# ai2cm/ace

Measured on AMD Instinct MI355X. Metric: rollout steps/sec (6-hourly forward steps of the 1-degree SFNO, whole job), higher is better.
Workload: dtype f32 (contractions with K>=32 on error-compensated fp16x3 MFMA, fp32 accumulate; DFT, norms, epilogues fp32; measured error vs fp64 below the fp32 CPU reference's); 1 GPU; ACE2-ERA5-shape 1deg SFNO rollout (BASELINE.json configs[1]): embed 384, 8 layers, dhconv, 44 in / 50 out channels, 180x360 legendre-gauss, lmax 180, mmax 181, B=1 member per GPU, random-init weights; members=1, members_per_gpu=1, graph=step, precision=f16x3, collective=none

## Files before the change

### ace_amd/csrc/capi.hip

```cpp
#include <hip/hip_runtime.h>

#include <algorithm>
#include <cmath>
#include <cstdio>
#include <cstdlib>
#include <cstring>
#include <map>
#include <memory>
#include <string>
#include <tuple>
#include <vector>

#include "../../include/ace_sfno.h"
#include "kernels.h"
#include "strip_pack.h"
#include "tables.h"

using namespace ace;

static thread_local std::string g_err;

static int fail(int code, const std::string& msg) {
    g_err = msg;
    return code;
}
#define HIP_TRY(expr)                                                                                      \
    do {                                                                                                   \
        hipError_t e__ = (expr);                                                                           \
        if (e__ != hipSuccess)                                                                             \
            return fail(ACE_ERR_RUNTIME, std::string(#expr) + ": " + hipGetErrorString(e__));              \
    } while (0)
#define ACE_TRY(expr)                \
    do {                             \
        int rc__ = (expr);           \
        if (rc__ != ACE_OK) return rc__; \
    } while (0)

extern "C" const char* ace_last_error(void) { return g_err.c_str(); }

namespace ace {
Switches read_switches() {
    auto on = [](const char* name) { const char* e = std::getenv(name); return e && e[0] && !(e[0] == '0' && !e[1]); };
    Switches sw;
    sw.no_fft = on("ACE_NO_FFT");
    sw.no_strip = on("ACE_NO_STRIP");
    sw.no_fold = on("ACE_NO_FOLD");
    sw.no_dhconv_strip = on("ACE_NO_DHCONV_STRIP");
#ifdef ACE_MEASUREMENT_SWITCHES
    sw.no_pk = on("ACE_NO_PK");
    sw.no_pk_sht = on("ACE_NO_PK_SHT");
#endif
    sw.no_enc_ws = on("ACE_NO_ENC_WS");
    sw.no_enc_pk = on("ACE_NO_ENC_PK");
    sw.no_cln_mfma = on("ACE_NO_CLN_MFMA");
    sw.no_cln_planes = on("ACE_NO_CLN_PLANES");
    sw.dense_grouped_filter = on("ACE_DENSE_GROUPED_FILTER");
    if (const char* e = std::getenv("ACE_CONV_WL")) sw.conv_wl = !(e[0] == '0' && !e[1]);
    if (const char* e = std::getenv("ACE_PLANES_STREAM")) sw.planes_stream = !(e[0] == '0' && !e[1]);
    if (const char* e = std::getenv("ACE_FUSED_PACK")) sw.fused_pack = !(e[0] == '0' && !e[1]);
    if (const char* e = std::getenv("ACE_CONV_WS")) {
        const std::string v(e);
        if (v == "all" || v == "1") sw.conv_ws_roles = 7;
        else sw.conv_ws_roles = (v.find("skip") != std::string::npos ? 1 : 0) | (v.find("fc1") != std::string::npos ? 2 : 0) |
                                (v.find("fc2") != std::string::npos ? 4 : 0);
    }
    return sw;
}
}
extern "C" int ace_version(void) { return 100; }

struct DevBuf {
    float* p = nullptr;
    size_t n = 0;
    DevBuf() = default;
    DevBuf(const DevBuf&) = delete;
    DevBuf& operator=(const DevBuf&) = delete;
    DevBuf(DevBuf&& o) noexcept : p(o.p), n(o.n) { o.p = nullptr; o.n = 0; }
    DevBuf& operator=(DevBuf&& o) noexcept {
        if (this != &o) { release(); p = o.p; n = o.n; o.p = nullptr; o.n = 0; }
        return *this;
    }
    ~DevBuf() { release(); }
    void release() {
        if (p) (void)hipFree(p);
        p = nullptr;
        n = 0;
    }
    hipError_t alloc(size_t count, bool zero = true) {
        release();
        if (count == 0) return hipSuccess;
        hipError_t e = hipMalloc(reinterpret_cast<void**>(&p), count * sizeof(float));
        if (e != hipSuccess) { p = nullptr; return e; }
        n = count;
        if (zero) e = hipMemset(p, 0, count * sizeof(float));
        return e;
    }
    hipError_t ensure(size_t count) { return count <= n ? hipSuccess : alloc(count); }
    hipError_t upload(const std::vector<float>& h) {
        hipError_t e = alloc(h.size(), false);
        if (e != hipSuccess) return e;
        return hipMemcpy(p, h.data(), h.size() * sizeof(float), hipMemcpyHostToDevice);
    }
};

struct ace_sht_plan {
    int nlat = 0, nlon = 0, lmax = 0, mmax = 0, Hp = 0, Lp = 0, Kfp = 0;
    Grid grid = GRID_LEGENDRE_GAUSS;
    DevBuf wt, pt, fc, fs, gc, gs;
    DevBuf X, D;
    DevBuf wt_hi, wt_lo, pt_hi, pt_lo;
    float wt_scale = 1.f, pt_scale = 1.f;
    float wt_winf = 0.f;
    bool f16 = false;
    DevBuf wt_frag, pt_frag, wt_off, pt_off;
    bool strip = false;
    DevBuf wt_ffrag, pt_ffrag, wt_foff, pt_foff;
    bool fold = false;
    DevBuf slots;
    Switches sw;
    mutable int route[2] = {-1, -1};
};
static int fold_route(const LegStripArgs& f) { return legendre_fold_is_big(f) ? 3 : 2; }

static float pow2_scale_for(const std::vector<float>& v) {
    float mx = 0.f;
    for (float x : v) mx = std::max(mx, std::fabs(x));
    int e = 0;
    if (mx > 0.f && std::isfinite(mx)) { (void)std::frexp(mx, &e); e = 10 - e; }
    return std::ldexp(1.0f, e);
}

static int plan_build(int nlat, int nlon, int lmax, int mmax, Grid g, std::unique_ptr<ace_sht_plan>& out,
                      bool f16 = false) {
    ShtTables t;
    std::string err = build_sht_tables(nlat, nlon, lmax, mmax, g, t);
    if (!err.empty()) return fail(ACE_ERR_INVALID, err);
    auto p = std::make_unique<ace_sht_plan>();
    p->sw = read_switches();
    p->nlat = t.nlat; p->nlon = t.nlon; p->lmax = t.lmax; p->mmax = t.mmax;
    p->Hp = t.Hp; p->Lp = t.Lp; p->Kfp = t.Kfp; p->grid = g;
    HIP_TRY(p->wt.upload(t.wt));
    HIP_TRY(p->pt.upload(t.pt));
    HIP_TRY(p->fc.upload(t.fc));
    HIP_TRY(p->fs.upload(t.fs));
    HIP_TRY(p->gc.upload(t.gc));
    HIP_TRY(p->gs.upload(t.gs));
    if (f16) {
        p->f16 = true;
        p->wt_scale = pow2_scale_for(t.wt);
        for (size_t r = 0; r < (size_t)t.mmax * t.lmax; ++r) {
            double rs = 0.0;
            for (int k = 0; k < t.nlat; ++k) rs += std::fabs((double)t.wt[r * t.Hp + k]);
            p->wt_winf = std::max(p->wt_winf, (float)(rs * (1.0 + 1e-6)));
        }
        p->pt_scale = pow2_scale_for(t.pt);
        const size_t hw = (t.wt.size() + 1) / 2, hp = (t.pt.size() + 1) / 2;
        HIP_TRY(p->wt_hi.alloc(hw, false)); HIP_TRY(p->wt_lo.alloc(hw, false));
        HIP_TRY(p->pt_hi.alloc(hp, false)); HIP_TRY(p->pt_lo.alloc(hp, false));
        HIP_TRY(launch_split_f16(p->wt.p, t.Hp, p->wt_hi.p, p->wt_lo.p, t.Hp, (long)t.mmax * t.lmax, t.Hp, p->wt_scale, nullptr));
        HIP_TRY(launch_split_f16(p->pt.p, t.Lp, p->pt_hi.p, p->pt_lo.p, t.Lp, (long)t.mmax * t.nlat, t.Lp, p->pt_scale, nullptr));
        HIP_TRY(hipDeviceSynchronize());
        auto up = [](const StripPack& sp, DevBuf& frag, DevBuf& off) -> hipError_t {
            hipError_t e = frag.alloc((sp.frags.size() + 1) / 2, false);
            if (e != hipSuccess) return e;
            e = hipMemcpy(frag.p, sp.frags.data(), sp.frags.size() * sizeof(uint16_t), hipMemcpyHostToDevice);
            if (e != hipSuccess) return e;
            e = off.alloc(sp.tile_off.size(), false);
            if (e != hipSuccess) return e;
            return hipMemcpy(off.p, sp.tile_off.data(), sp.tile_off.size() * sizeof(int), hipMemcpyHostToDevice);
        };
        if (t.nlat <= 192 && t.lmax <= 192) {
            StripPack sp;
            pack_legendre_strip(t.wt.data(), t.mmax, t.lmax, t.nlat, t.Hp, 0, p->wt_scale, sp);
            HIP_TRY(up(sp, p->wt_frag, p->wt_off));
            pack_legendre_strip(t.pt.data(), t.mmax, t.nlat, t.lmax, t.Lp, 1, p->pt_scale, sp);
            HIP_TRY(up(sp, p->pt_frag, p->pt_off));
            p->strip = true;
        }
        if ((t.nlat + 1) / 2 <= 16 * FOLD_NKP_BIG && (t.lmax + 1) / 2 <= 16 * FOLD_NKP_BIG && !p->sw.no_fold &&
            fold_symmetry_error(t.wt.data(), t.mmax, t.nlat, t.lmax, t.Hp, 0) < 2e-6 &&
            fold_symmetry_error(t.pt.data(), t.mmax, t.nlat, t.lmax, t.Lp, 1) < 2e-6) {
            StripPack sp;
            pack_legendre_fold(t.wt.data(), t.mmax, t.nlat, t.lmax, t.Hp, 0, p->wt_scale, sp);
            HIP_TRY(up(sp, p->wt_ffrag, p->wt_foff));
            pack_legendre_fold(t.pt.data(), t.mmax, t.nlat, t.lmax, t.Lp, 1, p->pt_scale, sp);
            HIP_TRY(up(sp, p->pt_ffrag, p->pt_foff));
            p->fold = true;
        }
    }
    out = std::move(p);
    return ACE_OK;
}

static int run_dft_forward(const ace_sht_plan& pl, const float* x, const float* sc, const float* sh, float* X, int Bt,
                           int C, hipStream_t s, unsigned* xmax = nullptr, const _Float16* xhi = nullptr,
                           const _Float16* xlo = nullptr, long sxp = 0, const unsigned* xslot = nullptr,
                           const PackFragArgs* ride = nullptr, bool* rode = nullptr) {
    DftArgs a;
    if (rode) *rode = false;
    if (ride && rode) { a.ride = *ride; a.nride = pack_frag_blocks(*ride); a.rode = rode; }
    a.omax = xmax;
    a.xhi = xhi; a.xlo = xlo; a.sxp = sxp; a.xslot = xslot;
    a.x = xhi ? nullptr : x; a.spec_out = X; a.tc = pl.fc.p; a.ts = pl.fs.p; a.ldt = pl.Kfp; a.sc = sc; a.sh = sh;
    a.Bt = Bt; a.C = C; a.H = pl.nlat; a.W = pl.nlon; a.Mm = pl.mmax; a.no_fft = pl.sw.no_fft;
    HIP_TRY(launch_dft_forward(a, s));
    return ACE_OK;
}
static int run_dft_inverse(const ace_sht_plan& pl, const float* X, const float* bias, float* y, int Bt, int C,
                           hipStream_t s, unsigned* ymax = nullptr) {
    DftArgs a;
    a.omax = ymax;
    a.spec = X; a.y = y; a.tc = pl.gc.p; a.ts = pl.gs.p; a.ldt = pl.Kfp; a.bias = bias;
    a.Bt = Bt; a.C = C; a.H = pl.nlat; a.W = pl.nlon; a.Mm = pl.mmax; a.no_fft = pl.sw.no_fft;
    HIP_TRY(launch_dft_inverse(a, s));
    return ACE_OK;
}
static int run_legendre_forward(const ace_sht_plan& pl, const float* X, float* D, long N2, hipStream_t s,
                                const unsigned* xmax = nullptr, unsigned* dmax = nullptr, bool planes = false) {
    GemmArgs g;
    g.omax = planes ? nullptr : dmax;
    g.A = pl.wt.p; g.lda = pl.Hp; g.sA = (long)pl.lmax * pl.Hp;
    g.B = X; g.ldb = N2; g.sB = (long)pl.nlat * N2;
    g.C = D; g.ldc = (long)pl.mmax * N2; g.sC = N2;
    g.M = pl.lmax; g.N = (int)N2; g.K = pl.nlat; g.nbatch = pl.mmax; g.a_kpad = pl.Hp;
    g.tri = TRI_ROWS_GE_BATCH;
    if ((pl.strip || pl.fold) && !pl.sw.no_strip && xmax) {
        LegStripArgs a;
        a.B = X; a.b_kstride = N2; a.b_moff = (long)pl.nlat * N2;
        a.A = reinterpret_cast<const _Float16*>(pl.wt_frag.p); a.tile_off = reinterpret_cast<const int*>(pl.wt_off.p);
        a.ascale = pl.wt_scale; a.bmax = xmax;
        a.c_rstride = (long)pl.mmax * N2; a.c_moff = N2;
        a.N = (int)N2; a.K = pl.nlat; a.R = pl.lmax; a.nbatch = pl.mmax; a.mode = 0;
        if (planes) {
            a.Chi = reinterpret_cast<_Float16*>(D);
            a.Clo = a.Chi + (size_t)pl.lmax * pl.mmax * N2;
            a.cw = pl.wt_winf; a.cslot = dmax;
        } else {
            a.C = D; a.omax = dmax;
        }
        if (pl.fold && !pl.sw.no_fold) {
            LegStripArgs f = a;
            f.A = reinterpret_cast<const _Float16*>(pl.wt_ffrag.p); f.tile_off = reinterpret_cast<const int*>(pl.wt_foff.p);
            if (legendre_fold_eligible(f)) {
                HIP_TRY(launch_legendre_fold(f, s));
                pl.route[0] = fold_route(f);
                return ACE_OK;
            }
        }
        if (pl.strip && legendre_strip_eligible(a)) {
            HIP_TRY(launch_legendre_strip(a, s));
            pl.route[0] = 1;
            return ACE_OK;
        }
    }
    pl.route[0] = 0;
    if (planes) {
        if (!(pl.f16 && xmax && dmax && gemm_f16x3_eligible(g))) return fail(ACE_ERR_STATE, "legendre planes path not eligible");
        _Float16* Dh = reinterpret_cast<_Float16*>(D);
        _Float16* Dl = Dh + (size_t)pl.lmax * pl.mmax * N2;
        HIP_TRY(launch_gemm_f16x3_planes(g, pl.wt_hi.p, pl.wt_lo.p, pl.wt_scale, xmax, Dh, Dl, pl.wt_winf, dmax, s));
        return ACE_OK;
    }
    if (pl.f16 && xmax && gemm_f16x3_eligible(g)) {
        HIP_TRY(launch_gemm_f16x3(g, pl.wt_hi.p, pl.wt_lo.p, pl.wt_scale, 1.f, s, xmax, dmax));
        return ACE_OK;
    }
    HIP_TRY(launch_gemm(g, s));
    return ACE_OK;
}
static int run_legendre_inverse(const ace_sht_plan& pl, const float* E, float* X, long N2, hipStream_t s,
                                const unsigned* emax = nullptr, bool dry = false) {
    GemmArgs g;
    g.A = pl.pt.p; g.lda = pl.Lp; g.sA = (long)pl.nlat * pl.Lp;
    g.B = E; g.ldb = (long)pl.mmax * N2; g.sB = N2;
    g.C = X; g.ldc = N2; g.sC = (long)pl.nlat * N2;
    g.M = pl.nlat; g.N = (int)N2; g.K = pl.lmax; g.nbatch = pl.mmax; g.a_kpad = pl.Lp;
    g.tri = TRI_K_GE_BATCH;
    if ((pl.strip || pl.fold) && !pl.sw.no_strip && emax) {
        LegStripArgs a;
        a.B = E; a.b_kstride = (long)pl.mmax * N2; a.b_moff = N2;
        a.A = reinterpret_cast<const _Float16*>(pl.pt_frag.p); a.tile_off = reinterpret_cast<const int*>(pl.pt_off.p);
        a.ascale = pl.pt_scale; a.bmax = emax;
        a.C = X; a.c_rstride = N2; a.c_moff = (long)pl.nlat * N2;
        a.N = (int)N2; a.K = pl.lmax; a.R = pl.nlat; a.nbatch = pl.mmax; a.mode = 1;
        if (pl.fold && !pl.sw.no_fold) {
            LegStripArgs f = a;
            f.A = reinterpret_cast<const _Float16*>(pl.pt_ffrag.p); f.tile_off = reinterpret_cast<const int*>(pl.pt_foff.p);
            if (legendre_fold_eligible(f)) {
                if (!dry) HIP_TRY(launch_legendre_fold(f, s));
                pl.route[1] = fold_route(f);
                return ACE_OK;
            }
        }
        if (pl.strip && legendre_strip_eligible(a)) {
            if (!dry) HIP_TRY(launch_legendre_strip(a, s));
            pl.route[1] = 1;
            return ACE_OK;
        }
    }
    pl.route[1] = 0;
    if (dry) return ACE_OK;
    if (pl.f16 && emax && gemm_f16x3_eligible(g)) {
        HIP_TRY(launch_gemm_f16x3(g, pl.pt_hi.p, pl.pt_lo.p, pl.pt_scale, 1.f, s, emax, nullptr));
        return ACE_OK;
    }
    HIP_TRY(launch_gemm(g, s));
    return ACE_OK;
}

extern "C" int ace_sht_plan_create_ex(int nlat, int nlon, int lmax, int mmax, const char* grid, int precision,
                                      ace_sht_plan** plan) {
    if (!plan || !grid) return fail(ACE_ERR_INVALID, "null argument");
    if (precision != 0 && precision != 1) return fail(ACE_ERR_INVALID, "precision must be 0 (fp32) or 1 (f16x3)");
    Grid g;
    if (std::string(grid) == "healpix") return fail(ACE_ERR_INVALID, "'healpix' grid not supported");
    if (!parse_grid(grid, &g)) return fail(ACE_ERR_INVALID, "Unknown quadrature mode");
    std::unique_ptr<ace_sht_plan> p;
    ACE_TRY(plan_build(nlat, nlon, lmax, mmax, g, p, precision == 1));
    if (precision == 1) HIP_TRY(p->slots.alloc((size_t)2 * AMAX_SHARDS));
    *plan = p.release();
    return ACE_OK;
}
extern "C" int ace_sht_plan_create(int nlat, int nlon, int lmax, int mmax, const char* grid, ace_sht_plan** plan) {
    return ace_sht_plan_create_ex(nlat, nlon, lmax, mmax, grid, 0, plan);
}
extern "C" void ace_sht_plan_destroy(ace_sht_plan* plan) { delete plan; }
extern "C" int ace_sht_plan_dims(const ace_sht_plan* p, int* nlat, int* nlon, int* lmax, int* mmax) {
    if (!p) return fail(ACE_ERR_INVALID, "null plan");
    if (nlat) *nlat = p->nlat;
    if (nlon) *nlon = p->nlon;
    if (lmax) *lmax = p->lmax;
    if (mmax) *mmax = p->mmax;
    return ACE_OK;
}

extern "C" int ace_sht_plan_route(const ace_sht_plan* p, int* forward, int* inverse) {
    if (!p) return fail(ACE_ERR_INVALID, "null plan");
    if (forward) *forward = p->route[0];
    if (inverse) *inverse = p->route[1];
    return ACE_OK;
}

extern "C" int ace_sht_forward(ace_sht_plan* p, const float* x, float* coeffs, int n, void* stream) {
    if (!p || !x || !coeffs || n <= 0) return fail(ACE_ERR_INVALID, "ace_sht_forward: bad argument");
    hipStream_t s = static_cast<hipStream_t>(stream);
    const long N2 = 2L * n;
    HIP_TRY(p->X.ensure(((size_t)p->mmax * p->nlat + LEG_STRIP_SLACK_ROWS) * N2));
    HIP_TRY(p->D.ensure(((size_t)p->lmax + LEG_STRIP_SLACK_ROWS) * p->mmax * N2));
    unsigned* xmax = nullptr;
    if (p->f16 && p->slots.p) {
        xmax = reinterpret_cast<unsigned*>(p->slots.p);
        HIP_TRY(launch_zero_u32(xmax, 2 * AMAX_SHARDS, s));
    }
    ACE_TRY(run_dft_forward(*p, x, nullptr, nullptr, p->X.p, 1, n, s, xmax));
    ACE_TRY(run_legendre_forward(*p, p->X.p, p->D.p, N2, s, xmax, xmax ? xmax + AMAX_SHARDS : nullptr));
    HIP_TRY(launch_spec_to_ref(p->D.p, coeffs, 1, n, p->lmax, p->mmax, s));
    return ACE_OK;
}
extern "C" int ace_sht_inverse(ace_sht_plan* p, const float* coeffs, float* x, int n, void* stream) {
    if (!p || !x || !coeffs || n <= 0) return fail(ACE_ERR_INVALID, "ace_sht_inverse: bad argument");
    hipStream_t s = static_cast<hipStream_t>(stream);
    const long N2 = 2L * n;
    HIP_TRY(p->X.ensure(((size_t)p->mmax * p->nlat + LEG_STRIP_SLACK_ROWS) * N2));
    HIP_TRY(p->D.ensure(((size_t)p->lmax + LEG_STRIP_SLACK_ROWS) * p->mmax * N2));
    unsigned* emax = nullptr;
    if (p->f16 && p->slots.p) {
        emax = reinterpret_cast<unsigned*>(p->slots.p);
        HIP_TRY(launch_zero_u32(emax, 2 * AMAX_SHARDS, s));
    }
    ACE_TRY(run_legendre_inverse(*p, p->D.p, p->X.p, N2, s, emax, true));
    HIP_TRY(launch_ref_to_spec(coeffs, p->D.p, 1, n, p->lmax, p->mmax, s, emax, p->route[1] != 0));
    ACE_TRY(run_legendre_inverse(*p, p->D.p, p->X.p, N2, s, emax));
    ACE_TRY(run_dft_inverse(*p, p->X.p, nullptr, x, 1, n, s));
    return ACE_OK;
}

extern "C" int ace_sht_tables_host(int nlat, int nlon, int lmax, int mmax, const char* grid, int which,
                                   void* out_host) {
    if (!grid || !out_host) return fail(ACE_ERR_INVALID, "null argument");
    Grid g;
    if (!parse_grid(grid, &g)) return fail(ACE_ERR_INVALID, "Unknown quadrature mode");
    if (which == 2 || which == 3) {
        std::vector<double> x, w;
        quadrature(g, nlat, x, w);
        std::memcpy(out_host, (which == 2 ? x : w).data(), sizeof(double) * nlat);
        return ACE_OK;
    }
    ShtTables t;
    std::string err = build_sht_tables(nlat, nlon, lmax, mmax, g, t);
    if (!err.empty()) return fail(ACE_ERR_INVALID, err);
    float* o = static_cast<float*>(out_host);
    for (int m = 0; m < t.mmax; ++m)
        for (int l = 0; l < t.lmax; ++l)
            for (int k = 0; k < t.nlat; ++k) {
                const size_t dst = ((size_t)m * t.lmax + l) * t.nlat + k;
                if (which == 0) o[dst] = t.wt[((size_t)m * t.lmax + l) * t.Hp + k];
                else if (which == 1) o[dst] = t.pt[((size_t)m * t.nlat + k) * t.Lp + l];
                else return fail(ACE_ERR_INVALID, "unknown table id");
            }
    return ACE_OK;
}

extern "C" int ace_conv1x1(const float* x, const float* weight, const float* bias, float* y, int n, int cin, int cout,
                           long hw, int act, void* stream) {
    if (!x || !weight || !y || n <= 0 || cin <= 0 || cout <= 0 || hw <= 0)
        return fail(ACE_ERR_INVALID, "ace_conv1x1: bad argument");
    GemmArgs g;
    g.A = weight; g.lda = cin; g.sA = 0;
    g.B = x; g.ldb = hw; g.sB = (long)cin * hw;
    g.C = y; g.ldc = hw; g.sC = (long)cout * hw;
    g.bias = bias; g.M = cout; g.N = (int)hw; g.K = cin; g.nbatch = n; g.act = act;
    g.a_kpad = cin;
    HIP_TRY(launch_gemm(g, static_cast<hipStream_t>(stream)));
    return ACE_OK;
}

extern "C" int ace_conv1x1_f16x3(const float* x, const float* weight, const float* bias, float* y, int n, int cin,
                                 int cout, long hw, int act, void* stream) {
    if (!x || !weight || !y || n <= 0 || cin <= 0 || cout <= 0 || hw <= 0)
        return fail(ACE_ERR_INVALID, "ace_conv1x1_f16x3: bad argument");
    hipStream_t s = static_cast<hipStream_t>(stream);
    const int pitch = (cin + 31) & ~31;
    std::vector<float> host((size_t)cout * cin);
    HIP_TRY(hipStreamSynchronize(s));
    HIP_TRY(hipMemcpy(host.data(), weight, host.size() * sizeof(float), hipMemcpyDeviceToHost));
    float mx = 0.f;
    for (float v : host) mx = std::max(mx, std::fabs(v));
    int e = 0;
    if (mx > 0.f && std::isfinite(mx)) { (void)std::frexp(mx, &e); e = 10 - e; }
    const float ascale = std::ldexp(1.0f, e);
    DevBuf hi, lo;
    const size_t halves = (size_t)cout * pitch;
    HIP_TRY(hi.alloc((halves + 1) / 2, false));
    HIP_TRY(lo.alloc((halves + 1) / 2, false));
    HIP_TRY(launch_split_f16(weight, cin, hi.p, lo.p, pitch, cout, cin, ascale, s));
    GemmArgs g;
    g.lda = pitch; g.sA = 0; g.a_kpad = pitch;
    g.B = x; g.ldb = hw; g.sB = (long)cin * hw;
    g.C = y; g.ldc = hw; g.sC = (long)cout * hw;
    g.bias = bias; g.M = cout; g.N = (int)hw; g.K = cin; g.nbatch = n; g.act = act;
    if (!gemm_f16x3_eligible(g)) return fail(ACE_ERR_INVALID, "ace_conv1x1_f16x3: needs 16-byte aligned x and hw % 4 == 0");
    if (g.act == ACT_GELU) g.act = ACT_GELU_FAST;
    DevBuf slotbuf;
    HIP_TRY(slotbuf.alloc(AMAX_SHARDS));
    unsigned* xslot = reinterpret_cast<unsigned*>(slotbuf.p);
    HIP_TRY(launch_absmax(x, (long)n * cin * hw, xslot, s));
    HIP_TRY(launch_gemm_f16x3(g, hi.p, lo.p, ascale, 1.0f, s, xslot, nullptr));
    HIP_TRY(hipStreamSynchronize(s));
    return ACE_OK;
}

struct PreparedWeight { DevBuf hi, lo; int pitch = 0; float ascale = 1.f, winf = 0.f; };
static int prepare_weight(const float* weight, int rows, int cols, hipStream_t s, PreparedWeight& out, bool tiled) {
    std::vector<float> host((size_t)rows * cols);
    HIP_TRY(hipStreamSynchronize(s));
    HIP_TRY(hipMemcpy(host.data(), weight, host.size() * sizeof(float), hipMemcpyDeviceToHost));
    float mx = 0.f;
    for (int r = 0; r < rows; ++r) {
        double rs = 0.0;
        for (int c = 0; c < cols; ++c) { const float v = std::fabs(host[(size_t)r * cols + c]); mx = std::max(mx, v); rs += v; }
        out.winf = std::max(out.winf, (float)(rs * (1.0 + 1e-6)));
    }
    int e = 0;
    if (mx > 0.f && std::isfinite(mx)) { (void)std::frexp(mx, &e); e = 10 - e; }
    out.ascale = std::ldexp(1.0f, e);
    out.pitch = (cols + 31) & ~31;
    const size_t halves = (size_t)((rows + 15) / 16 * 16) * out.pitch;
    HIP_TRY(out.hi.alloc((halves + 1) / 2, false));
    HIP_TRY(out.lo.alloc((halves + 1) / 2, false));
    if (tiled) HIP_TRY(launch_split_f16_tiled(weight, cols, out.hi.p, out.lo.p, out.pitch, rows, cols, out.ascale, s));
    else HIP_TRY(launch_split_f16(weight, cols, out.hi.p, out.lo.p, out.pitch, rows, cols, out.ascale, s));
    return ACE_OK;
}

extern "C" int ace_mlp_f16x3(const float* x, const float* w1, const float* b1, const float* w2, const float* b2, float* y,
                             int n, int cin, int hid, int cout, long hw, int act, void* stream) {
    if (!x || !w1 || !w2 || !y || n <= 0 || cin <= 0 || hid <= 0 || cout <= 0 || hw <= 0)
        return fail(ACE_ERR_INVALID, "ace_mlp_f16x3: bad argument");
    if (cin % 8 != 0 || hid % 8 != 0 || hw % 4 != 0)
        return fail(ACE_ERR_INVALID, "ace_mlp_f16x3: needs cin % 8 == 0, hid % 8 == 0, hw % 4 == 0");
    hipStream_t s = static_cast<hipStream_t>(stream);
    PreparedWeight p1, p2;
    ACE_TRY(prepare_weight(w1, hid, cin, s, p1, true));
    ACE_TRY(prepare_weight(w2, cout, hid, s, p2, true));
    float b1max = 0.f;
    if (b1) {
        std::vector<float> hb((size_t)hid);
        HIP_TRY(hipMemcpy(hb.data(), b1, hb.size() * sizeof(float), hipMemcpyDeviceToHost));
        for (float v : hb) b1max = std::max(b1max, std::fabs(v));
    }
    DevBuf slots, xp, up;
    HIP_TRY(slots.alloc(2 * AMAX_SHARDS, true));
    HIP_TRY(xp.alloc((size_t)n * cin * hw, true));
    HIP_TRY(up.alloc((size_t)n * hid * hw, true));
    unsigned* xslot = reinterpret_cast<unsigned*>(slots.p);
    unsigned* uslot = xslot + AMAX_SHARDS;
    _Float16* xh = reinterpret_cast<_Float16*>(xp.p);
    _Float16* xl = xh + (size_t)n * cin * hw;
    _Float16* uh = reinterpret_cast<_Float16*>(up.p);
    _Float16* ul = uh + (size_t)n * hid * hw;
    HIP_TRY(launch_absmax(x, (long)n * cin * hw, xslot, s));
    HIP_TRY(launch_pack_pformat(x, hw, (long)cin * hw, cin, (int)hw, n, nullptr, nullptr, 0, xslot, xh, xl, hw,
                                (long)cin * hw, s));
    Gemm4Args a;
    a.Ahi = reinterpret_cast<const _Float16*>(p1.hi.p); a.Alo = reinterpret_cast<const _Float16*>(p1.lo.p);
    a.lda = p1.pitch; a.ascale = p1.ascale; a.a_tiled = 1;
    a.Bhi = xh; a.Blo = xl; a.ldn = hw; a.sB = (long)cin * hw; a.bmax = xslot;
    a.Chi = uh; a.Clo = ul; a.ldnc = hw; a.sCp = (long)hid * hw; a.cw = p1.winf; a.cb = b1max; a.cslot = uslot;
    a.bias = b1; a.M = hid; a.N = (int)hw; a.K = cin; a.nbatch = n;
    a.act = act == ACT_GELU ? ACT_GELU_FAST : act;
    HIP_TRY(launch_gemm_f16x3_packed(a, s));
    Gemm4Args b;
    b.Ahi = reinterpret_cast<const _Float16*>(p2.hi.p); b.Alo = reinterpret_cast<const _Float16*>(p2.lo.p);
    b.lda = p2.pitch; b.ascale = p2.ascale; b.a_tiled = 1;
    b.Bhi = uh; b.Blo = ul; b.ldn = hw; b.sB = (long)hid * hw; b.bmax = uslot;
    b.C = y; b.ldc = hw; b.sC = (long)cout * hw;
    b.bias = b2; b.M = cout; b.N = (int)hw; b.K = hid; b.nbatch = n; b.act = ACT_NONE;
    HIP_TRY(launch_gemm_f16x3_packed(b, s));
    HIP_TRY(hipStreamSynchronize(s));
    return ACE_OK;
}

static hipError_t upload_dhconv_units(int L, int Mrows, int trimul, int C, DevBuf& buf, int* per_xcd) {
    std::vector<int> u;
    *per_xcd = dhconv_build_units(L, Mrows, trimul, C, u);
    hipError_t e = buf.alloc(u.size(), false);
// ... 136 lines not shown
    HIP_TRY(launch_unpack_denormalize(src, mean, std_, dsts, strides, batch, nch, hw, static_cast<hipStream_t>(stream)));
    return ACE_OK;
}

struct Weight {
    std::string name;
    long numel = 0;
    DevBuf buf;
    bool set = false;
    int block = -1;
    bool is_filter = false;
    long ext_numel = 0;
    int rows = 0, cols = 0, pitch = 0;
    DevBuf hi, lo;
    float ascale = 1.f;
    DevBuf thi, tlo;
    DevBuf frag0;
    float wabs = 0.f;
    float winf = 0.f;
    float absmax = 0.f;
};

struct GraphKey {
    const float* in; float* out; int batch;
    bool operator<(const GraphKey& o) const { return std::tie(in, out, batch) < std::tie(o.in, o.out, o.batch); }
};

struct ace_sfno {
    ace_sfno_config cfg;
    int H = 0, W = 0, C = 0, L = 0, Mm = 0, hid = 0, Bmax = 1;
    long HW = 0;
    long HWs = 0;
    int Hs = 0, Ws = 0;
    std::unique_ptr<ace_sht_plan> plan_lg, plan_data_own;
    ace_sht_plan* plan_data = nullptr;
    std::vector<std::unique_ptr<Weight>> weights;
    std::map<std::string, int> index;
    std::vector<DevBuf> wx;
    std::vector<DevBuf> wx_hi, wx_lo;
    std::vector<float> wx_scale;
    std::vector<char> wx_compact;
    std::vector<DevBuf> dh_units; std::vector<int> dh_units_per_xcd;
    std::vector<char> wx_native;
    DevBuf h0, h1, Y, T, R, U, X, D, E, stats;
    DevBuf P;
    DevBuf cln_stats;
    DevBuf inN;
    std::unique_ptr<ace_sht_plan> plan_res;
    DevBuf resX, resD, inF;
    DevBuf P2;
    DevBuf part;
    DevBuf Wp0, Wp1;
    DevBuf Wq1;
    DevBuf Wq0;
    DevBuf zero_c;
    DevBuf inP;
    DevBuf pe_slot;
    DevBuf phys;
    int nstrips = 0;
    DevBuf bf0, bf1;
    DevBuf amax;
    bool taps_on = false;
    std::vector<DevBuf> taps;
    std::map<GraphKey, hipGraphExec_t> graphs;
    hipStream_t capture_stream = nullptr;
    long weights_generation = 0;
    bool graphs_stale = false;
    mutable int norm_batch = 0;
    mutable hipStream_t norm_stream = nullptr;
    Switches sw;

    const float* w(const std::string& name) const {
        auto it = index.find(name);
        return it == index.end() ? nullptr : weights[it->second]->buf.p;
    }
    const Weight* find(const std::string& name) const {
        auto it = index.find(name);
        return it == index.end() ? nullptr : weights[it->second].get();
    }
};

static void add_weight(ace_sfno* n, const std::string& name, long numel, int block = -1, bool is_filter = false) {
    auto w = std::make_unique<Weight>();
    w->name = name; w->numel = numel; w->block = block; w->is_filter = is_filter;
    n->index[name] = (int)n->weights.size();
    n->weights.push_back(std::move(w));
}
static void add_conv_weight(ace_sfno* n, const std::string& name, int rows, int cols) {
    add_weight(n, name, (long)rows * cols);
    Weight& w = *n->weights.back();
    w.rows = rows; w.cols = cols; w.pitch = (cols + 31) & ~31;
}

static bool skip_on_conv_ws(const Switches& sw, int K, int M, long HW) { return conv_ws_eligible(K, M, HW, 0, sw.conv_ws_roles); }
static bool fc1_on_conv_ws(const Switches& sw, int K, int M, long HW) { return conv_ws_eligible(K, M, HW, 1, sw.conv_ws_roles); }
static bool fc2_on_conv_ws(const Switches& sw, int K, int M, long HW) { return conv_ws_eligible(K, M, HW, 2, sw.conv_ws_roles); }
static bool fc1_on_conv_wl(const Switches& sw, int K, int M, long HW) { return sw.conv_wl && conv_wl_eligible(K, M, HW); }
static bool cln_skip_on_conv_ws(const Switches& sw, int K, int M, long HW) {
    return (sw.conv_ws_roles & 1) && conv_ws_eligible(K, M, HW, -1, sw.conv_ws_roles);
}

extern "C" int ace_sfno_create(const ace_sfno_config* cfg, ace_sfno** out) {
    if (!cfg || !out) return fail(ACE_ERR_INVALID, "null argument");
    const ace_sfno_config& c = *cfg;
    if (c.scale_factor < 1) return fail(ACE_ERR_INVALID, "scale_factor must be >= 1");
    if ((c.scale_factor != 1 || c.residual_filter_factor > 1) && c.normalization_layer == 2)
        return fail(ACE_ERR_INVALID, "scale_factor / residual_filter_factor != 1 are not built for the noise-conditioned nets");
    if (c.residual_filter_factor < 0) return fail(ACE_ERR_INVALID, "residual_filter_factor must be >= 1");
    if (c.in_chans <= 0 || c.out_chans <= 0 || c.embed_dim <= 0 || c.num_layers <= 0 || c.nlat < 2 || c.nlon < 2)
        return fail(ACE_ERR_INVALID, "non-positive dimension in ace_sfno_config");
    if (c.operator_type != 0 && c.operator_type != 1) return fail(ACE_ERR_INVALID, "Unsupported operator type");
    if (c.normalization_layer < 0 || c.normalization_layer > 3)
        return fail(ACE_ERR_INVALID, "normalization_layer must be 'none', 'instance_norm', conditional layer norm or 'layer_norm'");
    const bool cln = c.normalization_layer == 2;
    if (cln) {
        if (c.operator_type != 1) return fail(ACE_ERR_INVALID, "Only 'dhconv' operator_type is supported for NoiseConditionedSFNO models.");
        if (c.noise_embed_dim < 0 || c.noise_embed_dim > 512) return fail(ACE_ERR_INVALID, "noise_embed_dim must be in [0, 512]");
        if (c.filter_num_groups < 1 || c.embed_dim % c.filter_num_groups != 0)
            return fail(ACE_ERR_INVALID, "embed_dim must be divisible by filter_num_groups");
    }
    if (c.activation_function < 1 || c.activation_function > 3)
        return fail(ACE_ERR_INVALID, "Unknown activation function");
    if (c.data_grid != GRID_LEGENDRE_GAUSS && c.data_grid != GRID_EQUIANGULAR && c.data_grid != GRID_LOBATTO)
        return fail(ACE_ERR_INVALID, "data_grid must be 'legendre-gauss', 'equiangular' or 'lobatto'");
    if (c.encoder_layers < 0) return fail(ACE_ERR_INVALID, "encoder_layers must be >= 0");
    if (c.precision != 0 && c.precision != 1) return fail(ACE_ERR_INVALID, "precision must be 0 (fp32) or 1 (f16x3)");

    auto n = std::make_unique<ace_sfno>();
    n->cfg = c;
    n->sw = read_switches();
    n->H = c.nlat; n->W = c.nlon; n->C = c.embed_dim; n->HW = (long)c.nlat * c.nlon;
    n->Bmax = c.max_batch > 0 ? c.max_batch : 1;
    const int sf = c.scale_factor;
    n->Hs = c.nlat / sf; n->Ws = c.nlon / sf; n->HWs = (long)n->Hs * n->Ws;
    if (n->Hs < 1 || n->Ws < 2) return fail(ACE_ERR_INVALID, "scale_factor leaves no grid");
    n->L = (int)(n->Hs * c.hard_thresholding_fraction);
    n->Mm = (int)((n->Ws / 2 + 1) * c.hard_thresholding_fraction);
    if (n->L < 1 || n->Mm < 1) return fail(ACE_ERR_INVALID, "hard_thresholding_fraction leaves no modes");
    n->hid = (int)(c.embed_dim * c.mlp_ratio);

    ACE_TRY(plan_build(n->Hs, n->Ws, n->L, n->Mm, GRID_LEGENDRE_GAUSS, n->plan_lg, c.precision == 1));
    if (c.data_grid == GRID_LEGENDRE_GAUSS && sf == 1) {
        n->plan_data = n->plan_lg.get();
    } else {
        ACE_TRY(plan_build(c.nlat, c.nlon, n->L, n->Mm, (Grid)c.data_grid, n->plan_data_own, c.precision == 1));
        n->plan_data = n->plan_data_own.get();
    }

    if (c.residual_filter_factor > 1 && c.big_skip) {
        const int rl = c.nlat / c.residual_filter_factor, rm = c.nlon / c.residual_filter_factor / 2 + 1;
        if (rl < 1 || rm < 1) return fail(ACE_ERR_INVALID, "residual_filter_factor leaves no modes");
        ACE_TRY(plan_build(c.nlat, c.nlon, rl, rm, (Grid)c.data_grid, n->plan_res, false));
        const size_t n2 = (size_t)n->Bmax * 2 * c.in_chans;
        HIP_TRY(n->resX.alloc(((size_t)rm * c.nlat + LEG_STRIP_SLACK_ROWS) * n2));
        HIP_TRY(n->resD.alloc(((size_t)rl + LEG_STRIP_SLACK_ROWS) * rm * n2));
        HIP_TRY(n->inF.alloc((size_t)n->Bmax * c.in_chans * n->HW));
    }

    const long C = n->C, HW = n->HW;
    if (c.pos_embed) add_weight(n.get(), "pos_embed", C * HW);
    long cur = c.in_chans;
    for (int j = 0; j < c.encoder_layers; ++j) {
        add_conv_weight(n.get(), "encoder." + std::to_string(2 * j) + ".weight", (int)C, (int)cur);
        add_weight(n.get(), "encoder." + std::to_string(2 * j) + ".bias", C);
        cur = C;
    }
    add_conv_weight(n.get(), "encoder." + std::to_string(2 * c.encoder_layers) + ".weight", (int)C, (int)cur);
    for (int i = 0; i < c.num_layers; ++i) {
        const std::string p = "blocks." + std::to_string(i) + ".";
        if (c.normalization_layer == 1) { add_weight(n.get(), p + "norm0.weight", C); add_weight(n.get(), p + "norm0.bias", C); }
        const long hw_n0 = i == 0 ? HW : n->HWs;
        const long hw_n1 = (i == 0 || i + 1 < c.num_layers) ? n->HWs : HW;
        if (c.normalization_layer == 3) { add_weight(n.get(), p + "norm0.weight", hw_n0); add_weight(n.get(), p + "norm0.bias", hw_n0); }
        auto add_cln = [&](const std::string& q, long ch) {
            if (c.noise_embed_dim > 0) {
                add_weight(n.get(), q + "W_scale_2d.weight", ch * c.noise_embed_dim);
                add_weight(n.get(), q + "W_bias_2d.weight", ch * c.noise_embed_dim);
            }
            if (c.affine_norms) { add_weight(n.get(), q + "norm.weight", ch); add_weight(n.get(), q + "norm.bias", ch); }
        };
        if (cln) add_cln(p + "norm0.", C);
        const long fw = c.operator_type == 1 ? C * C * n->L * 2 : C * C * (long)n->L * n->Mm * 2;
        add_weight(n.get(), p + "filter.filter.weight", fw, i, true);
        if (cln) n->weights.back()->ext_numel = fw / c.filter_num_groups;
        add_weight(n.get(), p + "filter.filter.bias", C);
        add_conv_weight(n.get(), p + "inner_skip.weight", (int)C, (int)C);
        add_weight(n.get(), p + "inner_skip.bias", C);
        if (c.normalization_layer == 1) { add_weight(n.get(), p + "norm1.weight", C); add_weight(n.get(), p + "norm1.bias", C); }
        if (c.normalization_layer == 3) { add_weight(n.get(), p + "norm1.weight", hw_n1); add_weight(n.get(), p + "norm1.bias", hw_n1); }
        if (cln) add_cln(p + "norm1.", C);
        if (c.use_mlp) {
            add_conv_weight(n.get(), p + "mlp.fwd.0.weight", n->hid, (int)C);
            add_weight(n.get(), p + "mlp.fwd.0.bias", n->hid);
            add_conv_weight(n.get(), p + "mlp.fwd.2.weight", (int)C, n->hid);
            add_weight(n.get(), p + "mlp.fwd.2.bias", C);
        }
    }
    cur = C + (c.big_skip ? c.in_chans : 0);
    for (int j = 0; j < c.encoder_layers; ++j) {
        add_conv_weight(n.get(), "decoder." + std::to_string(2 * j) + ".weight", (int)C, (int)cur);
        add_weight(n.get(), "decoder." + std::to_string(2 * j) + ".bias", C);
        cur = C;
    }
    add_conv_weight(n.get(), "decoder." + std::to_string(2 * c.encoder_layers) + ".weight", c.out_chans, (int)cur);
    if (cln && c.normalize_big_skip && c.big_skip) {
        if (c.noise_embed_dim > 0) {
            add_weight(n.get(), "norm_big_skip.W_scale_2d.weight", (long)c.in_chans * c.noise_embed_dim);
            add_weight(n.get(), "norm_big_skip.W_bias_2d.weight", (long)c.in_chans * c.noise_embed_dim);
        }
        if (c.affine_norms) { add_weight(n.get(), "norm_big_skip.norm.weight", c.in_chans); add_weight(n.get(), "norm_big_skip.norm.bias", c.in_chans); }
    }

    n->wx.resize(c.num_layers);
    n->wx_hi.resize(c.num_layers);
    n->wx_lo.resize(c.num_layers);
    n->wx_scale.assign(c.num_layers, 1.f);
    n->wx_compact.assign(c.num_layers, 0);
    n->wx_native.assign(c.num_layers, 0);
    for (int i = 0; i < c.num_layers; ++i) {
        const bool mixed = (n->plan_data != n->plan_lg.get()) && (i == 0 || i == c.num_layers - 1);
        n->wx_compact[i] = (!n->sw.no_pk_sht && c.precision == 1 && c.operator_type == 1 && n->C % 128 == 0 && !mixed &&
                            ((long)n->Bmax * 2 * n->C) % 4 == 0) ? 1 : 0;
        const bool strip_rows_ok = ((long)n->Mm * n->Bmax + 191) / 192 <= 65535;
        n->wx_native[i] = (n->wx_compact[i] && cln && c.filter_num_groups > 1 && !n->sw.dense_grouped_filter && !n->sw.no_dhconv_strip &&
                           strip_rows_ok && dhconv_native_groups_ok(n->C, c.filter_num_groups)) ? 1 : 0;
    }
    if (c.operator_type == 1 && c.precision == 1 && n->C % 128 == 0) {
        n->dh_units.resize(n->Bmax);
        n->dh_units_per_xcd.assign(n->Bmax, 0);
        for (int b = 1; b <= n->Bmax; ++b)
            HIP_TRY(upload_dhconv_units(n->L, n->Mm * b, b, n->C, n->dh_units[b - 1], &n->dh_units_per_xcd[b - 1]));
    }
    const size_t act = (size_t)n->Bmax * C * HW;
    const size_t spec_x = ((size_t)n->Mm * n->H + LEG_STRIP_SLACK_ROWS) * n->Bmax * 2 * C;
    const size_t spec_d = ((size_t)n->L + LEG_STRIP_SLACK_ROWS) * n->Mm * n->Bmax * 2 * C;
    HIP_TRY(n->h0.alloc(act));
    HIP_TRY(n->h1.alloc(act));
    HIP_TRY(n->Y.alloc(act));
    HIP_TRY(n->T.alloc(act));
    if (n->plan_data != n->plan_lg.get()) HIP_TRY(n->R.alloc(act));
    if (c.use_mlp) HIP_TRY(n->U.alloc((size_t)n->Bmax * n->hid * HW, true));
    if (c.precision == 1) {
        HIP_TRY(n->P.alloc(act, true));
        if (c.normalization_layer == 1 && c.use_mlp) {
            HIP_TRY(n->P2.alloc(act, true));
            n->nstrips = (int)((HW + 31) / 32) + 8;
            if (fc1_on_conv_ws(n->sw, (int)C, n->hid, HW) || fc1_on_conv_wl(n->sw, (int)C, n->hid, HW))
                HIP_TRY(n->Wq1.alloc((size_t)n->Bmax * n->hid * C, true));
            if (skip_on_conv_ws(n->sw, (int)C, (int)C, HW)) HIP_TRY(n->Wq0.alloc((size_t)n->Bmax * C * C, true));
            HIP_TRY(n->zero_c.alloc((size_t)C, true));
            HIP_TRY(n->inP.alloc((size_t)n->Bmax * ((c.in_chans + 7) / 8 * 8) * n->HW, true));
            HIP_TRY(n->pe_slot.alloc(64, true));
            HIP_TRY(n->part.alloc((size_t)2 * n->Bmax * n->nstrips * C * 4, true));
            const size_t cp = (size_t)((C + 31) & ~31);
            HIP_TRY(n->Wp0.alloc((size_t)n->Bmax * ((C + 15) / 16 * 16) * cp, true));
            HIP_TRY(n->Wp1.alloc((size_t)n->Bmax * ((n->hid + 15) / 16 * 16) * cp, true));
        }
    }
    HIP_TRY(n->X.alloc(spec_x));
    HIP_TRY(n->D.alloc(spec_d));
    HIP_TRY(n->E.alloc(spec_d));
    HIP_TRY(n->stats.alloc((size_t)4 * n->Bmax * C));
    if (cln) {
        HIP_TRY(n->cln_stats.alloc((size_t)2 * n->Bmax * HW));
        if (c.normalize_big_skip && c.big_skip) HIP_TRY(n->inN.alloc((size_t)n->Bmax * c.in_chans * HW));
    }
    HIP_TRY(n->amax.alloc((size_t)(16 + 12 * c.num_layers + 1) * AMAX_SHARDS));
    if (c.normalization_layer == 1) {
        HIP_TRY(n->bf0.alloc((size_t)n->Bmax * C));
        if (c.use_mlp) {
            HIP_TRY(n->bf1.alloc((size_t)n->Bmax * n->hid));
        }
    }
    *out = n.release();
    return ACE_OK;
}

extern "C" void ace_sfno_destroy(ace_sfno* n) {
    if (!n) return;
    for (auto& kv : n->graphs) (void)hipGraphExecDestroy(kv.second);
    if (n->capture_stream) (void)hipStreamDestroy(n->capture_stream);
    delete n;
}

extern "C" long ace_sfno_weights_generation(const ace_sfno* n) { return n ? n->weights_generation : -1; }

extern "C" long ace_sfno_workspace_size(const ace_sfno* n, int batch) {
    if (!n) { (void)fail(ACE_ERR_INVALID, "null argument"); return -1; }
    if (batch <= 0 || batch > n->Bmax) {
        (void)fail(ACE_ERR_INVALID, "batch " + std::to_string(batch) + " outside [1, max_batch=" + std::to_string(n->Bmax) + "]");
        return -1;
    }
    size_t fl = 0;
    auto add = [&](const DevBuf& b) { fl += b.n; };
    for (const DevBuf* b : {&n->h0, &n->h1, &n->Y, &n->T, &n->R, &n->U, &n->X, &n->D, &n->E, &n->stats, &n->P, &n->cln_stats, &n->inN,
                            &n->P2, &n->part, &n->Wp0, &n->Wp1, &n->Wq1, &n->Wq0, &n->zero_c, &n->inP, &n->pe_slot, &n->bf0,
                            &n->bf1, &n->amax, &n->phys})
        add(*b);
    for (const auto& t : n->taps) add(t);
    for (const auto& v : {&n->wx, &n->wx_hi, &n->wx_lo})
        for (const auto& b : *v) add(b);
    for (const auto& w : n->weights)
        for (const DevBuf* b : {&w->buf, &w->hi, &w->lo, &w->thi, &w->tlo, &w->frag0}) add(*b);
    auto plan_bytes = [&](const ace_sht_plan* p) {
        if (!p) return;
        for (const DevBuf* b : {&p->wt, &p->pt, &p->fc, &p->fs, &p->gc, &p->gs, &p->X, &p->D, &p->wt_hi, &p->wt_lo, &p->pt_hi, &p->pt_lo,
                                &p->wt_frag, &p->pt_frag, &p->wt_off, &p->pt_off, &p->slots})
            add(*b);
    };
    plan_bytes(n->plan_lg.get());
    plan_bytes(n->plan_data_own.get());
    plan_bytes(n->plan_res.get());
    for (const DevBuf* b : {&n->resX, &n->resD, &n->inF}) add(*b);
    return (long)(fl * sizeof(float));
}

extern "C" int ace_sfno_num_weights(const ace_sfno* n) { return n ? (int)n->weights.size() : 0; }
extern "C" const char* ace_sfno_weight_name(const ace_sfno* n, int i) {
    if (!n || i < 0 || i >= (int)n->weights.size()) return nullptr;
    return n->weights[i]->name.c_str();
}
extern "C" long ace_sfno_weight_numel(const ace_sfno* n, int i) {
    if (!n || i < 0 || i >= (int)n->weights.size()) return -1;
    return n->weights[i]->ext_numel ? n->weights[i]->ext_numel : n->weights[i]->numel;
}

extern "C" int ace_sfno_set_weight(ace_sfno* n, const char* name, const float* src, long numel, void* stream) {
    if (!n || !name || !src) return fail(ACE_ERR_INVALID, "null argument");
    auto it = n->index.find(name);
    if (it == n->index.end()) return fail(ACE_ERR_INVALID, std::string("unknown parameter '") + name + "'");
    Weight& w = *n->weights[it->second];
    const long expect = w.ext_numel ? w.ext_numel : w.numel;
    if (numel != expect)
        return fail(ACE_ERR_INVALID, std::string("size mismatch for ") + name + ": expected " +
                                         std::to_string(expect) + " elements, got " + std::to_string(numel));
    hipStream_t s = static_cast<hipStream_t>(stream);
    const bool native_groups = w.ext_numel && w.is_filter && w.block >= 0 && n->wx_native[w.block];
    if (native_groups) {
        if (!w.buf.p) HIP_TRY(w.buf.alloc((size_t)w.ext_numel, false));
        HIP_TRY(hipMemcpyAsync(w.buf.p, src, sizeof(float) * w.ext_numel, hipMemcpyDeviceToDevice, s));
        src = nullptr;
        numel = w.ext_numel;
    } else if (w.ext_numel) {
        if (!w.buf.p) HIP_TRY(w.buf.alloc((size_t)w.numel, false));
        HIP_TRY(launch_csfno_weight_to_dense(src, w.buf.p, n->C, n->cfg.filter_num_groups, n->L, s));
        src = nullptr;
        numel = w.numel;
    }
    if (w.pitch > 0) {
        if (!w.buf.p) HIP_TRY(w.buf.alloc((size_t)w.rows * w.pitch, true));
        HIP_TRY(hipMemcpy2DAsync(w.buf.p, sizeof(float) * w.pitch, src, sizeof(float) * w.cols, sizeof(float) * w.cols,
                                 w.rows, hipMemcpyDeviceToDevice, s));
    } else if (src) {
        if (!w.buf.p) HIP_TRY(w.buf.alloc((size_t)numel, false));
        HIP_TRY(hipMemcpyAsync(w.buf.p, src, sizeof(float) * numel, hipMemcpyDeviceToDevice, s));
    }
    if (w.is_filter && n->cfg.operator_type == 1) {
        const size_t cnt = (size_t)n->L * 2 * n->C * 2 * n->C;
        const bool packed = n->cfg.precision == 1 && (2 * n->C) % 32 == 0;
        if (packed) {
            DevBuf slotbuf;
            HIP_TRY(slotbuf.alloc(AMAX_SHARDS));
            HIP_TRY(launch_absmax(w.buf.p, numel, reinterpret_cast<unsigned*>(slotbuf.p), s));
            unsigned bits[AMAX_SHARDS];
            HIP_TRY(hipMemcpyAsync(bits, slotbuf.p, sizeof(bits), hipMemcpyDeviceToHost, s));
            HIP_TRY(hipStreamSynchronize(s));
            float mx = 0.f;
            for (unsigned b : bits) { float f; std::memcpy(&f, &b, 4); mx = std::max(mx, f); }
            int e = 0;
            if (mx > 0.f && std::isfinite(mx)) { (void)std::frexp(mx, &e); e = 10 - e; }
            n->wx_scale[w.block] = std::ldexp(1.0f, e);
            const bool compact = n->wx_compact[w.block] != 0;
            const size_t halves = native_groups ? cnt / 2 / n->cfg.filter_num_groups : (compact ? cnt / 2 : cnt);
            if (!n->wx_hi[w.block].p) HIP_TRY(n->wx_hi[w.block].alloc((halves + 1) / 2, false));
            if (!n->wx_lo[w.block].p) HIP_TRY(n->wx_lo[w.block].alloc((halves + 1) / 2, false));
            if (native_groups)
                HIP_TRY(launch_pack_dhconv_f16g(w.buf.p, n->wx_hi[w.block].p, n->wx_lo[w.block].p, n->C, n->cfg.filter_num_groups, n->L,
                                                n->wx_scale[w.block], s));
            else if (compact)
                HIP_TRY(launch_pack_dhconv_f16c(w.buf.p, n->wx_hi[w.block].p, n->wx_lo[w.block].p, n->C, n->C, n->L,
                                                n->wx_scale[w.block], s));
            else
                HIP_TRY(launch_pack_dhconv_f16(w.buf.p, n->wx_hi[w.block].p, n->wx_lo[w.block].p, n->C, n->C, n->L,
                                               n->wx_scale[w.block], s));
        } else {
            DevBuf& wx = n->wx[w.block];
            if (!wx.p) HIP_TRY(wx.alloc(cnt, false));
            HIP_TRY(launch_expand_dhconv_weight(w.buf.p, wx.p, n->C, n->C, n->L, s));
        }
    }
    HIP_TRY(hipStreamSynchronize(s));
    if (w.pitch > 0 && n->cfg.precision == 1) {
        std::vector<float> host((size_t)w.rows * w.pitch);
        HIP_TRY(hipMemcpy(host.data(), w.buf.p, host.size() * sizeof(float), hipMemcpyDeviceToHost));
        float mx = 0.f;
        for (float v : host) mx = std::max(mx, std::fabs(v));
        w.wabs = mx;
        w.winf = 0.f;
        for (int r = 0; r < w.rows; ++r) {
            double rs = 0.0;
            for (int cidx = 0; cidx < w.cols; ++cidx) rs += std::fabs((double)host[(size_t)r * w.pitch + cidx]);
            w.winf = std::max(w.winf, (float)(rs * (1.0 + 1e-6)));
        }
        int e = 0;
        if (mx > 0.f && std::isfinite(mx)) { (void)std::frexp(mx, &e); e = 10 - e; }
        w.ascale = std::ldexp(1.0f, e);
        const size_t halves = (size_t)w.rows * w.pitch;
        if (!w.hi.p) HIP_TRY(w.hi.alloc((halves + 1) / 2, false));
        if (!w.lo.p) HIP_TRY(w.lo.alloc((halves + 1) / 2, false));
        HIP_TRY(launch_split_f16(w.buf.p, w.pitch, w.hi.p, w.lo.p, w.pitch, w.rows, w.pitch, w.ascale, s));
        const size_t thalves = (size_t)((w.rows + 15) / 16 * 16) * w.pitch;
        if (!w.thi.p) HIP_TRY(w.thi.alloc((thalves + 1) / 2, false));
// ... 326 lines not shown
    return ACE_OK;
}

static int pack_act(const Fwd& f, const float* x, long x_bs, int cin, const float* sc, const float* sh, const unsigned* slot,
                    void* hi, void* lo) {
    HIP_TRY(launch_pack_pformat(x, f.HW, x_bs, cin, (int)f.HW, f.B, sc, sh, sc ? cin : 0, slot, hi, lo, f.HW, (long)cin * f.HW, f.s));
    return ACE_OK;
}
struct PkOpts {
    const Weight* w = nullptr;
    const void* fhi = nullptr; const void* flo = nullptr; const unsigned* fslot = nullptr; long f_stride = 0;
    const float* bias = nullptr; long sbias = 0;
    const void* bhi = nullptr; const void* blo = nullptr; int cin = 0; const unsigned* in_slot = nullptr;
    float* out = nullptr; int cout = 0; unsigned* omax = nullptr;
    const float* R = nullptr; long r_bs = 0; const float* rsc = nullptr; const float* rsh = nullptr;
    int act = ACT_NONE;
    void* ohi = nullptr; void* olo = nullptr; float cb = 0.f; unsigned* cslot = nullptr;
    const unsigned* cinb = nullptr; const unsigned* rmax = nullptr;
    float* part = nullptr;
};
static int conv_packed(const Fwd& f, const PkOpts& o) {
    Gemm4Args a;
    if (o.fhi) {
        a.Ahi = static_cast<const _Float16*>(o.fhi); a.Alo = static_cast<const _Float16*>(o.flo);
        a.sA = o.f_stride; a.amax = o.fslot;
    } else {
        a.Ahi = reinterpret_cast<const _Float16*>(o.w->thi.p); a.Alo = reinterpret_cast<const _Float16*>(o.w->tlo.p);
        a.sA = 0; a.ascale = o.w->ascale;
    }
    a.lda = o.w->pitch; a.a_tiled = 1;
    a.Bhi = static_cast<const _Float16*>(o.bhi); a.Blo = static_cast<const _Float16*>(o.blo);
    a.ldn = f.HW; a.sB = (long)o.cin * f.HW; a.bmax = o.in_slot;
    a.C = o.out; a.ldc = f.HW; a.sC = (long)o.cout * f.HW; a.omax = o.omax;
    a.Chi = static_cast<_Float16*>(o.ohi); a.Clo = static_cast<_Float16*>(o.olo); a.ldnc = f.HW; a.sCp = (long)o.cout * f.HW;
    a.cw = o.w->winf; a.cb = o.cb; a.cslot = o.cslot; a.cinb = o.cinb; a.rmax = o.rmax;
    a.part = reinterpret_cast<float4*>(o.part);
    a.bias = o.bias; a.sbias = o.sbias;
    a.R = o.R; a.ldr = f.HW; a.sR = o.r_bs; a.rsc = o.rsc; a.rsh = o.rsh; a.srs = o.rsc ? o.cout : 0;
    a.M = o.cout; a.N = (int)f.HW; a.K = o.cin; a.nbatch = f.B;
    a.act = o.act == ACT_GELU ? ACT_GELU_FAST : o.act;
    HIP_TRY(launch_gemm_f16x3_packed(a, f.s));
    return ACE_OK;
}
static ConvStripArgs strip_args(const Fwd& f, const _Float16* xhi, const _Float16* xlo, const unsigned* xslot, int cin, int cout, int act) {
    ConvStripArgs k;
    k.Xhi = xhi; k.Xlo = xlo; k.ldn = f.HW; k.sX = (long)cin * f.HW; k.xslot = xslot;
    k.C = cin; k.M = cout; k.HW = (int)f.HW; k.nbatch = f.B; k.act = act;
    return k;
}
static void static_frags(ConvStripArgs& k, const Weight& w, const float* bias) {
    k.A = reinterpret_cast<const _Float16*>(w.frag0.p); k.sA = 0; k.ascale = w.ascale;
    k.bias = bias; k.sbias = 0;
}

static int cond_norm(const Fwd& f, const float* x, float* y, const std::string& q, int Cc, unsigned* omax, _Float16* phi = nullptr,
                     _Float16* plo = nullptr, bool fp32_needed = true, bool* planes_done = nullptr) {
    const ace_sfno* n = f.n;
    const int J = n->cfg.noise_embed_dim;
    const Weight* wsc = n->find(q + "W_scale_2d.weight");
    const Weight* wbi = n->find(q + "W_bias_2d.weight");
    const Weight* wga = n->find(q + "norm.weight");
    const Weight* wbe = n->find(q + "norm.bias");
    if (planes_done) *planes_done = false;
    ClnMfmaArgs a;
    a.x = x; a.y = y; a.sx = (long)Cc * f.HW; a.C = Cc; a.HW = f.HW; a.nbatch = f.B; a.eps = 1e-5f; a.omax = omax;
    a.gamma = f.W(q + "norm.weight"); a.beta = f.W(q + "norm.bias");
    if (n->cfg.precision == 1 && f.noise && wsc && wbi && wsc->frag0.p && wbi->frag0.p && !n->sw.no_cln_mfma) {
        a.cond = f.noise; a.scond = (long)J * f.HW; a.J = J; a.cslot = f.slot(16 + 12 * n->cfg.num_layers);
        a.As = reinterpret_cast<const _Float16*>(wsc->frag0.p); a.Ab = reinterpret_cast<const _Float16*>(wbi->frag0.p);
        a.ascale_s = wsc->ascale; a.ascale_b = wbi->ascale;
        if (phi && plo && omax && !n->sw.no_cln_planes && cln_mfma_planes_ok(a) && (!a.gamma || (wga && wbe))) {
            a.Phi = phi; a.Plo = plo; a.sP = (long)Cc * f.HW;
            a.gmax = a.gamma ? wga->absmax : 1.f; a.bmax = a.gamma ? wbe->absmax : 0.f;
            a.ws_inf = wsc->winf; a.wb_inf = wbi->winf;
            if (!fp32_needed) a.y = nullptr;
        }
        if (cln_mfma_eligible(a)) {
            HIP_TRY(launch_cln_mfma(a, f.s));
            if (planes_done) *planes_done = a.Phi != nullptr;
            return ACE_OK;
        }
        a.Phi = a.Plo = nullptr; a.y = y;
    }
    HIP_TRY(launch_cond_layer_norm(x, f.noise, a.gamma, a.beta, f.W(q + "W_scale_2d.weight"), f.W(q + "W_bias_2d.weight"), 1e-5f,
                                   n->cln_stats.p, y, f.B, Cc, J, f.HW, f.s, omax));
    return ACE_OK;
}

static int enqueue_encoder(Fwd& f, const float* in) {
    const ace_sfno* n = f.n;
    const ace_sfno_config& c = n->cfg;
    const FwdRoute& r = *f.route;
    const int C = n->C, Cin = c.in_chans, act = c.activation_function;
    const long HW = f.HW, actB = f.actB();
    if (c.precision == 1) {
        HIP_TRY(launch_zero_u32(f.slot(0), (long)n->amax.n, f.s));
        HIP_TRY(launch_absmax(in, (long)f.B * Cin * HW, f.slot(0), f.s));
    }
    const float* cur = in;
    long cur_bs = (long)Cin * HW;
    int curC = Cin;
    float* ping[2] = {n->Y.p, n->T.p};
    if (r.enc_hidden_planes) {
        const Weight& b0 = f.wt("encoder.0.bias");
        const int cin8 = (Cin + 7) / 8 * 8;
        _Float16* Ih = reinterpret_cast<_Float16*>(n->inP.p);
        _Float16* Il = Ih + (size_t)n->Bmax * cin8 * HW;
        HIP_TRY(launch_pack_pformat(in, HW, (long)Cin * HW, Cin, (int)HW, f.B, nullptr, nullptr, 0, f.slot(0), Ih, Il, HW, (long)cin8 * HW, f.s));
        PkOpts o;
        o.w = &f.wt("encoder.0.weight"); o.bias = b0.buf.p;
        o.bhi = Ih; o.blo = Il; o.cin = cin8; o.in_slot = f.slot(0);
        o.cout = C; o.act = act;
        o.ohi = f.PAh; o.olo = f.PAl; o.cb = b0.absmax; o.cslot = f.slot(1);
        ACE_TRY(conv_packed(f, o));
    } else {
        for (int j = 0; j < c.encoder_layers; ++j) {
            const std::string p = "encoder." + std::to_string(2 * j);
            ACE_TRY(conv(f, conv_weight(n, p + ".weight", p + ".bias"), cur, cur_bs, curC, nullptr, 0, -1, ping[j & 1], C,
                         nullptr, 0, nullptr, nullptr, act, nullptr, nullptr, f.slot(j), nullptr, f.slot(1 + j)));
            cur = ping[j & 1]; cur_bs = actB; curC = C;
        }
    }
    const std::string last = "encoder." + std::to_string(2 * c.encoder_layers) + ".weight";
    if (r.enc_planes) {
        const Weight& we = f.wt(last);
        if (!r.enc_hidden_planes) ACE_TRY(pack_act(f, cur, cur_bs, C, nullptr, nullptr, f.slot(c.encoder_layers), f.PAh, f.PAl));
        ConvStripArgs k = strip_args(f, f.PAh, f.PAl, f.slot(c.encoder_layers), C, C, ACT_NONE);
        static_frags(k, we, n->zero_c.p);
        k.R = f.W("pos_embed"); k.sR = 0;
        if (!r.enc_planes_only) { k.Cf = f.h; k.sCf = actB; }
        k.Chi = f.PBh; k.Clo = f.PBl; k.sCp = (long)C * HW; k.cslot = f.hslot(0);
        k.cw = we.winf; k.cb = 0.f; k.rmax = reinterpret_cast<const unsigned*>(n->pe_slot.p);
        k.part = reinterpret_cast<float4*>(f.part_h); k.nstrips32 = r.enc_nparts;
        HIP_TRY(launch_conv_ws(k, f.s));
    } else {
        ACE_TRY(conv(f, conv_weight(n, last, ""), cur, cur_bs, curC, nullptr, 0, -1, f.h, C, c.pos_embed ? f.W("pos_embed") : nullptr, 0,
                     nullptr, nullptr, ACT_NONE, nullptr, nullptr, f.slot(c.encoder_layers), nullptr, f.hslot(0)));
    }
    MARK(ST_ENCODER);
    if (n->taps_on) HIP_TRY(hipMemcpyAsync(n->taps[0].p, f.h, sizeof(float) * f.B * actB, hipMemcpyDeviceToDevice, f.s));
    return ACE_OK;
}

static int enqueue_big_skip_source(Fwd& f, const float* in) {
    const ace_sfno* n = f.n;
    const ace_sfno_config& c = n->cfg;
    const int Cin = c.in_chans;
    f.skip_in = in;
    f.skip_in_slot = f.slot(0);
    if (f.route->noise_range)
        HIP_TRY(launch_absmax(f.noise, (long)f.B * c.noise_embed_dim * f.HW, f.slot(16 + 12 * c.num_layers), f.s));
    if (n->plan_res) {
        const long NR = (long)f.B * 2 * Cin;
        ACE_TRY(run_dft_forward(*n->plan_res, in, nullptr, nullptr, n->resX.p, f.B, Cin, f.s));
        ACE_TRY(run_legendre_forward(*n->plan_res, n->resX.p, n->resD.p, NR, f.s));
        ACE_TRY(run_legendre_inverse(*n->plan_res, n->resD.p, n->resX.p, NR, f.s));
        ACE_TRY(run_dft_inverse(*n->plan_res, n->resX.p, nullptr, n->inF.p, f.B, Cin, f.s, f.slot(7)));
        f.skip_in = n->inF.p;
        f.skip_in_slot = f.slot(7);
    }
    if (c.normalization_layer == 2 && c.big_skip && c.normalize_big_skip) {
        ACE_TRY(cond_norm(f, in, n->inN.p, "norm_big_skip.", Cin, f.slot(7)));
        f.skip_in = n->inN.p;
        f.skip_in_slot = f.slot(7);
    }
    return ACE_OK;
}

static int enqueue_norm0(Fwd& f, int i, const BlockRoute& b) {
    const ace_sfno* n = f.n;
    const int C = n->C, sb = 16 + 12 * i, kind = n->cfg.normalization_layer;
    const std::string p = "blocks." + std::to_string(i) + ".";
    if (n->cfg.precision == 1 && i + 1 >= 8) HIP_TRY(launch_zero_u32(f.hslot(i + 1), AMAX_SHARDS, f.s));
    f.a0 = f.b0 = nullptr;
    f.n0_planes = false;
    if (kind == 0) return ACE_OK;
    if (kind == 2) {
        ACE_TRY(cond_norm(f, f.h, f.h, p + "norm0.", C, f.slot(sb + 3), b.n0_to_planes ? f.PAh : nullptr,
                          b.n0_to_planes ? f.Pl() : nullptr, true, &f.n0_planes));
    } else if (kind == 3) {
        HIP_TRY(launch_spatial_layer_norm(f.h, f.W(p + "norm0.weight"), f.W(p + "norm0.bias"), 1e-6f, (long)f.B * C, f.HW, f.h, f.slot(sb + 3), f.s));
    } else {
        if (b.in_planes)
            HIP_TRY(launch_instnorm_finalize(reinterpret_cast<const float4*>(f.part_h), b.in_nparts, f.B, C, f.HW,
                                             f.W(p + "norm0.weight"), f.W(p + "norm0.bias"), 1e-6f, f.sc0, f.sh0, f.slot(sb + 3), f.s));
        else
            HIP_TRY(launch_instnorm_stats(f.h, f.W(p + "norm0.weight"), f.W(p + "norm0.bias"), 1e-6f, f.B, C, f.HW, f.sc0, f.sh0, f.s,
                                          f.slot(sb + 3)));
        f.a0 = f.sc0; f.b0 = f.sh0;
    }
    MARK(ST_NORM0);
    return ACE_OK;
}

static int enqueue_forward_transform(Fwd& f, int i, const BlockRoute& b) {
    const ace_sfno* n = f.n;
    const int C = n->C, sb = 16 + 12 * i, B = f.B;
    const long N2 = (long)B * 2 * C;
    unsigned *xmax = f.slot(sb + 0), *dmax = f.slot(sb + 1);
    PackFragArgs skip_pack;
    if (b.ride_skip_pack) {
        const std::string p = "blocks." + std::to_string(i) + ".";
        const Weight& wsk = f.wt(p + "inner_skip.weight");
        skip_pack.W = wsk.buf.p; skip_pack.ldw = wsk.pitch; skip_pack.O = C; skip_pack.I = C; skip_pack.order = 0;
        skip_pack.a = f.a0; skip_pack.wmax = wsk.wabs; skip_pack.scale_static = 1.f; skip_pack.wslot = f.slot(sb + 8);
        skip_pack.dst = reinterpret_cast<_Float16*>(n->Wq0.p); skip_pack.sDst = (long)C * C * 2;
        skip_pack.b = f.b0; skip_pack.bias = f.wt(p + "inner_skip.bias").buf.p; skip_pack.bf = n->bf0.p; skip_pack.nsamples = B;
    }
    const PackFragArgs* ride = b.ride_skip_pack ? &skip_pack : nullptr;
    if (b.in_planes_only)
        ACE_TRY(run_dft_forward(*b.fwd, nullptr, f.a0, f.b0, n->X.p, B, C, f.s, xmax, f.PBh, f.PBl, (long)C * f.HW, f.hslot(i), ride, &f.skip_pack_rode));
    else
        ACE_TRY(run_dft_forward(*b.fwd, f.h, f.a0, f.b0, n->X.p, B, C, f.s, xmax, nullptr, nullptr, 0, nullptr, ride, &f.skip_pack_rode));
    MARK(ST_DFT_FWD);
    ACE_TRY(run_legendre_forward(*b.fwd, n->X.p, n->D.p, N2, f.s, xmax, dmax, b.dplanes));
    MARK(ST_LEGENDRE_FWD);
    f.res = f.h; f.ra = f.a0; f.rb = f.b0;
    if (b.scale_residual) {
        ACE_TRY(run_legendre_inverse(*b.inv, n->D.p, n->X.p, N2, f.s, dmax));
        MARK(ST_LEGENDRE_INV);
        ACE_TRY(run_dft_inverse(*b.inv, n->X.p, nullptr, n->R.p, B, C, f.s));
        MARK(ST_DFT_INV);
        f.res = n->R.p; f.ra = nullptr; f.rb = nullptr;
    }
    return ACE_OK;
}

static int enqueue_contraction(Fwd& f, int i, const BlockRoute& b) {
    const ace_sfno* n = f.n;
    const int C = n->C, sb = 16 + 12 * i, B = f.B;
    const long N2 = (long)B * 2 * C;
    unsigned *dmax = f.slot(sb + 1), *emax = f.slot(sb + 2);
    switch (b.filter) {
    case FLT_DHCONV_STRIP:
        HIP_TRY(launch_dhconv_strip(dhconv_strip_args(n, i, B, dmax, emax), f.s));
        break;
    case FLT_PACKED_TILE: {
        Gemm4Args a;
        a.Ahi = reinterpret_cast<const _Float16*>(n->D.p);
        a.Alo = a.Ahi + (size_t)n->L * n->Mm * N2;
        a.lda = 2 * C; a.sA = (long)n->Mm * N2; a.amax = dmax;
        a.Bhi = reinterpret_cast<const _Float16*>(n->wx_hi[i].p);
        a.Blo = reinterpret_cast<const _Float16*>(n->wx_lo[i].p);
        a.ldn = 2 * C; a.sB = (long)2 * C * 2 * C; a.bscale = n->wx_scale[i];
        if (n->wx_compact[i]) { a.cplx = C; a.ldn = C; a.sB = (long)2 * C * C; a.tile = 1; }
        a.C = n->E.p; a.ldc = 2 * C; a.sC = (long)n->Mm * N2; a.omax = emax;
        a.M = n->Mm * B; a.N = 2 * C; a.K = 2 * C; a.nbatch = n->L;
        a.tri = TRI_ROWS_LE_BATCH; a.trimul = B;
        HIP_TRY(launch_gemm_f16x3_packed(a, f.s));
        break;
    }
    case FLT_ADYN_F16X3:
    case FLT_FP32: {
        GemmArgs g;
        g.A = n->D.p; g.lda = 2 * C; g.sA = (long)n->Mm * N2;
        g.B = n->wx[i].p; g.ldb = 2 * C; g.sB = (long)2 * C * 2 * C;
        g.C = n->E.p; g.ldc = 2 * C; g.sC = (long)n->Mm * N2;
        g.M = n->Mm * B; g.N = 2 * C; g.K = 2 * C; g.nbatch = n->L; g.a_kpad = 2 * C;
        g.tri = TRI_ROWS_LE_BATCH; g.trimul = B;
        g.omax = emax;
        if (b.filter == FLT_ADYN_F16X3)
            HIP_TRY(launch_gemm_f16x3_adyn(g, n->wx_hi[i].p, n->wx_lo[i].p, 2 * C, (long)2 * C * 2 * C, n->wx_scale[i], dmax, emax, f.s));
        else
            HIP_TRY(launch_gemm(g, f.s));
        break;
    }
    case FLT_DIAGONAL:
        HIP_TRY(launch_contract_diagonal(n->D.p, f.W("blocks." + std::to_string(i) + ".filter.filter.weight"), n->E.p, B, C, C, n->L, n->Mm, f.s, emax));
        break;
    }
    MARK(ST_CONTRACT);
    return ACE_OK;
}

static int enqueue_inverse_transform(Fwd& f, int i, const BlockRoute& b) {
    const ace_sfno* n = f.n;
    const int sb = 16 + 12 * i;
    ACE_TRY(run_legendre_inverse(*b.inv, n->E.p, n->X.p, (long)f.B * 2 * n->C, f.s, f.slot(sb + 2)));
    MARK(ST_LEGENDRE_INV);
    ACE_TRY(run_dft_inverse(*b.inv, n->X.p, f.W("blocks." + std::to_string(i) + ".filter.filter.bias"), n->Y.p, f.B, n->C, f.s, f.slot(sb + 7)));
    MARK(ST_DFT_INV);
    f.HW = b.hw_out;
    return ACE_OK;
}

static int enqueue_fused_body(Fwd& f, int i, const BlockRoute& b) {
    const ace_sfno* n = f.n;
    const int C = n->C, hid = n->hid, B = f.B, act = n->cfg.activation_function, sb = 16 + 12 * i;
    const long HW = f.HW, actB = f.actB();
    hipStream_t s = f.s;
    const std::string p = "blocks." + std::to_string(i) + ".";
    const Weight &ws = f.wt(p + "inner_skip.weight"), &bsw = f.wt(p + "inner_skip.bias");
    const Weight &w1 = f.wt(p + "mlp.fwd.0.weight"), &b1w = f.wt(p + "mlp.fwd.0.bias");
    const Weight &w2 = f.wt(p + "mlp.fwd.2.weight"), &b2w = f.wt(p + "mlp.fwd.2.bias");
    const long cp = ws.pitch;
    _Float16* F0h = reinterpret_cast<_Float16*>(n->Wp0.p);
    const long f0s = (long)((C + 15) / 16 * 16) * cp;
    _Float16* F0l = F0h + (size_t)n->Bmax * f0s;
    _Float16* F1h = reinterpret_cast<_Float16*>(n->Wp1.p);
    const long f1s = (long)((hid + 15) / 16 * 16) * cp;
    _Float16* F1l = F1h + (size_t)n->Bmax * f1s;
    _Float16 *Uh = f.Uh(), *Ul = f.Ul();

    const float* skip_bias = bsw.buf.p;
    long skip_sbias = 0;
    const unsigned* in_slot = f.slot(b.skip_slot);
    if (b.in_planes) {
        if (b.skip != CONV_WS)
            HIP_TRY(launch_fold_affine_f16(ws.buf.p, ws.pitch, ws.wabs, f.ra, f.rb, bsw.buf.p, F0h, F0l, n->bf0.p, B, C, C, cp, f0s, f.slot(sb + 8), s));
        skip_bias = n->bf0.p; skip_sbias = C; in_slot = f.hslot(i);
    } else {
        ACE_TRY(pack_act(f, f.res, actB, C, f.ra, f.rb, in_slot, f.PBh, f.PBl));
    }
    if (b.skip == CONV_WS) {
        ConvStripArgs k = strip_args(f, f.PBh, f.PBl, in_slot, C, C, ACT_GELU);
        if (b.in_planes) {
            _Float16* Q0 = reinterpret_cast<_Float16*>(n->Wq0.p);
            if (!f.skip_pack_rode)
                HIP_TRY(launch_pack_conv_frag(ws.buf.p, ws.pitch, C, C, 0, f.ra, ws.wabs, 1.f, f.slot(sb + 8), Q0, (long)C * C * 2, B, s,
                                              f.rb, bsw.buf.p, n->bf0.p));
            k.A = Q0; k.sA = (long)C * C * 2; k.aslot = f.slot(sb + 8);
        } else {
            k.A = reinterpret_cast<const _Float16*>(ws.frag0.p); k.sA = 0; k.ascale = ws.ascale;
        }
        k.bias = skip_bias; k.sbias = skip_sbias;
        k.R = n->Y.p; k.sR = actB;
        k.cw = ws.winf; k.cb = bsw.absmax; k.cinb = f.slot(sb + 3); k.rmax = f.slot(sb + 7);
        k.Chi = f.PAh; k.Clo = f.PAl; k.sCp = (long)C * HW; k.cslot = f.slot(sb + 4);
        k.part = reinterpret_cast<float4*>(f.part_t); k.nstrips32 = b.t_nparts;
        HIP_TRY(launch_conv_ws(k, s));
    } else {
        PkOpts o;
        o.w = &ws; o.cin = C; o.cout = C; o.act = act;
        if (b.in_planes) { o.fhi = F0h; o.flo = F0l; o.fslot = f.slot(sb + 8); o.f_stride = f0s; }
        o.bias = skip_bias; o.sbias = skip_sbias;
        o.bhi = f.PBh; o.blo = f.PBl; o.in_slot = in_slot;
        o.R = n->Y.p; o.r_bs = actB;
        o.ohi = f.PAh; o.olo = f.PAl; o.cb = bsw.absmax; o.cslot = f.slot(sb + 4); o.cinb = f.slot(sb + 3); o.rmax = f.slot(sb + 7);
        o.part = f.part_t;
        ACE_TRY(conv_packed(f, o));
    }
    MARK(ST_INNER_SKIP);

    HIP_TRY(launch_instnorm_finalize(reinterpret_cast<const float4*>(f.part_t), b.t_nparts, B, C, HW, f.W(p + "norm1.weight"),
                                     f.W(p + "norm1.bias"), 1e-6f, f.sc1, f.sh1, f.slot(sb + 5), s));
    if (b.fc1 == CONV_WS || b.fc1 == CONV_WL) {
        _Float16* Q1 = reinterpret_cast<_Float16*>(n->Wq1.p);
        const long q1s = (long)hid * C * 2;
        if (!b.pfold)
            HIP_TRY(launch_pack_conv_frag(w1.buf.p, w1.pitch, hid, C, 0, f.sc1, w1.wabs, 1.f, f.slot(sb + 9), Q1, q1s, B, s, f.sh1,
                                          b1w.buf.p, n->bf1.p));
        MARK(ST_NORM1);
        ConvStripArgs k = strip_args(f, f.PAh, f.PAl, f.slot(sb + 4), C, hid, ACT_GELU);
        if (b.pfold) {
            k.Wraw = w1.buf.p; k.ldw = w1.pitch; k.wabs = w1.wabs; k.fa = f.sc1; k.fb = f.sh1; k.sfa = C;
            k.bias = b1w.buf.p; k.sbias = 0;
        } else {
            k.A = Q1; k.sA = q1s; k.aslot = f.slot(sb + 9);
            k.bias = n->bf1.p; k.sbias = hid;
        }
        k.cw = w1.winf; k.cb = b1w.absmax; k.cinb = f.slot(sb + 5);
        k.Chi = Uh; k.Clo = Ul; k.sCp = (long)hid * HW; k.cslot = f.slot(sb + 6);
        HIP_TRY(b.fc1 == CONV_WL ? launch_conv_wl(k, s) : launch_conv_ws(k, s));
    } else {
        HIP_TRY(launch_fold_affine_f16(w1.buf.p, w1.pitch, w1.wabs, f.sc1, f.sh1, b1w.buf.p, F1h, F1l, n->bf1.p, B, hid, C, cp, f1s,
                                       f.slot(sb + 9), s));
        MARK(ST_NORM1);
        PkOpts f1;
        f1.w = &w1; f1.fhi = F1h; f1.flo = F1l; f1.fslot = f.slot(sb + 9); f1.f_stride = f1s;
        f1.bias = n->bf1.p; f1.sbias = hid;
        f1.bhi = f.PAh; f1.blo = f.PAl; f1.cin = C; f1.in_slot = f.slot(sb + 4);
        f1.cout = hid; f1.act = act;
        f1.ohi = Uh; f1.olo = Ul; f1.cb = b1w.absmax; f1.cslot = f.slot(sb + 6); f1.cinb = f.slot(sb + 5);
        ACE_TRY(conv_packed(f, f1));
    }
    MARK(ST_MLP_FC1);

    if (b.fc2 == CONV_WS) {
        ConvStripArgs k = strip_args(f, Uh, Ul, f.slot(sb + 6), hid, C, ACT_NONE);
        static_frags(k, w2, b2w.buf.p);
        k.rsc = f.ra; k.rsh = f.rb; k.srs = C;
        if (b.res_planes) { k.Rhi = f.PBh; k.Rlo = f.PBl; k.sRp = (long)C * HW; k.rslot = f.hslot(i); }
        else { k.R = f.res; k.sR = actB; }
        if (b.out_f32) { k.Cf = f.hn; k.sCf = actB; }
        if (b.out_planes) {
            k.Chi = f.PBh; k.Clo = f.PBl; k.sCp = (long)C * HW; k.cslot = f.hslot(i + 1);
            k.cw = w2.winf; k.cb = b2w.absmax; k.rmax = f.slot(sb + 3);
            k.part = reinterpret_cast<float4*>(f.part_h); k.nstrips32 = b.out_nparts;
        } else {
            k.omax = f.hslot(i + 1);
        }
        HIP_TRY(launch_conv_ws(k, s));
    } else {
        PkOpts f2;
        f2.w = &w2; f2.bias = b2w.buf.p;
        f2.bhi = Uh; f2.blo = Ul; f2.cin = hid; f2.in_slot = f.slot(sb + 6);
        f2.out = f.hn; f2.cout = C; f2.act = ACT_NONE;
        f2.R = f.res; f2.r_bs = actB; f2.rsc = f.ra; f2.rsh = f.rb;
        if (b.out_planes) {
            f2.ohi = f.PBh; f2.olo = f.PBl; f2.cb = b2w.absmax; f2.cslot = f.hslot(i + 1); f2.rmax = f.slot(sb + 3);
            f2.part = f.part_h;
        } else {
            f2.omax = f.hslot(i + 1);
        }
        ACE_TRY(conv_packed(f, f2));
    }
    return ACE_OK;
}

static int enqueue_norm1(Fwd& f, int i, const BlockRoute& b, const float** a1, const float** b1, bool* planes) {
    const ace_sfno* n = f.n;
    const int C = n->C, sb = 16 + 12 * i, kind = n->cfg.normalization_layer;
    const std::string p = "blocks." + std::to_string(i) + ".";
    *a1 = *b1 = nullptr;
    *planes = false;
    if (kind == 0) return ACE_OK;
    if (kind == 2) {
        ACE_TRY(cond_norm(f, n->T.p, n->T.p, p + "norm1.", C, f.slot(sb + 5), b.n1_to_planes ? f.PAh : nullptr,
                          b.n1_to_planes ? f.Pl() : nullptr, false, planes));
    } else if (kind == 3) {
        HIP_TRY(launch_spatial_layer_norm(n->T.p, f.W(p + "norm1.weight"), f.W(p + "norm1.bias"), 1e-6f, (long)f.B * C, f.HW, n->T.p, f.slot(sb + 5), f.s));
    } else {
        HIP_TRY(launch_instnorm_stats(n->T.p, f.W(p + "norm1.weight"), f.W(p + "norm1.bias"), 1e-6f, f.B, C, f.HW, f.sc1, f.sh1, f.s,
                                      f.slot(sb + 5)));
        *a1 = f.sc1; *b1 = f.sh1;
    }
    MARK(ST_NORM1);
    return ACE_OK;
}

static int enqueue_packed_body(Fwd& f, int i, const BlockRoute& b) {
    const ace_sfno* n = f.n;
    const int C = n->C, hid = n->hid, act = n->cfg.activation_function, sb = 16 + 12 * i;
// ... 277 lines not shown
```

### ace_amd/csrc/fft.hip

```cpp
#include <hip/hip_runtime.h>

#include <cstdint>
#include <cstdlib>

#include "kernels.h"
#include "pack_frag.h"
#include "small_fft.h"
#include "strip_common.h"

namespace ace {
namespace {

#define FDEV __device__ __forceinline__

typedef float v2f __attribute__((ext_vector_type(2)));
typedef unsigned u32x4 __attribute__((ext_vector_type(4)));

FDEV v2f cmul(const v2f y, const v2f w) {
    const v2f t = v2f{y.x, y.x} * w;
    return v2f{y.y, y.y} * v2f{-w.y, w.x} + t;
}
FDEV auto wide_rsrc(const void* base) { return __builtin_amdgcn_make_buffer_rsrc(const_cast<void*>(base), 0, 0x7FFFFFFF, 0x00020000); }

using sfft::cdbl;
using sfft::kPi;
using sfft::unit_root;

template <int N>
struct RootTab {
    float re[N], im[N];
    constexpr explicit RootTab(double scale = 1.0) : re(), im() {
        for (int j = 0; j < N; ++j) {
            const cdbl w = unit_root(j, N);
            re[j] = (float)(scale * w.re);
            im[j] = (float)(scale * w.im);
        }
    }
};

template <int N1, int N2, bool INV>
struct alignas(16) TwTab {
    static constexpr int ROWS = INV ? N1 / 2 + 1 : N2, COLS = INV ? N2 : N1 / 2 + 1, CP = (COLS + 1) & ~1;
    float v[ROWS * CP * 2];
    constexpr TwTab() : v() {
        constexpr long W = (long)N1 * N2;
        for (int r = 0; r < ROWS; ++r)
            for (int c = 0; c < COLS; ++c) {
                const cdbl w = unit_root((long)r * c, W);
                const double scale = INV ? 1.0 : 2.0 * kPi / (double)W;
                v[2 * (r * CP + c)] = (float)(scale * w.re);
                v[2 * (r * CP + c) + 1] = (float)(scale * (INV ? -w.im : w.im));
            }
    }
};
template <int N1, int N2, bool INV>
__device__ constexpr TwTab<N1, N2, INV> kTw{};

#ifndef ACE_FFT_ABL
#define ACE_FFT_ABL 0
#endif
#ifndef ACE_FFT_ROWS
#define ACE_FFT_ROWS 16
#endif
constexpr int FFT_ROWS = ACE_FFT_ROWS;

template <int N2, int R>
struct ZPitch {
    static constexpr int raw = N2 * R;
    static constexpr int value = R >= 32 ? raw : raw + ((R - raw) % 32 + 32) % 32;
};


#ifndef ACE_FFT_XCD
#define ACE_FFT_XCD 1
#endif
#ifndef ACE_FFT_XCD_INV
#define ACE_FFT_XCD_INV 0
#endif
template <bool XCD>
FDEV void fft_unit(int& cblk, int& lat) {
    const int gx = (int)gridDim.x, id = (int)blockIdx.x + gx * (int)blockIdx.y, total = gx * (int)gridDim.y;
    int u = id;
    if (XCD && (total & 7) == 0) u = (id & 7) * (total >> 3) + (id >> 3);
    cblk = u % gx;
    lat = u / gx;
}
template <bool XCD>
FDEV bool fft_unit_ride(int nride, int& cblk, int& lat, int& rid) {
    const int gx = (int)gridDim.x, id = (int)blockIdx.x + gx * (int)blockIdx.y, total = gx * (int)gridDim.y;
    const int nextra = nride > 0 ? (nride + gx - 1) / gx * gx : 0;
    int u;
    if (XCD && (total & 7) == 0 && (nextra & 7) == 0) {
        const int xcd = id & 7, pos = id >> 3, nr8 = nextra >> 3;
        if (pos < nr8) { rid = pos * 8 + xcd; return true; }
        u = xcd * ((total >> 3) - nr8) + (pos - nr8);
    } else {
        if (id < nextra) { rid = id; return true; }
        u = id - nextra;
    }
    cblk = u % gx;
    lat = u / gx;
    return false;
}

#ifndef ACE_FFT_FWD_WAVES
#define ACE_FFT_FWD_WAVES 0
#endif
#ifndef ACE_FFT_FWD_PLN_WAVES
#define ACE_FFT_FWD_PLN_WAVES 7
#endif
#ifndef ACE_FFT_QROWS
#define ACE_FFT_QROWS 8
#endif
#ifndef ACE_FFT_INV_ROWS
#define ACE_FFT_INV_ROWS 32
#endif
#ifndef ACE_FFT_INV_WAVES
#define ACE_FFT_INV_WAVES 7
#endif
template <int N1, int N2, int R, bool PLN, bool FULLM>
__global__ __launch_bounds__(R * N2, N1 * N2 == 360 ? (PLN ? ACE_FFT_FWD_PLN_WAVES : ACE_FFT_FWD_WAVES) : (N1 * N2 == 1440 && R == 8 ? 4 : 0)) void dft_forward_fft_kernel(DftArgs p) {
    constexpr int W = N1 * N2, H1 = N1 / 2 + 1, NT = R * N2;
    constexpr int PITCH = W + 4;
    constexpr int K2N = N2 / 2 + 1;
    static_assert(N1 % 2 == 0 && N2 % 2 == 0 && N2 >= H1 && W % 4 == 0, "even factors, level 1 at least as wide as level 2");
    constexpr int ZP = ZPitch<N2, R>::value;
    constexpr int XS = R * PITCH, ZS = 2 * H1 * ZP;
    __shared__ __attribute__((aligned(16))) float smem[XS > ZS ? XS : ZS];
    float* xs = smem;
    v2f* Zs = reinterpret_cast<v2f*>(smem);

    const int tid = threadIdx.x;
    int cblk = 0, k = 0, rid = 0;
    if (fft_unit_ride<ACE_FFT_XCD != 0>(p.nride, cblk, k, rid)) {
        if (rid >= p.nride || blockIdx.z != 0) return;
        float* red = smem;
        for (int smp = 0; smp < p.ride.nsamples; ++smp) {
            if (smp) __syncthreads();
            pack_frag_block(p.ride, rid, smp, tid, red);
        }
        return;
    }
    const int c0 = cblk * R, b = blockIdx.z;
    const long HW = (long)p.H * W;
    constexpr int NPF = (R * (W / 4) + NT - 1) / NT;
    const int rlast = (p.C - c0 < R ? p.C - c0 : R) - 1;

    const int r1 = tid % R, b1 = tid / R;
    const int cr = c0 + (r1 < rlast ? r1 : rlast);
    float sc = 1.f, sh = 0.f;
    using Tw = TwTab<N1, N2, false>;
    float4 tw[Tw::CP / 2];
    constexpr bool TW_EARLY = Tw::CP / 2 <= 6;
    auto load_tw = [&]() {
        const float4* twp = reinterpret_cast<const float4*>(kTw<N1, N2, false>.v) + b1 * (Tw::CP / 2);
#pragma unroll
        for (int i = 0; i < Tw::CP / 2; ++i) tw[i] = twp[i];
    };
    auto load_affine = [&]() {
        sc = p.sc ? p.sc[(long)b * p.C + cr] : 1.f;
        sh = p.sc ? p.sh[(long)b * p.C + cr] : 0.f;
        if constexpr (TW_EARLY) load_tw();
    };
    if constexpr (PLN) {
        static_assert(R % 8 == 0, "whole k-groups");
        constexpr int NE = (R / 8) * W, NPE = (NE + NT - 1) / NT;
        const int kgmax = p.C / 8 - 1;
        const auto rsh = wide_rsrc(p.xhi + (long)b * p.sxp + (long)k * W * 8);
        const auto rsl = wide_rsrc(p.xlo + (long)b * p.sxp + (long)k * W * 8);
        u32x4 eh[NPE], el[NPE];
#pragma unroll
        for (int q = 0; q < NPE; ++q) {
            const int idx = tid + q * NT;
            if (idx < NE) {
                int kg = c0 / 8 + idx / W;
                kg = kg < kgmax ? kg : kgmax;
                const int off = (int)(((unsigned)kg * (unsigned)HW + (unsigned)(idx % W)) * 16u);
                eh[q] = __builtin_amdgcn_raw_buffer_load_b128(rsh, off, 0, 0);
                el[q] = __builtin_amdgcn_raw_buffer_load_b128(rsl, off, 0, 0);
            }
        }
        __builtin_amdgcn_sched_barrier(0);
        load_affine();
        sc *= ldexpf(1.0f, -pow2_exponent_for(wave_max_bits(slot_load(p.xslot + (tid & 63)))));
#pragma unroll
        for (int q = 0; q < NPE; ++q) {
            const int idx = tid + q * NT;
            if (idx < NE) {
                const half8 h8 = __builtin_bit_cast(half8, eh[q]), l8 = __builtin_bit_cast(half8, el[q]);
                float* d = xs + (8 * (idx / W)) * PITCH + idx % W;
#pragma unroll
                for (int e = 0; e < 8; ++e) d[e * PITCH] = (float)h8[e] + (float)l8[e];
            }
        }
    } else {
    const auto rsx = wide_rsrc(p.x + ((long)b * p.C + c0) * HW + (long)k * W);
    float4 pf[NPF];
#pragma unroll
    for (int q = 0; q < NPF; ++q) {
        const int idx = tid + q * NT;
        if (idx < R * (W / 4)) {
            const int r = idx / (W / 4), j = idx % (W / 4);
            const unsigned off = ((unsigned)(r < rlast ? r : rlast) * (unsigned)HW + 4u * j) * 4u;
#if ACE_FFT_ABL == 3
            pf[q] = make_float4(1.f + off, 2.f, 3.f, 4.f);
#else
            pf[q] = __builtin_bit_cast(float4, __builtin_amdgcn_raw_buffer_load_b128(rsx, (int)off, 0, 0));
#endif
        }
    }
    __builtin_amdgcn_sched_barrier(0);
    load_affine();
#pragma unroll
    for (int q = 0; q < NPF; ++q) {
        const int idx = tid + q * NT;
        if (idx < R * (W / 4)) {
            const int r = idx / (W / 4), j = idx % (W / 4);
            *reinterpret_cast<float4*>(xs + r * PITCH + 4 * j) = pf[q];
        }
    }
    }
    __syncthreads();

    const int kb = k * p.Bt + b;
    {
        float xv[N1];
#pragma unroll
        for (int a = 0; a < N1; ++a) xv[a] = fmaf(xs[r1 * PITCH + N2 * a + b1], sc, sh);
        if constexpr (!TW_EARLY) load_tw();
        __syncthreads();
        sfft::RFft<N1, v2f>::run([&](int a) { return xv[a]; }, [&](int k1, v2f y) {
            const v2f w = k1 % 2 ? v2f{tw[k1 / 2].z, tw[k1 / 2].w} : v2f{tw[k1 / 2].x, tw[k1 / 2].y};
            Zs[k1 * ZP + b1 * R + r1] = cmul(y, w);
        });
    }
    __syncthreads();

    float vmax = 0.f;
    {
        const int r = tid % R, k1 = tid / R;
        if (k1 < H1 && r <= rlast) {
            const long ms = (long)p.H * p.Bt * 2 * p.C;
            char* obase = reinterpret_cast<char*>(p.spec_out + (long)kb * 2 * p.C + c0);
            constexpr unsigned kDrop = 0xF0000000u;
            const unsigned od = (unsigned)(k1 * ms + r) * 4u, om = (unsigned)((N1 - k1) * ms + r) * 4u;
            const int imoff = p.C * 4;
            const bool has_mirror = k1 > 0 && k1 < N1 / 2;
            const v2f* zcol = Zs + k1 * ZP + r;
            sfft::CFft<N2, false, v2f>::run([&](int bb) { return zcol[bb * R]; }, [&](int q, v2f out) {
                const float mag = FULLM ? 0.f : fmaxf(fabsf(out.x), fabsf(out.y));
                if (FULLM) vmax = fmaxf(vmax, fmaxf(fabsf(out.x), fabsf(out.y)));
                if (q < K2N) {
                    const bool ok = k1 + N1 * q < p.Mm && (ACE_FFT_ABL != 1 || out.x == 1.2345e-30f);
                    const auto rs = wide_rsrc(obase + (long)q * N1 * ms * 4);
                    const int off = (int)(ok ? od : kDrop);
                    __builtin_amdgcn_raw_buffer_store_b32(__float_as_uint(out.x), rs, off, 0, 0);
                    __builtin_amdgcn_raw_buffer_store_b32(__float_as_uint(out.y), rs, off, imoff, 0);
                    if (!FULLM) vmax = fmaxf(vmax, ok ? mag : 0.f);
                }
                if (q >= N2 / 2) {
                    const bool ok = has_mirror && (N1 - k1) + N1 * (N2 - 1 - q) < p.Mm && (ACE_FFT_ABL != 1 || out.x == 1.2345e-30f);
                    const auto rs = wide_rsrc(obase + (long)(N2 - 1 - q) * N1 * ms * 4);
                    const int off = (int)(ok ? om : kDrop);
                    __builtin_amdgcn_raw_buffer_store_b32(__float_as_uint(out.x), rs, off, 0, 0);
                    __builtin_amdgcn_raw_buffer_store_b32(__float_as_uint(-out.y), rs, off, imoff, 0);
                    if (!FULLM) vmax = fmaxf(vmax, ok ? mag : 0.f);
                }
            });
        }
    }
    if (p.omax) {
#pragma unroll
        for (int off = 32; off > 0; off >>= 1) vmax = fmaxf(vmax, __shfl_xor(vmax, off, 64));
        __syncthreads();
        if ((tid & 63) == 0) smem[tid >> 6] = vmax;
        __syncthreads();
        if (tid == 0) {
            float m = 0.f;
            for (int w = 0; w < (NT + 63) / 64; ++w) m = fmaxf(m, smem[w]);
            atomicMax(p.omax + ((blockIdx.x + blockIdx.y) & 63), __float_as_uint(m));
        }
    }
}

template <int N1, int N2, int R = FFT_ROWS>
hipError_t launch_fwd(const DftArgs& a0, hipStream_t s) {
    DftArgs a = a0;
    const int gx = (a.C + R - 1) / R;
    if (a.nride > 0 && (R * N2 < 256 || !pack_frag_args_ok(a.ride) || a.nride != pack_frag_blocks(a.ride) || a.H + (a.nride + gx - 1) / gx > 65535)) a.nride = 0;
    if (a.rode) *a.rode = a.nride > 0;
    dim3 grid((unsigned)gx, (unsigned)(a.H + (a.nride > 0 ? (a.nride + gx - 1) / gx : 0)), (unsigned)a.Bt), block(R * N2);
    const bool full = a.Mm == a.W / 2 + 1;
    if (a.xhi) {
        if (!a.xlo || !a.xslot || a.C % 8 != 0) return hipErrorInvalidValue;
        if (full) hipLaunchKernelGGL((dft_forward_fft_kernel<N1, N2, R, true, true>), grid, block, 0, s, a);
        else hipLaunchKernelGGL((dft_forward_fft_kernel<N1, N2, R, true, false>), grid, block, 0, s, a);
    } else {
        if (full) hipLaunchKernelGGL((dft_forward_fft_kernel<N1, N2, R, false, true>), grid, block, 0, s, a);
        else hipLaunchKernelGGL((dft_forward_fft_kernel<N1, N2, R, false, false>), grid, block, 0, s, a);
    }
    return hipGetLastError();
}


template <int N1, int N2, int R, bool XCD>
__global__ __launch_bounds__(R * N2, N1 * N2 == 360 ? ACE_FFT_INV_WAVES : (N1 * N2 == 1440 && R == 8 ? 4 : 0)) void dft_inverse_fft_kernel(DftArgs p) {
    constexpr int W = N1 * N2, H1 = N1 / 2 + 1, NT = R * N2;
    constexpr int RP = R + 1;
    static_assert(N1 % 2 == 0 && N2 % 2 == 0 && N1 >= 4 && N2 >= H1 && W % 4 == 0 && R % 8 == 0, "even factors, whole row groups");
    constexpr int ZP = ZPitch<N2, R>::value;
    constexpr int YS = W * RP, US = 2 * H1 * ZP;
    __shared__ __attribute__((aligned(16))) float smem[YS > US ? YS : US];
    float* ys = smem;
    v2f* Us = reinterpret_cast<v2f*>(smem);

    const int tid = threadIdx.x;
    int cblk, k;
    fft_unit<XCD>(cblk, k);
    const int c0 = cblk * R, b = blockIdx.z;
    const int kb = k * p.Bt + b;
    const long HW = (long)p.H * W;
    const int rlast = (p.C - c0 < R ? p.C - c0 : R) - 1;
    const int crb = c0 + ((tid % R) < rlast ? (tid % R) : rlast);
    const float bias = p.bias ? p.bias[crb] : 0.f;

    {
        const int r = tid % R, k1 = tid / R;
        if (k1 < H1) {
            const int rr = r < rlast ? r : rlast;
            const long ms = (long)p.H * p.Bt * 2 * p.C;
            const char* sbase = reinterpret_cast<const char*>(p.spec + (long)kb * 2 * p.C + c0);
            constexpr unsigned kDrop = 0xF0000000u;
            const unsigned od = (unsigned)(k1 * ms + rr) * 4u, om = (unsigned)((N1 - k1) * ms + rr) * 4u;
            const int imoff = p.C * 4;
            v2f f[N2];
#pragma unroll
            for (int k2 = 0; k2 < N2; ++k2) {
                const bool mir = k2 > N2 / 2 || (k2 == N2 / 2 && k1 > 0);
                const int blk = k2 < N2 / 2 ? k2 : N2 - 1 - k2;
                const int m = (mir ? N1 - k1 : k1) + N1 * blk;
                if (k2 == N2 / 2) {
                    const auto rs0 = wide_rsrc(sbase + (long)(N2 / 2) * N1 * ms * 4);
                    const auto rs1 = wide_rsrc(sbase + (long)(N2 / 2 - 1) * N1 * ms * 4);
                    const int off0 = (int)((k1 == 0 && N1 * (N2 / 2) < p.Mm) ? od : kDrop);
                    const int off1 = (int)((k1 > 0 && m < p.Mm) ? om : kDrop);
                    const float re0 = __uint_as_float(__builtin_amdgcn_raw_buffer_load_b32(rs0, off0, 0, 0));
                    const float re1 = __uint_as_float(__builtin_amdgcn_raw_buffer_load_b32(rs1, off1, 0, 0));
                    const float im1 = __uint_as_float(__builtin_amdgcn_raw_buffer_load_b32(rs1, off1, imoff, 0));
                    f[k2] = v2f{re0 + re1, -im1};
                } else {
                    const auto rs = wide_rsrc(sbase + (long)blk * N1 * ms * 4);
                    const int off = (int)(m < p.Mm ? (mir ? om : od) : kDrop);
                    const float re = __uint_as_float(__builtin_amdgcn_raw_buffer_load_b32(rs, off, 0, 0));
                    const float im = __uint_as_float(__builtin_amdgcn_raw_buffer_load_b32(rs, off, imoff, 0));
                    f[k2] = v2f{re, mir ? -im : ((k2 == 0 && k1 == 0) ? 0.f : im)};
                }
            }
            using Tw = TwTab<N1, N2, true>;
            const float4* twp = reinterpret_cast<const float4*>(kTw<N1, N2, true>.v) + k1 * (Tw::CP / 2);
            sfft::CFft<N2, true, v2f>::run([&](int j) { return f[j]; }, [&](int j, v2f t) {
                const float4 w2 = twp[j / 2];
                Us[k1 * ZP + j * R + r] = cmul(t, j % 2 ? v2f{w2.z, w2.w} : v2f{w2.x, w2.y});
            });
        }
    }
    __syncthreads();

    {
        const int r = tid % R, b1 = tid / R;
        v2f u[H1];
#pragma unroll
        for (int k1 = 0; k1 < H1; ++k1) u[k1] = Us[k1 * ZP + b1 * R + r];
        __syncthreads();
        constexpr RootTab<N1> T1{};
        float* yr = ys + b1 * RP + r;
        float s0 = u[0].x + u[N1 / 2].x + bias, sh = u[0].x + ((N1 / 2) % 2 ? -u[N1 / 2].x : u[N1 / 2].x) + bias;
#pragma unroll
        for (int k1 = 1; k1 < N1 / 2; ++k1) {
            s0 += 2.f * u[k1].x;
            sh += (k1 % 2 ? -2.f : 2.f) * u[k1].x;
        }
        yr[0] = s0;
        yr[N2 * (N1 / 2) * RP] = sh;
#pragma unroll
        for (int a = 1; a < N1 / 2; ++a) {
            v2f pq = {u[0].x + (a % 2 ? -u[N1 / 2].x : u[N1 / 2].x) + bias, 0.f};
#pragma unroll
            for (int k1 = 1; k1 < N1 / 2; ++k1) {
                const int j = (k1 * a) % N1;
                pq += u[k1] * v2f{2.f * T1.re[j], 2.f * T1.im[j]};
            }
            yr[N2 * a * RP] = pq.x + pq.y;
            yr[N2 * (N1 - a) * RP] = pq.x - pq.y;
        }
    }
    __syncthreads();

    float vmax = 0.f;
    const auto rsy = wide_rsrc(p.y + ((long)b * p.C + c0) * HW + (long)k * W);
    constexpr int JG = (W / 4 + 7) / 8;
    for (int idx = tid; idx < JG * 8 * R; idx += NT) {
        const int j = (idx / (8 * R)) * 8 + (idx & 7), r = (idx >> 3) % R;
        if (r <= rlast && j < W / 4) {
            const float* src = ys + (4 * j) * RP + r;
            const float4 v = make_float4(src[0], src[RP], src[2 * RP], src[3 * RP]);
            __builtin_amdgcn_raw_buffer_store_b128(__builtin_bit_cast(u32x4, v), rsy, (int)(((unsigned)r * (unsigned)HW + 4u * j) * 4u), 0, 0);
            vmax = fmaxf(vmax, fmaxf(fmaxf(fabsf(v.x), fabsf(v.y)), fmaxf(fabsf(v.z), fabsf(v.w))));
        }
    }
    if (p.omax) {
#pragma unroll
        for (int off = 32; off > 0; off >>= 1) vmax = fmaxf(vmax, __shfl_xor(vmax, off, 64));
        __syncthreads();
        if ((tid & 63) == 0) smem[tid >> 6] = vmax;
        __syncthreads();
        if (tid == 0) {
            float m = 0.f;
            for (int w = 0; w < (NT + 63) / 64; ++w) m = fmaxf(m, smem[w]);
            atomicMax(p.omax + ((blockIdx.x + blockIdx.y) & 63), __float_as_uint(m));
        }
    }
}

template <int N1, int N2, int R = FFT_ROWS>
hipError_t launch_inv(const DftArgs& a, hipStream_t s) {
    dim3 grid((unsigned)((a.C + R - 1) / R), (unsigned)a.H, (unsigned)a.Bt), block(R * N2);
    constexpr bool XCD = ACE_FFT_XCD_INV != 0 || R * 4 < 128;
    hipLaunchKernelGGL((dft_inverse_fft_kernel<N1, N2, R, XCD>), grid, block, 0, s, a);
    return hipGetLastError();
}

bool lane_offsets_fit(const DftArgs& a) {
    const double plane = (double)a.H * a.Bt * 2.0 * a.C * 4.0, rows = 33.0 * (double)a.H * a.W * 4.0;
    return 42.0 * plane < 2147483647.0 && rows < 2147483647.0;
}

}

bool launch_dft_forward_fft(const DftArgs& a, hipStream_t s, hipError_t* err) {
    if (a.no_fft || (!a.xhi && (reinterpret_cast<uintptr_t>(a.x) & 15) != 0) || a.Mm > a.W / 2 + 1 || a.H > 65535 || a.Bt > 65535 || !lane_offsets_fit(a))
        return false;
    switch (a.W) {
        case 360: *err = launch_fwd<20, 18>(a, s); return true;
        case 1440: *err = launch_fwd<40, 36, ACE_FFT_QROWS>(a, s); return true;
        case 720: *err = launch_fwd<30, 24, 8>(a, s); return true;
        case 48: *err = launch_fwd<8, 6>(a, s); return true;
        case 24: *err = launch_fwd<6, 4>(a, s); return true;
        case 16: *err = launch_fwd<4, 4>(a, s); return true;
        default: return false;
    }
}

bool dft_fft_has_width(int W) { return W == 360 || W == 1440 || W == 720 || W == 48 || W == 24 || W == 16; }

bool launch_dft_inverse_fft(const DftArgs& a, hipStream_t s, hipError_t* err) {
    if (a.no_fft || (reinterpret_cast<uintptr_t>(a.y) & 15) != 0 || a.Mm > a.W / 2 + 1 || a.H > 65535 || a.Bt > 65535 || !lane_offsets_fit(a))
        return false;
    switch (a.W) {
        case 360: *err = launch_inv<20, 18, ACE_FFT_INV_ROWS>(a, s); return true;
        case 1440: *err = launch_inv<40, 36, ACE_FFT_QROWS>(a, s); return true;
        case 720: *err = launch_inv<30, 24, 8>(a, s); return true;
        case 48: *err = launch_inv<8, 6>(a, s); return true;
        case 24: *err = launch_inv<6, 4>(a, s); return true;
        case 16: *err = launch_inv<4, 4>(a, s); return true;
        default: return false;
    }
}

}
```

### ace_amd/csrc/kernels.h

```cpp
#pragma once
#include "tuning_guard.h"

#include <hip/hip_runtime.h>

#include <vector>

namespace ace {

struct Switches {
    bool no_fft = false;
    bool no_strip = false;
    bool no_fold = false;
    bool no_dhconv_strip = false;
    bool no_pk = false;
    bool no_pk_sht = false;
    bool no_enc_ws = false;
    bool no_enc_pk = false;
    bool no_cln_mfma = false;
    bool no_cln_planes = false;
    int conv_ws_roles = 7;
    bool conv_wl = true;
    bool fused_pack = true;
    bool planes_stream = true;
    bool dense_grouped_filter = false;
};
Switches read_switches();

enum Act { ACT_NONE = 0, ACT_GELU = 1, ACT_RELU = 2, ACT_SILU = 3, ACT_GELU_FAST = 4  };
enum Tri {
    TRI_NONE = 0,
    TRI_ROWS_GE_BATCH = 1,
    TRI_K_GE_BATCH = 2,
    TRI_ROWS_LE_BATCH = 3
};

struct GemmArgs {
    const float* A = nullptr; long lda = 0; long sA = 0;
    const float* B = nullptr; long ldb = 0; long sB = 0;
    const float* B2 = nullptr; long ldb2 = 0; long sB2 = 0; int K1 = -1;
    const long* brow = nullptr;
    const float* bsc = nullptr; const float* bsh = nullptr; long sbs = 0;
    float* C = nullptr; long ldc = 0; long sC = 0;
    const float* bias = nullptr; long sbias = 0;
    int a_kpad = 0;
    const float* R = nullptr; long ldr = 0; long sR = 0;
    const float* rsc = nullptr; const float* rsh = nullptr; long srs = 0;
    const float* osc = nullptr; const float* osh = nullptr;
    int M = 0, N = 0, K = 0, nbatch = 1;
    int tri = TRI_NONE; int trimul = 1;
    int act = ACT_NONE;
    float cap = __builtin_inff();
    unsigned* omax = nullptr;
};
hipError_t launch_gemm(const GemmArgs& a, hipStream_t s);

bool gemm_f16x3_eligible(const GemmArgs& g);
constexpr int AMAX_SHARDS = 64;
hipError_t launch_gemm_f16x3(const GemmArgs& g, const void* Ahi, const void* Alo, float ascale, float bscale,
                             hipStream_t s, const unsigned* bmax = nullptr, unsigned* omax = nullptr,
                             const unsigned* bmax2 = nullptr);
hipError_t launch_gemm_f16x3_planes(const GemmArgs& g, const void* Ahi, const void* Alo, float ascale, const unsigned* bmax,
                                    void* Chi, void* Clo, float cw, unsigned* cslot, hipStream_t s);
hipError_t launch_gemm_f16x3_adyn(const GemmArgs& g, const void* Bhi, const void* Blo, long ldn, long sB_halves,
                                  float bscale_static, const unsigned* amax, unsigned* omax, hipStream_t s);
hipError_t launch_pack_dhconv_f16(const float* w, void* hi, void* lo, int Cin, int Cout, int L, float scale, hipStream_t s);
hipError_t launch_csfno_weight_to_dense(const float* w, float* dense, int C, int G, int L, hipStream_t s);
hipError_t launch_pack_dhconv_f16c(const float* w, void* hi, void* lo, int Cin, int Cout, int L, float scale, hipStream_t s);
hipError_t launch_zero_u32(unsigned* p, long n, hipStream_t s);
hipError_t launch_spatial_layer_norm(const float* x, const float* gamma, const float* beta, float eps, long planes, long HW, float* y,
                                     unsigned* omax, hipStream_t s);
hipError_t launch_absmax(const float* x, long n, unsigned* omax, hipStream_t s);
hipError_t launch_split_f16(const float* src, long lds, void* hi, void* lo, long ldd, long rows, int cols, float scale,
                            hipStream_t s);

struct Gemm4Args {
    const _Float16* Ahi = nullptr; const _Float16* Alo = nullptr; long lda = 0; long sA = 0;
    const _Float16* Bhi = nullptr; const _Float16* Blo = nullptr; long ldn = 0; long sB = 0;
    int a_tiled = 0;
    int cplx = 0;
    int tile = 0;
    float ascale = 1.f, bscale = 1.f;
    const unsigned* amax = nullptr;
    const unsigned* bmax = nullptr;
    float* C = nullptr; long ldc = 0; long sC = 0;
    _Float16* Chi = nullptr; _Float16* Clo = nullptr; long ldnc = 0; long sCp = 0;
    float cw = 0.f, cb = 0.f;
    unsigned* cslot = nullptr;
    const unsigned* cinb = nullptr;
    const unsigned* rmax = nullptr;
    float4* part = nullptr;
    unsigned* omax = nullptr;
    const float* bias = nullptr; long sbias = 0;
    const float* R = nullptr; long ldr = 0; long sR = 0;
    const float* rsc = nullptr; const float* rsh = nullptr; long srs = 0;
    int M = 0, N = 0, K = 0, nbatch = 1;
    int tri = TRI_NONE; int trimul = 1;
    int act = ACT_NONE;
    int impl_k = 0, impl_cg8 = 0, impl_pitch = 0, impl_dil = 1;
    float cap = 3.0e38f;
};
hipError_t launch_gemm_f16x3_packed(const Gemm4Args& a, hipStream_t s);
int gemm4_strips(int M, int N);
hipError_t launch_split_f16_tiled(const float* src, long lds_, void* hi, void* lo, long ldd, long rows, int cols,
                                  float scale, hipStream_t s);
hipError_t launch_pack_pformat(const float* src, long ldb, long sSrc, int K, int N, int nbatch, const float* sc,
                               const float* sh, long sbs, const unsigned* slot, void* hi, void* lo, long ldn, long sPl,
                               hipStream_t s);

struct LegStripArgs {
    const float* B = nullptr;
    long b_kstride = 0, b_moff = 0;
    const _Float16* A = nullptr;
    const int* tile_off = nullptr;
    float ascale = 1.f;
    const unsigned* bmax = nullptr;
    float* C = nullptr; _Float16* Chi = nullptr; _Float16* Clo = nullptr;
    long c_rstride = 0, c_moff = 0;
    float cw = 0.f; unsigned* cslot = nullptr;
    unsigned* omax = nullptr;
    int N = 0;
    int K = 0;
    int R = 0;
    int nbatch = 0;
    int mode = 0;
};
constexpr int LEG_STRIP_SLACK_ROWS = 16;
bool legendre_strip_eligible(const LegStripArgs& a);
hipError_t launch_legendre_strip(const LegStripArgs& a, hipStream_t s);
bool legendre_fold_eligible(const LegStripArgs& a);
bool legendre_fold_is_big(const LegStripArgs& a);
hipError_t launch_legendre_fold(const LegStripArgs& a, hipStream_t s);

hipError_t launch_pack_conv_frag(const float* W, long ldw, int O, int I, int order, const float* a, float wmax,
                                 float scale_static, unsigned* wslot, void* dst, long sDst, int nsamples, hipStream_t s,
                                 const float* b = nullptr, const float* bias = nullptr, float* bf = nullptr);

struct ConvStripArgs {
    const _Float16* Xhi = nullptr; const _Float16* Xlo = nullptr; long ldn = 0; long sX = 0;
    const unsigned* xslot = nullptr;
    const _Float16* A = nullptr; long sA = 0;
    const unsigned* aslot = nullptr; float ascale = 1.f;
    const float* Wraw = nullptr; long ldw = 0; float wabs = 0.f;
    const float* fa = nullptr; const float* fb = nullptr; long sfa = 0;
    const float* bias = nullptr; long sbias = 0;
    const float* R = nullptr; long sR = 0;
    const _Float16* Rhi = nullptr; const _Float16* Rlo = nullptr; long sRp = 0; const unsigned* rslot = nullptr;
    float cw = 0.f, cb = 0.f; const unsigned* cinb = nullptr; const unsigned* rmax = nullptr;
    _Float16* Chi = nullptr; _Float16* Clo = nullptr; long sCp = 0; unsigned* cslot = nullptr;
    float4* part = nullptr; int nstrips32 = 0;
    int C = 0, M = 0, HW = 0, nbatch = 1, act = ACT_NONE;
    float* Cf = nullptr; long sCf = 0;
    const float* rsc = nullptr; const float* rsh = nullptr; long srs = 0;
    unsigned* omax = nullptr;
};
bool conv_ws_eligible(int K, int M, long HW, int role, int roles_on = 7);
hipError_t launch_conv_ws(const ConvStripArgs& a, hipStream_t s);
int conv_ws_stat_parts(const ConvStripArgs& a);
bool conv_wl_eligible(int K, int M, long HW);
hipError_t launch_conv_wl(const ConvStripArgs& a, hipStream_t s);

struct DhconvStripArgs {
    const _Float16* Dhi = nullptr; const _Float16* Dlo = nullptr; long sD = 0;
    const unsigned* amax = nullptr;
    const _Float16* Whi = nullptr; const _Float16* Wlo = nullptr; long sW = 0;
    float bscale = 1.f;
    float* E = nullptr; long sE = 0;
    unsigned* omax = nullptr;
    int C = 0, L = 0, Mrows = 0, trimul = 1;
    int groups = 1;
    const int* units = nullptr; int units_per_xcd = 0;
    int kstore = 0;
};
bool dhconv_native_groups_ok(int C, int groups);
hipError_t launch_pack_dhconv_f16g(const float* w_grouped, void* hi, void* lo, int C, int G, int L, float scale, hipStream_t s);
bool dhconv_strip_eligible(const DhconvStripArgs& a);
int dhconv_build_units(int L, int Mrows, int trimul, int C, std::vector<int>& out);
hipError_t launch_dhconv_strip(const DhconvStripArgs& a, hipStream_t s);

struct PackFragArgs {
    const float* W = nullptr; long ldw = 0; int O = 0, I = 0, order = 0;
    const float* a = nullptr; float wmax = 0.f, scale_static = 1.f; unsigned* wslot = nullptr;
    _Float16* dst = nullptr; long sDst = 0;
    const float* b = nullptr; const float* bias = nullptr; float* bf = nullptr;
    int nsamples = 1;
};
inline int pack_frag_blocks(const PackFragArgs& q) { return (q.O / 32) * (q.I / 16) + (q.bf ? q.O / 32 : 0); }

bool pack_frag_args_ok(const PackFragArgs& q);

struct DftArgs {
    const float* x = nullptr;
    const _Float16* xhi = nullptr; const _Float16* xlo = nullptr; long sxp = 0; const unsigned* xslot = nullptr;
    float* y = nullptr;
    const float* spec = nullptr;
    float* spec_out = nullptr;
    const float* tc = nullptr; const float* ts = nullptr; int ldt = 0;
    const float* sc = nullptr; const float* sh = nullptr;
    const float* bias = nullptr;
    int Bt = 1, C = 0, H = 0, W = 0, Mm = 0;
    unsigned* omax = nullptr;
    bool no_fft = false;
    PackFragArgs ride; int nride = 0; bool* rode = nullptr;
};
hipError_t launch_dft_forward(const DftArgs& a, hipStream_t s);
hipError_t launch_dft_inverse(const DftArgs& a, hipStream_t s);
bool launch_dft_forward_fft(const DftArgs& a, hipStream_t s, hipError_t* err);
bool launch_dft_inverse_fft(const DftArgs& a, hipStream_t s, hipError_t* err);
bool dft_fft_has_width(int W);

struct ClnMfmaArgs {
    const float* x = nullptr; float* y = nullptr; long sx = 0;
    const float* cond = nullptr; long scond = 0; int J = 0;
    const unsigned* cslot = nullptr;
    const _Float16* As = nullptr; const _Float16* Ab = nullptr; float ascale_s = 1.f, ascale_b = 1.f;
    const float* gamma = nullptr; const float* beta = nullptr;
    float eps = 1e-5f; int C = 0; long HW = 0; int nbatch = 1;
    unsigned* omax = nullptr;
    _Float16* Phi = nullptr; _Float16* Plo = nullptr; long sP = 0;
    float gmax = 1.f, bmax = 0.f;
    float ws_inf = 0.f, wb_inf = 0.f;
};
bool cln_mfma_eligible(const ClnMfmaArgs& a);
bool cln_mfma_planes_ok(const ClnMfmaArgs& a);
hipError_t launch_cln_mfma(const ClnMfmaArgs& a, hipStream_t s);

hipError_t launch_instnorm_stats(const float* x, const float* gamma, const float* beta, float eps, int Bt, int C,
                                 long HW, float* scale, float* shift, hipStream_t s, unsigned* omax = nullptr);

hipError_t launch_instnorm_finalize(const float4* part, int nparts, int Bt, int C, long HW, const float* gamma,
                                    const float* beta, float eps, float* scale, float* shift, unsigned* omax,
                                    hipStream_t s);
hipError_t launch_fold_affine_f16(const float* W, long ldw, float wmax, const float* a, const float* b, const float* bias,
                                  void* hi, void* lo, float* bf, int nsamples, int O, int I, long ldd, long sPl,
                                  unsigned* wslot, hipStream_t s);

hipError_t launch_cond_layer_norm(const float* x, const float* noise, const float* gamma, const float* beta,
                                  const float* ws, const float* wb, float eps, float* stats, float* y, int Bt, int C,
                                  int J, long HW, hipStream_t s, unsigned* omax = nullptr);

hipError_t launch_spec_to_ref(const float* D, float* out, int Bt, int C, int L, int Mm, hipStream_t s);
hipError_t launch_ref_to_spec(const float* in, float* E, int Bt, int C, int L, int Mm, hipStream_t s, unsigned* omax = nullptr, bool triangular_consumer = false);

hipError_t launch_contract_diagonal(const float* D, const float* w, float* E, int Bt, int Cin, int Cout, int L, int Mm,
                                    hipStream_t s, unsigned* omax = nullptr);

hipError_t launch_expand_dhconv_weight(const float* w, float* wx, int Cin, int Cout, int L, hipStream_t s);

hipError_t launch_rowaffine_add(const float* x, const float* sc, const float* sh, const float* r, const float* rsc,
                                const float* rsh, float* y, long rows, long n, hipStream_t s);

hipError_t launch_pack_normalize(const float* const* srcs, const long* strides, const float* mean, const float* stdv,
                                 float* dst, int Bt, int nch, long HW, hipStream_t s);
hipError_t launch_unpack_denormalize(const float* src, const float* mean, const float* stdv, float* const* dsts,
                                     const long* strides, int Bt, int nch, long HW, hipStream_t s);

}
```

### ace_amd/csrc/strip_fold.hip

```cpp
#include <hip/hip_runtime.h>

#include <cstdint>
#include <cstdlib>
#include <type_traits>

#include "kernels.h"
#include "strip_pack.h"

namespace ace {
namespace {

#define FDEV __device__ __forceinline__

typedef _Float16 half8 __attribute__((ext_vector_type(8)));
typedef float f32x16 __attribute__((ext_vector_type(16)));
typedef float f32x4 __attribute__((ext_vector_type(4)));
typedef unsigned u32x4 __attribute__((ext_vector_type(4)));
typedef unsigned u32x2 __attribute__((ext_vector_type(2)));
typedef __attribute__((address_space(3))) char* lds_cptr;

constexpr int NH_MAX = FOLD_NKP_SMALL / 2;
constexpr int NH_BIG = FOLD_NKP_BIG / 2;
constexpr int FNSLOT = 3;
constexpr int FTS_BYTES = 2048;
constexpr int fold_lds_bytes(int nh) { return FNSLOT * 2 * nh * 2048 + 4 * FTS_BYTES; }
constexpr int FLDS_BYTES = fold_lds_bytes(NH_MAX);

FDEV unsigned slot_load(const unsigned* p) { return __hip_atomic_load(p, __ATOMIC_RELAXED, __HIP_MEMORY_SCOPE_AGENT); }
FDEV int pow2_exponent_for(float mx) {
    int e = 0;
    if (mx > 0.f && mx < 3.0e38f) { (void)frexpf(mx, &e); e = 12 - e; }
    return e > 100 ? 100 : (e < -100 ? -100 : e);
}
FDEV float wave_max_bits(unsigned raw) {
    float mx = __uint_as_float(raw);
#pragma unroll
    for (int off = 32; off > 0; off >>= 1) mx = fmaxf(mx, __shfl_xor(mx, off, 64));
    return __uint_as_float(__builtin_amdgcn_readfirstlane(__float_as_uint(mx)));
}
FDEV void glds16(const void* gsrc, const char* lds_dst_uniform) {
    const unsigned addr = __builtin_amdgcn_readfirstlane((unsigned)(size_t)(lds_cptr)lds_dst_uniform);
    asm volatile("s_mov_b32 m0, %1\n\ts_nop 0\n\tglobal_load_lds_dwordx4 %0, off"
                 :
                 : "v"(gsrc), "s"(addr)
                 : "memory", "m0");
}
FDEV int acc_row(int r, int h) { return (r & 3) + 8 * (r >> 2) + 4 * h; }

struct RowMap { int rbase, rstep, vlo, vhi; };

template <int NH, int OUT, bool FULLN, int MODE>
FDEV void fold_body(const LegStripArgs& p, char* smem, const int m, const int grp, const FoldGeom gm) {
    constexpr int NKP = 2 * NH;
    constexpr int FSLOT_BYTES = NKP * 2048;
    constexpr bool BIG = NH > NH_MAX;
    const int tid = threadIdx.x;
    const int lane = tid & 63;
    const int wave = __builtin_amdgcn_readfirstlane(tid >> 6);
    const int i = lane & 31, g = lane >> 5;
    const int N = p.N, K = p.K, R = p.R;
    const int H = MODE == 0 ? K : R;
    const int n0 = grp * 128 + wave * 32;
    const int n = n0 + i;
    const int nc = n < N ? n : N - 1;
    char* ring = smem;
    char* Ts = smem + FNSLOT * FSLOT_BYTES + wave * FTS_BYTES;
    const int nunits = 2 * gm.npairs;

    const unsigned raw_b = slot_load(p.bmax + lane);

    const _Float16* Am = p.A + (long)p.tile_off[m] * 1024;
    auto issue_unit = [&](int u) {
        const int uu = u < nunits ? u : nunits - 1;
        const _Float16* src = Am + (long)uu * NKP * 1024 + lane * 8;
        const char* dst = ring + (u % FNSLOT) * FSLOT_BYTES;
#pragma unroll
        for (int c = 0; c < NH; ++c) {
            const int pc = wave + 4 * c;
            glds16(src + pc * 512, dst + pc * 1024);
        }
    };
    if (nunits > 0) { issue_unit(0); issue_unit(1); }

    const long ks = p.b_kstride;
    float bbound = wave_max_bits(raw_b);
    if (MODE == 0) bbound *= 2.f;
    const int eb = pow2_exponent_for(bbound);
    const float bscale = ldexpf(1.0f, eb), inv_b = ldexpf(1.0f, -eb);
    half8 bh[2][NKP], bl[2][NKP];
#define ACE_FOLD_SPLIT(x, H_, L_) do { const float x_ = (x); const _Float16 h_ = (_Float16)x_; (H_) = h_; (L_) = (_Float16)(x_ - (float)h_); } while (0)
    if constexpr (MODE == 0) {
        const float* Xm = p.B + (long)m * p.b_moff;
        const long rowb = ks * 4;
        const auto rsD = __builtin_amdgcn_make_buffer_rsrc(const_cast<float*>(Xm), 0, (unsigned)((long)gm.Hh * rowb), 0x00020000);
        const auto rsM = __builtin_amdgcn_make_buffer_rsrc(const_cast<float*>(Xm + (long)gm.Hh * ks), 0, (unsigned)((long)(H - gm.Hh) * rowb), 0x00020000);
        unsigned vd[8], vm[8];
#pragma unroll
        for (int e = 0; e < 8; ++e) {
            vd[e] = (unsigned)(((long)(8 * g + e) * ks + nc) * 4);
            vm[e] = (unsigned)(((long)(H - 1 - gm.Hh - (8 * g + e)) * ks + nc) * 4);
        }
        constexpr int CHK = BIG ? 4 : NKP;
#pragma unroll
        for (int j0 = 0; j0 < NKP; j0 += CHK) {
            float ra[CHK][8], rb[CHK][8];
#pragma unroll
            for (int jc = 0; jc < CHK; ++jc) {
                const unsigned so = (unsigned)((long)(16 * (j0 + jc)) * rowb);
#pragma unroll
                for (int e = 0; e < 8; ++e) {
                    ra[jc][e] = __uint_as_float(__builtin_amdgcn_raw_buffer_load_b32(rsD, vd[e] + so, 0, 0));
                    rb[jc][e] = __uint_as_float(__builtin_amdgcn_raw_buffer_load_b32(rsM, vm[e] - so, 0, 0));
                }
            }
#pragma unroll
            for (int jc = 0; jc < CHK; ++jc)
#pragma unroll
                for (int e = 0; e < 8; ++e) {
                    const float a = ra[jc][e] * bscale, b = rb[jc][e] * bscale;
                    ACE_FOLD_SPLIT(a + b, bh[0][j0 + jc][e], bl[0][j0 + jc][e]);
                    ACE_FOLD_SPLIT(a - b, bh[1][j0 + jc][e], bl[1][j0 + jc][e]);
                }
            if (BIG) __builtin_amdgcn_sched_barrier(0);
        }
    } else {
        const float* Em = p.B + (long)m * p.b_moff;
        const long rowb = ks * 4;
        const long span = ((long)(K - 1) * ks + N) * 4;
        const auto rsE = __builtin_amdgcn_make_buffer_rsrc(const_cast<float*>(Em), 0, (unsigned)(span > 0 ? span : 0), 0x00020000);
        unsigned ve[8];
#pragma unroll
        for (int e = 0; e < 8; ++e) ve[e] = (unsigned)(((long)(m + 2 * (8 * g + e)) * ks + nc) * 4);
        constexpr int CHK = BIG ? 2 : NKP;
#pragma unroll
        for (int j0 = 0; j0 < NKP; j0 += CHK) {
            float r0[CHK][8], r1[CHK][8];
#pragma unroll
            for (int jc = 0; jc < CHK; ++jc) {
                const unsigned so = (unsigned)((long)(32 * (j0 + jc)) * rowb);
#pragma unroll
                for (int e = 0; e < 8; ++e) {
                    r0[jc][e] = __uint_as_float(__builtin_amdgcn_raw_buffer_load_b32(rsE, ve[e] + so, 0, 0));
                    r1[jc][e] = __uint_as_float(__builtin_amdgcn_raw_buffer_load_b32(rsE, ve[e] + so + (unsigned)rowb, 0, 0));
                }
            }
#pragma unroll
            for (int jc = 0; jc < CHK; ++jc)
#pragma unroll
                for (int e = 0; e < 8; ++e) {
                    ACE_FOLD_SPLIT(r0[jc][e] * bscale, bh[0][j0 + jc][e], bl[0][j0 + jc][e]);
                    ACE_FOLD_SPLIT(r1[jc][e] * bscale, bh[1][j0 + jc][e], bl[1][j0 + jc][e]);
                }
            if (BIG) __builtin_amdgcn_sched_barrier(0);
        }
    }

    const float inv_a = 1.0f / p.ascale;
    float oscale = inv_a * inv_b;
    if (OUT == 1) {
        const float cbound = p.cw * wave_max_bits(raw_b);
        oscale *= ldexpf(1.0f, pow2_exponent_for(cbound));
        if (tid == 0) atomicMax(p.cslot + (blockIdx.x & 63), __float_as_uint(cbound));
    }

    float vmax = 0.f;
    const long cm = (long)m * p.c_moff;
    auto tile_max = [&](const RowMap rm, const f32x16& acc, auto inner_tag) {
        constexpr bool NOMASK = decltype(inner_tag)::value && FULLN;
#pragma unroll
        for (int r = 0; r < 16; ++r) {
            const int row = rm.rbase + rm.rstep * acc_row(r, g);
            const bool ok = NOMASK || (row >= rm.vlo && row < rm.vhi && n < N);
            vmax = fmaxf(vmax, ok ? fabsf(acc[r] * oscale) : 0.f);
        }
    };
    auto store_tile = [&](const RowMap rm, const f32x16& acc, auto inner_tag) {
        constexpr bool NOMASK = decltype(inner_tag)::value && FULLN;
        if (OUT == 2) {
#pragma unroll
            for (int r = 0; r < 16; ++r) {
                const int row = rm.rbase + rm.rstep * acc_row(r, g);
                const float v = acc[r] * oscale;
                if (row >= rm.vlo && row < rm.vhi && n < N) p.C[cm + (long)row * p.c_rstride + n] = v;
            }
            return;
        }
        unsigned* T32 = reinterpret_cast<unsigned*>(Ts);
        const int c4 = (lane & 7) * 4;
        const int ncol = n0 + c4;
#pragma unroll
        for (int hf = 0; hf < 2; ++hf) {
#pragma unroll
            for (int r8 = 0; r8 < 8; ++r8) {
                const int r = 8 * hf + r8;
                const float v = acc[r] * oscale;
                unsigned w;
                if (OUT == 1) {
                    const _Float16 h = (_Float16)v;
                    const _Float16 l = (_Float16)(v - (float)h);
                    w = (unsigned)__builtin_bit_cast(unsigned short, h) | ((unsigned)__builtin_bit_cast(unsigned short, l) << 16);
                } else {
                    w = __float_as_uint(v);
                }
                T32[(acc_row(r, g) - 16 * hf) * 32 + i] = w;
            }
#pragma unroll
            for (int ps = 0; ps < 2; ++ps) {
                const int rl = ps * 8 + (lane >> 3);
                const int row = rm.rbase + rm.rstep * (16 * hf + rl);
                const u32x4 d = *reinterpret_cast<const u32x4*>(T32 + rl * 32 + c4);
                const bool ok = NOMASK || (row >= rm.vlo && row < rm.vhi && ncol < N);
                if (OUT == 1) {
                    u32x2 hi2, lo2;
                    hi2[0] = (d[0] & 0xffffu) | (d[1] << 16);
                    hi2[1] = (d[2] & 0xffffu) | (d[3] << 16);
                    lo2[0] = (d[0] >> 16) | (d[1] & 0xffff0000u);
                    lo2[1] = (d[2] >> 16) | (d[3] & 0xffff0000u);
                    if (ok) {
                        const long off = cm + (long)row * p.c_rstride + ncol;
                        *reinterpret_cast<u32x2*>(p.Chi + off) = hi2;
                        *reinterpret_cast<u32x2*>(p.Clo + off) = lo2;
                    }
                } else {
                    if (ok) {
                        f32x4 v;
                        v[0] = __uint_as_float(d[0]); v[1] = __uint_as_float(d[1]);
                        v[2] = __uint_as_float(d[2]); v[3] = __uint_as_float(d[3]);
                        *reinterpret_cast<f32x4*>(p.C + cm + (long)row * p.c_rstride + ncol) = v;
                    }
                }
            }
        }
    };
    auto fwd_map = [&](int tp, int par) { return RowMap{m + par + 64 * tp, 2, 0, R}; };
    auto north_map = [&](int tp) { return RowMap{32 * tp, 1, 0, gm.Hh}; };
    auto south_map = [&](int tp) { return RowMap{H - 1 - 32 * tp, -1, gm.Hh, H}; };

    auto unit = [&](int u, auto par_tag, auto&& under) -> f32x16 {
        constexpr int PAR = decltype(par_tag)::value;
        if (u == 0) asm volatile("s_waitcnt vmcnt(0)" ::: "memory");
        else asm volatile("s_waitcnt vmcnt(%0)" ::"n"(NH) : "memory");
        __syncthreads();
        issue_unit(u + 2);
        under();
        const char* slot = ring + (u % FNSLOT) * FSLOT_BYTES + lane * 16;
        f32x16 a0, a1, a2;
#pragma unroll
        for (int r = 0; r < 16; ++r) { a0[r] = 0.f; a1[r] = 0.f; a2[r] = 0.f; }
        (void)a1;
        constexpr int FG = BIG ? (MODE == 1 ? 1 : 2) : NKP;
        half8 fh[2][FG], fl[2][FG];
#pragma unroll
        for (int q = 0; q < FG; ++q) {
            fh[0][q] = *reinterpret_cast<const half8*>(slot + q * 2048);
            fl[0][q] = *reinterpret_cast<const half8*>(slot + q * 2048 + 1024);
        }
#pragma unroll
        for (int g0 = 0; g0 < NKP; g0 += FG) {
            constexpr int dummy = 0; (void)dummy;
            const int cur = (g0 / FG) & 1;
            if (g0 + FG < NKP) {
#pragma unroll
                for (int q = 0; q < FG; ++q) {
                    fh[cur ^ 1][q] = *reinterpret_cast<const half8*>(slot + (g0 + FG + q) * 2048);
                    fl[cur ^ 1][q] = *reinterpret_cast<const half8*>(slot + (g0 + FG + q) * 2048 + 1024);
                }
            }
#pragma unroll
            for (int q = 0; q < FG; ++q) {
                if constexpr (BIG) {
                    a0 = __builtin_amdgcn_mfma_f32_32x32x16_f16(fl[cur][q], bh[PAR][g0 + q], a0, 0, 0, 0);
                    a2 = __builtin_amdgcn_mfma_f32_32x32x16_f16(fh[cur][q], bh[PAR][g0 + q], a2, 0, 0, 0);
                    a0 = __builtin_amdgcn_mfma_f32_32x32x16_f16(fh[cur][q], bl[PAR][g0 + q], a0, 0, 0, 0);
                } else {
                    a0 = __builtin_amdgcn_mfma_f32_32x32x16_f16(fl[cur][q], bh[PAR][g0 + q], a0, 0, 0, 0);
                    a1 = __builtin_amdgcn_mfma_f32_32x32x16_f16(fh[cur][q], bl[PAR][g0 + q], a1, 0, 0, 0);
                    a2 = __builtin_amdgcn_mfma_f32_32x32x16_f16(fh[cur][q], bh[PAR][g0 + q], a2, 0, 0, 0);
                }
            }
        }
        if constexpr (BIG) return a0 + a2;
        else return (a0 + a1) + a2;
    };
    using T0 = std::integral_constant<int, 0>;
    using T1 = std::integral_constant<int, 1>;

    f32x16 pa, pb;
#pragma unroll
    for (int r = 0; r < 16; ++r) { pa[r] = 0.f; pb[r] = 0.f; }
    if constexpr (MODE == 0) {
        for (int tp = 0; tp < gm.npairs; ++tp) {
            const f32x16 ev = unit(2 * tp, T0{}, [&] {
                if (tp > 0) {
                    if (OUT != 1) tile_max(fwd_map(tp - 1, 1), pb, std::true_type{});
                    store_tile(fwd_map(tp - 1, 1), pb, std::true_type{});
                }
            });
            const bool last = tp + 1 == gm.npairs;
            pb = unit(2 * tp + 1, T1{}, [&] {
                if (!last) {
                    if (OUT != 1) tile_max(fwd_map(tp, 0), ev, std::true_type{});
                    store_tile(fwd_map(tp, 0), ev, std::true_type{});
                }
            });
            if (last) pa = ev;
        }
    } else if constexpr (BIG) {
        for (int tp = 0; tp < gm.npairs; ++tp) {
            const f32x16 ev = unit(2 * tp, T0{}, [] {});
            const f32x16 od = unit(2 * tp + 1, T1{}, [] {});
            f32x16 t = ev + od;
            const bool inner = tp + 1 < gm.npairs;
            if (inner) { tile_max(north_map(tp), t, std::true_type{}); store_tile(north_map(tp), t, std::true_type{}); }
            else { tile_max(north_map(tp), t, std::false_type{}); store_tile(north_map(tp), t, std::false_type{}); }
            __builtin_amdgcn_sched_barrier(0);
            t = ev - od;
            if (inner) { tile_max(south_map(tp), t, std::true_type{}); store_tile(south_map(tp), t, std::true_type{}); }
            else { tile_max(south_map(tp), t, std::false_type{}); store_tile(south_map(tp), t, std::false_type{}); }
            __builtin_amdgcn_sched_barrier(0);
        }
    } else {
        for (int tp = 0; tp < gm.npairs; ++tp) {
            const f32x16 ev = unit(2 * tp, T0{}, [&] {
                if (tp > 0) {
                    tile_max(north_map(tp - 1), pa, std::true_type{});
                    store_tile(north_map(tp - 1), pa, std::true_type{});
                }
            });
            const f32x16 od = unit(2 * tp + 1, T1{}, [&] {
                if (tp > 0) {
                    tile_max(south_map(tp - 1), pb, std::true_type{});
                    store_tile(south_map(tp - 1), pb, std::true_type{});
                }
            });
            pa = ev + od;
            pb = ev - od;
        }
    }
    asm volatile("s_waitcnt vmcnt(0)" ::: "memory");
    constexpr bool STORED_IN_LOOP = BIG && MODE == 1;
    const int tl = gm.npairs - 1;
    const RowMap ma = MODE == 0 ? fwd_map(tl, 0) : north_map(tl), mb = MODE == 0 ? fwd_map(tl, 1) : south_map(tl);
    if (OUT != 1 && gm.npairs > 0 && !STORED_IN_LOOP) {
        tile_max(ma, pa, std::false_type{});
        tile_max(mb, pb, std::false_type{});
    }
    if (OUT != 1 && p.omax) {
#pragma unroll
        for (int off = 32; off > 0; off >>= 1) vmax = fmaxf(vmax, __shfl_xor(vmax, off, 64));
        float* red = reinterpret_cast<float*>(smem);
        __syncthreads();
        if (lane == 0) red[wave] = vmax;
        __syncthreads();
        if (tid == 0) atomicMax(p.omax + (blockIdx.x & 63), __float_as_uint(fmaxf(fmaxf(red[0], red[1]), fmaxf(red[2], red[3]))));
        __syncthreads();
    }
    if (gm.npairs > 0 && !STORED_IN_LOOP) {
        store_tile(ma, pa, std::false_type{});
        store_tile(mb, pb, std::false_type{});
    }
}

#ifdef ACE_LF_TRACE
__device__ unsigned long long lf_wg_span[2][4096][5];
#endif

template <int OUT, bool FULLN, int MODE>
__global__ __launch_bounds__(256, 2) void legendre_fold_kernel(LegStripArgs p, int G) {
    __shared__ __attribute__((aligned(16))) char smem[FLDS_BYTES];
#ifdef ACE_LF_TRACE
    const unsigned long long lf_t0 = __builtin_amdgcn_s_memtime();
#endif
    const int xcd = blockIdx.x & 7, idx = blockIdx.x >> 3;
    const int m = (idx / G) * 8 + xcd;
    const int grp = idx % G;
    if (m >= p.nbatch) return;
    const FoldGeom gm = fold_geom(MODE, m, p.R, p.K);
    switch (gm.nkp2) {
        case 2: fold_body<1, OUT, FULLN, MODE>(p, smem, m, grp, gm); break;
        case 4: fold_body<2, OUT, FULLN, MODE>(p, smem, m, grp, gm); break;
        case 6: fold_body<3, OUT, FULLN, MODE>(p, smem, m, grp, gm); break;
        default: break;
    }
#ifdef ACE_LF_TRACE
    if (threadIdx.x == 0 && blockIdx.x < 4096) {
        unsigned xcc, hwid;
        asm volatile("s_getreg_b32 %0, hwreg(HW_REG_XCC_ID)" : "=s"(xcc));
        asm volatile("s_getreg_b32 %0, hwreg(HW_REG_HW_ID)" : "=s"(hwid));
        unsigned long long* e = lf_wg_span[MODE][blockIdx.x];
        e[0] = lf_t0; e[1] = __builtin_amdgcn_s_memtime(); e[2] = (unsigned long long)m; e[3] = hwid; e[4] = xcc & 0xf;
    }
#endif
}

template <int OUT, int MODE>
__global__ __launch_bounds__(256, 1) void legendre_fold_big_kernel(LegStripArgs p, int G) {
    extern __shared__ __attribute__((aligned(16))) char smem_big[];
    const int xcd = blockIdx.x & 7, idx = blockIdx.x >> 3;
    const int m = (idx / G) * 8 + xcd;
    const int grp = idx % G;
    if (m >= p.nbatch) return;
    const FoldGeom gm = fold_geom(MODE, m, p.R, p.K);
    switch (gm.nkp2) {
        case 12: fold_body<6, OUT, true, MODE>(p, smem_big, m, grp, gm); break;
        case 18: fold_body<9, OUT, true, MODE>(p, smem_big, m, grp, gm); break;
        case 24: fold_body<12, OUT, true, MODE>(p, smem_big, m, grp, gm); break;
        default:
            if constexpr (MODE == 1) {
                switch (gm.nkp2) {
                    case 2: fold_body<1, OUT, true, MODE>(p, smem_big, m, grp, gm); break;
                    case 4: fold_body<2, OUT, true, MODE>(p, smem_big, m, grp, gm); break;
                    case 6: fold_body<3, OUT, true, MODE>(p, smem_big, m, grp, gm); break;
                    default: break;
                }
            }
            break;
    }
}

}

#ifdef ACE_LF_TRACE
extern "C" int ace_debug_lf_spans(void* dst) { return (int)hipMemcpyFromSymbol(dst, HIP_SYMBOL(lf_wg_span), sizeof(lf_wg_span)); }
#endif

bool legendre_fold_eligible(const LegStripArgs& a) {
    if (a.K < 1 || a.R < 1 || a.N < 1 || a.nbatch < 1 || (a.mode != 0 && a.mode != 1)) return false;
    const FoldGeom g0 = fold_geom(a.mode, 0, a.R, a.K);
    if (g0.nkp2 > 2 * NH_BIG) return false;
    if (!a.A || !a.tile_off || !a.B || !a.bmax) return false;
    if (g0.nkp2 > 2 * NH_MAX) {
        const bool vec = a.N % 4 == 0 && a.c_rstride % 4 == 0 && a.c_moff % 4 == 0;
        if (a.N % 128 != 0 || !vec || (!a.Chi && (reinterpret_cast<uintptr_t>(a.C) & 15) != 0)) return false;
    }
    const double rowb = (double)a.b_kstride * 4.0;
    if (a.mode == 0 ? ((double)a.K + 2.0 * (16.0 * FOLD_NKP_BIG + 64.0)) * rowb >= 4.0e9 : ((double)a.K + 256.0) * rowb >= 4.0e9) return false;
    if (a.Chi) return a.mode == 0 && a.N % 4 == 0 && a.c_rstride % 4 == 0 && a.c_moff % 4 == 0 && a.cslot &&
                      (reinterpret_cast<uintptr_t>(a.Chi) & 7) == 0 && (reinterpret_cast<uintptr_t>(a.Clo) & 7) == 0;
    return a.C != nullptr;
}

bool legendre_fold_is_big(const LegStripArgs& a) { return fold_geom(a.mode, 0, a.R, a.K).nkp2 > 2 * NH_MAX; }

template <int MODE>
static hipError_t launch_fold_mode(const LegStripArgs& a, hipStream_t s) {
    const int G = (a.N + 127) / 128;
    const int mgroups = (a.nbatch + 7) / 8;
    dim3 grid((unsigned)(mgroups * 8 * G)), block(256);
    const bool fulln = a.N % 128 == 0;
    if (a.Chi) {
        if (fulln) hipLaunchKernelGGL((legendre_fold_kernel<1, true, MODE>), grid, block, 0, s, a, G);
        else hipLaunchKernelGGL((legendre_fold_kernel<1, false, MODE>), grid, block, 0, s, a, G);
    } else {
        const bool vec = a.N % 4 == 0 && a.c_rstride % 4 == 0 && a.c_moff % 4 == 0 && (reinterpret_cast<uintptr_t>(a.C) & 15) == 0;
        if (vec && fulln) hipLaunchKernelGGL((legendre_fold_kernel<0, true, MODE>), grid, block, 0, s, a, G);
        else if (vec) hipLaunchKernelGGL((legendre_fold_kernel<0, false, MODE>), grid, block, 0, s, a, G);
        else hipLaunchKernelGGL((legendre_fold_kernel<2, false, MODE>), grid, block, 0, s, a, G);
    }
    return hipGetLastError();
}

template <int OUT, int MODE>
static hipError_t launch_fold_big(const LegStripArgs& a, int nh, hipStream_t s) {
    const int G = a.N / 128;
    const int mgroups = (a.nbatch + 7) / 8;
    const int lds = fold_lds_bytes(nh);
    static bool configured = false;
    if (!configured) {
        const hipError_t e = hipFuncSetAttribute(reinterpret_cast<const void*>(legendre_fold_big_kernel<OUT, MODE>),
                                                 hipFuncAttributeMaxDynamicSharedMemorySize, fold_lds_bytes(NH_BIG));
        if (e != hipSuccess) return e;
        configured = true;
    }
    hipLaunchKernelGGL((legendre_fold_big_kernel<OUT, MODE>), dim3((unsigned)(mgroups * 8 * G)), dim3(256), (size_t)lds, s, a, G);
    return hipGetLastError();
}

hipError_t launch_legendre_fold(const LegStripArgs& a, hipStream_t s) {
    const FoldGeom g0 = fold_geom(a.mode, 0, a.R, a.K);
    if (legendre_fold_is_big(a)) {
        const int nh = g0.nkp2 / 2;
        if (a.mode == 0) return a.Chi ? launch_fold_big<1, 0>(a, nh, s) : launch_fold_big<0, 0>(a, nh, s);
        return launch_fold_big<0, 1>(a, nh, s);
    }
    return a.mode == 0 ? launch_fold_mode<0>(a, s) : launch_fold_mode<1>(a, s);
}

}
```

### ace_amd/csrc/strip_pack.h

```cpp
#pragma once
#include <cmath>
#include <cstdint>
#include <cstring>
#include <vector>

namespace ace {

struct StripGeom {
    int row0;
    int ntiles;
    int j0;
    int nks;
    int nks4;
    int klo;
};

#if defined(__HIPCC__)
__host__ __device__
#endif
inline StripGeom strip_geom(int mode, int m, int R, int K) {
    StripGeom g;
    if (mode == 0) {
        g.row0 = (m / 32) * 32;
        g.ntiles = (R - g.row0 + 31) / 32;
        g.j0 = 0;
        g.nks = (K + 15) / 16;
        g.klo = 0;
    } else {
        g.row0 = 0;
        g.ntiles = (R + 31) / 32;
        g.j0 = m / 16;
        g.nks = (K + 15) / 16 - g.j0;
        g.klo = m;
    }
    if (g.ntiles < 0) g.ntiles = 0;
    if (g.nks < 0) g.nks = 0;
    g.nks4 = g.nks > 0 ? (g.nks + 3) & ~3 : 4;
    return g;
}

inline uint16_t f32_to_f16_bits(float f) {
    uint32_t x;
    std::memcpy(&x, &f, 4);
    const uint32_t sign = (x >> 16) & 0x8000u;
    const uint32_t em = x & 0x7fffffffu;
    if (em >= 0x7f800000u) return (uint16_t)(sign | 0x7c00u | ((em > 0x7f800000u) ? 0x200u : 0u));
    if (em >= 0x477ff000u) return (uint16_t)(sign | 0x7c00u);
    if (em < 0x33000001u) return (uint16_t)sign;
    int e = (int)(em >> 23) - 127;
    uint32_t man = (em & 0x7fffffu) | 0x800000u;
    int shift;
    uint32_t base;
    if (e >= -14) { shift = 13; base = (uint32_t)(e + 15) << 10; man &= 0x7fffffu; }
    else { shift = 13 + (-14 - e); base = 0; }
    uint32_t q = man >> shift;
    const uint32_t rem = man & ((1u << shift) - 1u), half = 1u << (shift - 1);
    if (rem > half || (rem == half && (q & 1u))) ++q;
    return (uint16_t)(sign | (base + q));
}
inline float f16_bits_to_f32(uint16_t h) {
    const uint32_t sign = (uint32_t)(h & 0x8000u) << 16;
    const uint32_t e = (h >> 10) & 0x1fu, man = h & 0x3ffu;
    float v;
    if (e == 0) v = std::ldexp((float)man, -24);
    else if (e == 31) v = man ? NAN : INFINITY;
    else v = std::ldexp((float)(man | 0x400u), (int)e - 25);
    uint32_t b;
    std::memcpy(&b, &v, 4);
    b |= sign;
    std::memcpy(&v, &b, 4);
    return v;
}

struct StripPack {
    std::vector<uint16_t> frags;
    std::vector<int> tile_off;
    long blocks = 0;
};

inline void pack_legendre_strip(const float* tab, int mmax, int nrows, int ncols, int pitch, int mode, float scale,
                                StripPack& out) {
    out.tile_off.assign((size_t)mmax, 0);
    long blocks = 0;
    for (int m = 0; m < mmax; ++m) {
        const StripGeom g = strip_geom(mode, m, nrows, ncols);
        out.tile_off[m] = (int)blocks;
        blocks += (long)g.ntiles * g.nks4;
    }
    out.blocks = blocks;
    out.frags.assign((size_t)blocks * 1024, 0);
    for (int m = 0; m < mmax; ++m) {
        const StripGeom g = strip_geom(mode, m, nrows, ncols);
        for (int t = 0; t < g.ntiles; ++t)
            for (int jj = 0; jj < g.nks; ++jj) {
                uint16_t* blk = out.frags.data() + ((size_t)out.tile_off[m] + (size_t)t * g.nks4 + jj) * 1024;
                for (int lane = 0; lane < 64; ++lane) {
                    const int i = lane & 31, gg = lane >> 5;
                    const int row = g.row0 + 32 * t + i;
                    for (int e = 0; e < 8; ++e) {
                        const int col = 16 * (g.j0 + jj) + 8 * gg + e;
                        float v = 0.f;
                        const bool ok = row < nrows && col < ncols && (mode == 0 ? row >= m : col >= m);
                        if (ok) v = tab[((size_t)m * nrows + row) * pitch + col] * scale;
                        const uint16_t hi = f32_to_f16_bits(v);
                        const uint16_t lo = f32_to_f16_bits(v - f16_bits_to_f32(hi));
                        blk[lane * 8 + e] = hi;
                        blk[512 + lane * 8 + e] = lo;
                    }
                }
            }
    }
}

struct FoldGeom {
    int Hh;
    int nkp;
    int nkp2;
    int npairs;
};
#if defined(__HIPCC__)
__host__ __device__
#endif
inline int fold_round_nkp(int nkp) {
    if (nkp <= 6) return nkp > 0 ? (nkp + 1) & ~1 : 2;
    return ((nkp + 5) / 6) * 6;
}
constexpr int FOLD_NKP_SMALL = 6, FOLD_NKP_BIG = 24;

#if defined(__HIPCC__)
__host__ __device__
#endif
inline FoldGeom fold_geom(int mode, int m, int R, int K) {
    FoldGeom g;
    int n16;
    if (mode == 0) {
        g.Hh = (K + 1) / 2;
        n16 = g.Hh;
        const int nr0 = (R - m + 1) / 2;
        g.npairs = nr0 > 0 ? (nr0 + 31) / 32 : 0;
    } else {
        g.Hh = (R + 1) / 2;
        n16 = (K - m + 1) / 2;
        if (n16 < 0) n16 = 0;
        g.npairs = (g.Hh + 31) / 32;
    }
    g.nkp = (n16 + 15) / 16;
    g.nkp2 = fold_round_nkp(g.nkp);
    return g;
}

inline double fold_symmetry_error(const float* tab, int mmax, int nlat, int lmax, int pitch, int mode) {
    double worst = 0.0, mx = 0.0;
    for (int m = 0; m < mmax; ++m)
        for (int l = m; l < lmax; ++l) {
            const double s = ((l - m) & 1) ? -1.0 : 1.0;
            for (int k = 0; k < nlat; ++k) {
                const double a = mode == 0 ? tab[((size_t)m * lmax + l) * pitch + k] : tab[((size_t)m * nlat + k) * pitch + l];
                const double b = mode == 0 ? tab[((size_t)m * lmax + l) * pitch + (nlat - 1 - k)] : tab[((size_t)m * nlat + (nlat - 1 - k)) * pitch + l];
                worst = std::fmax(worst, std::fabs(b - s * a));
                mx = std::fmax(mx, std::fabs(a));
            }
        }
    return mx > 0.0 ? worst / mx : 0.0;
}

inline void pack_legendre_fold(const float* tab, int mmax, int nlat, int lmax, int pitch, int mode, float scale, StripPack& out) {
    const int R = mode == 0 ? lmax : nlat, K = mode == 0 ? nlat : lmax;
    out.tile_off.assign((size_t)mmax, 0);
    long blocks = 0;
    for (int m = 0; m < mmax; ++m) {
        const FoldGeom g = fold_geom(mode, m, R, K);
        out.tile_off[m] = (int)blocks;
        blocks += (long)g.npairs * 2 * g.nkp2;
    }
    out.blocks = blocks;
    out.frags.assign((size_t)blocks * 1024, 0);
    for (int m = 0; m < mmax; ++m) {
        const FoldGeom g = fold_geom(mode, m, R, K);
        for (int u = 0; u < 2 * g.npairs; ++u) {
            const int tp = u >> 1, p = u & 1;
            for (int jj = 0; jj < g.nkp; ++jj) {
                uint16_t* blk = out.frags.data() + ((size_t)out.tile_off[m] + (size_t)u * g.nkp2 + jj) * 1024;
                for (int lane = 0; lane < 64; ++lane) {
                    const int i = lane & 31, gg = lane >> 5;
                    for (int e = 0; e < 8; ++e) {
                        const int c = 16 * jj + 8 * gg + e;
                        const int kf = mode == 0 ? c : 32 * tp + i;
                        const int l = m + p + 2 * (mode == 0 ? 32 * tp + i : c);
                        float v = 0.f;
                        if (kf < g.Hh && l < lmax) {
                            const int km = nlat - 1 - kf;
                            const double s = p ? -1.0 : 1.0;
                            const double a = mode == 0 ? tab[((size_t)m * lmax + l) * pitch + kf] : tab[((size_t)m * nlat + kf) * pitch + l];
                            const double b = mode == 0 ? tab[((size_t)m * lmax + l) * pitch + km] : tab[((size_t)m * nlat + km) * pitch + l];
                            v = (float)((km == kf ? a : 0.5 * (a + s * b)) * (double)scale);
                        }
                        const uint16_t hi = f32_to_f16_bits(v);
                        const uint16_t lo = f32_to_f16_bits(v - f16_bits_to_f32(hi));
                        blk[lane * 8 + e] = hi;
                        blk[512 + lane * 8 + e] = lo;
                    }
                }
            }
        }
    }
}

inline float cln_frag_scale(float wabs) {
    int e = 0;
    if (wabs > 0.f && std::isfinite(wabs)) { (void)std::frexp(wabs, &e); e = 10 - e; }
    return std::ldexp(1.0f, e);
}
inline size_t cln_frag_halves(int C, int J) { return (size_t)(C / 32) * (size_t)((J + 15) / 16) * 1024; }
inline void pack_cln_frags(const float* W, int C, int J, float scale, uint16_t* out) {
    const int nk = (J + 15) / 16;
    for (int rt = 0; rt < C / 32; ++rt)
        for (int ks = 0; ks < nk; ++ks) {
            uint16_t* blk = out + ((size_t)rt * nk + ks) * 1024;
            for (int lane = 0; lane < 64; ++lane)
                for (int e = 0; e < 8; ++e) {
                    const int row = 32 * rt + (lane & 31), j = 16 * ks + 8 * (lane >> 5) + e;
                    const float v = j < J ? W[(size_t)row * J + j] * scale : 0.f;
                    const uint16_t hi = f32_to_f16_bits(v);
                    blk[lane * 8 + e] = hi;
                    blk[512 + lane * 8 + e] = f32_to_f16_bits(v - f16_bits_to_f32(hi));
                }
        }
}

}
```

Measured before the change: 187.3 steps/s.

## Skip polar-dead Legendre rows and truncate DFT modes per latitude

Scans the packed fold Legendre tables at plan build to find, for each order m, the first latitude whose weights are not zero in fp16 (r0), and from that, for each latitude, the highest useful m (mcut). The forward DFT and inverse DFT stop at mcut, the fold kernels start at r0, and when the table is small enough the forward weights are repacked without the leading dead K blocks. This removes multiply-adds against associated Legendre values that underflow near the poles. The cost is extra plan-time scanning, dry-run route probes on every call, and a poison option for debugging uninitialised spectral rows.

```diff
diff --git a/ace_amd/csrc/capi.hip b/ace_amd/csrc/capi.hip
--- a/ace_amd/csrc/capi.hip
+++ b/ace_amd/csrc/capi.hip
@@ -46,6 +46,8 @@
     sw.no_strip = on("ACE_NO_STRIP");
     sw.no_fold = on("ACE_NO_FOLD");
     sw.no_dhconv_strip = on("ACE_NO_DHCONV_STRIP");
+    sw.no_polar_cut = on("ACE_NO_POLAR_CUT");
+    sw.polar_poison = on("ACE_POLAR_POISON");
 #ifdef ACE_MEASUREMENT_SWITCHES
     sw.no_pk = on("ACE_NO_PK");
     sw.no_pk_sht = on("ACE_NO_PK_SHT");
@@ -96,6 +98,12 @@
         return e;
     }
     hipError_t ensure(size_t count) { return count <= n ? hipSuccess : alloc(count); }
+    hipError_t alloc_x(size_t count, bool poison) {
+        hipError_t e = alloc(count);
+        if (e == hipSuccess && poison && count) e = hipMemsetD32(reinterpret_cast<hipDeviceptr_t>(p), 0x7fc00000, count);
+        return e;
+    }
+    hipError_t ensure_x(size_t count, bool poison) { return count <= n ? hipSuccess : alloc_x(count, poison); }
     hipError_t upload(const std::vector<float>& h) {
         hipError_t e = alloc(h.size(), false);
         if (e != hipSuccess) return e;
@@ -116,6 +124,9 @@
     bool strip = false;
     DevBuf wt_ffrag, pt_ffrag, wt_foff, pt_foff;
     bool fold = false;
+    DevBuf cut_r0, cut_mcut;
+    bool cut = false, kdrop = false;
+    double cut_share = 0.0;
     DevBuf slots;
     Switches sw;
     mutable int route[2] = {-1, -1};
@@ -180,11 +191,30 @@
         if ((t.nlat + 1) / 2 <= 16 * FOLD_NKP_BIG && (t.lmax + 1) / 2 <= 16 * FOLD_NKP_BIG && !p->sw.no_fold &&
             fold_symmetry_error(t.wt.data(), t.mmax, t.nlat, t.lmax, t.Hp, 0) < 2e-6 &&
             fold_symmetry_error(t.pt.data(), t.mmax, t.nlat, t.lmax, t.Lp, 1) < 2e-6) {
-            StripPack sp;
+            StripPack sp, spi;
             pack_legendre_fold(t.wt.data(), t.mmax, t.nlat, t.lmax, t.Hp, 0, p->wt_scale, sp);
+            pack_legendre_fold(t.pt.data(), t.mmax, t.nlat, t.lmax, t.Lp, 1, p->pt_scale, spi);
+            if (!p->sw.no_polar_cut) {
+                const PolarCut pc = derive_polar_cut(sp, spi, t.mmax, t.nlat, t.lmax);
+                if (pc.ok && pc.dead_share > 0.0) {
+                    auto upi = [](const std::vector<int>& v, DevBuf& d) -> hipError_t {
+                        const hipError_t e = d.alloc(v.size(), false);
+                        return e != hipSuccess ? e : hipMemcpy(d.p, v.data(), v.size() * sizeof(int), hipMemcpyHostToDevice);
+                    };
+                    HIP_TRY(upi(pc.r0, p->cut_r0));
+                    HIP_TRY(upi(pc.mcut, p->cut_mcut));
+                    p->cut = true;
+                    p->cut_share = pc.dead_share;
+                    if (fold_geom(0, 0, t.lmax, t.nlat).nkp2 <= FOLD_NKP_SMALL) {
+                        std::vector<int> kskip(pc.r0.size());
+                        for (size_t m = 0; m < kskip.size(); ++m) kskip[m] = pc.r0[m] / 16;
+                        pack_legendre_fold(t.wt.data(), t.mmax, t.nlat, t.lmax, t.Hp, 0, p->wt_scale, sp, kskip.data());
+                        p->kdrop = true;
+                    }
+                }
+            }
             HIP_TRY(up(sp, p->wt_ffrag, p->wt_foff));
-            pack_legendre_fold(t.pt.data(), t.mmax, t.nlat, t.lmax, t.Lp, 1, p->pt_scale, sp);
-            HIP_TRY(up(sp, p->pt_ffrag, p->pt_foff));
+            HIP_TRY(up(spi, p->pt_ffrag, p->pt_foff));
             p->fold = true;
         }
     }
@@ -195,8 +225,9 @@
 static int run_dft_forward(const ace_sht_plan& pl, const float* x, const float* sc, const float* sh, float* X, int Bt,
                            int C, hipStream_t s, unsigned* xmax = nullptr, const _Float16* xhi = nullptr,
                            const _Float16* xlo = nullptr, long sxp = 0, const unsigned* xslot = nullptr,
-                           const PackFragArgs* ride = nullptr, bool* rode = nullptr) {
+                           const PackFragArgs* ride = nullptr, bool* rode = nullptr, const int* mcut = nullptr) {
     DftArgs a;
+    a.mcut = mcut;
     if (rode) *rode = false;
     if (ride && rode) { a.ride = *ride; a.nride = pack_frag_blocks(*ride); a.rode = rode; }
     a.omax = xmax;
@@ -206,17 +237,22 @@
     HIP_TRY(launch_dft_forward(a, s));
     return ACE_OK;
 }
-static int run_dft_inverse(const ace_sht_plan& pl, const float* X, const float* bias, float* y, int Bt, int C,
-                           hipStream_t s, unsigned* ymax = nullptr) {
+static DftArgs dft_inverse_args(const ace_sht_plan& pl, const float* X, const float* bias, float* y, int Bt, int C, unsigned* ymax) {
     DftArgs a;
     a.omax = ymax;
     a.spec = X; a.y = y; a.tc = pl.gc.p; a.ts = pl.gs.p; a.ldt = pl.Kfp; a.bias = bias;
     a.Bt = Bt; a.C = C; a.H = pl.nlat; a.W = pl.nlon; a.Mm = pl.mmax; a.no_fft = pl.sw.no_fft;
+    return a;
+}
+static int run_dft_inverse(const ace_sht_plan& pl, const float* X, const float* bias, float* y, int Bt, int C,
+                           hipStream_t s, unsigned* ymax = nullptr, const int* mcut = nullptr) {
+    DftArgs a = dft_inverse_args(pl, X, bias, y, Bt, C, ymax);
+    a.mcut = mcut;
     HIP_TRY(launch_dft_inverse(a, s));
     return ACE_OK;
 }
 static int run_legendre_forward(const ace_sht_plan& pl, const float* X, float* D, long N2, hipStream_t s,
-                                const unsigned* xmax = nullptr, unsigned* dmax = nullptr, bool planes = false) {
+                                const unsigned* xmax = nullptr, unsigned* dmax = nullptr, bool planes = false, bool dry = false) {
     GemmArgs g;
     g.omax = planes ? nullptr : dmax;
     g.A = pl.wt.p; g.lda = pl.Hp; g.sA = (long)pl.lmax * pl.Hp;
@@ -241,19 +277,21 @@
         if (pl.fold && !pl.sw.no_fold) {
             LegStripArgs f = a;
             f.A = reinterpret_cast<const _Float16*>(pl.wt_ffrag.p); f.tile_off = reinterpret_cast<const int*>(pl.wt_foff.p);
+            if (pl.cut) { f.r0 = reinterpret_cast<const int*>(pl.cut_r0.p); f.kdrop = pl.kdrop; }
             if (legendre_fold_eligible(f)) {
-                HIP_TRY(launch_legendre_fold(f, s));
+                if (!dry) HIP_TRY(launch_legendre_fold(f, s));
                 pl.route[0] = fold_route(f);
                 return ACE_OK;
             }
         }
         if (pl.strip && legendre_strip_eligible(a)) {
-            HIP_TRY(launch_legendre_strip(a, s));
+            if (!dry) HIP_TRY(launch_legendre_strip(a, s));
             pl.route[0] = 1;
             return ACE_OK;
         }
     }
     pl.route[0] = 0;
+    if (dry) return ACE_OK;
     if (planes) {
         if (!(pl.f16 && xmax && dmax && gemm_f16x3_eligible(g))) return fail(ACE_ERR_STATE, "legendre planes path not eligible");
         _Float16* Dh = reinterpret_cast<_Float16*>(D);
@@ -269,7 +307,7 @@
     return ACE_OK;
 }
 static int run_legendre_inverse(const ace_sht_plan& pl, const float* E, float* X, long N2, hipStream_t s,
-                                const unsigned* emax = nullptr, bool dry = false) {
+                                const unsigned* emax = nullptr, bool dry = false, bool skip_dead = false) {
     GemmArgs g;
     g.A = pl.pt.p; g.lda = pl.Lp; g.sA = (long)pl.nlat * pl.Lp;
     g.B = E; g.ldb = (long)pl.mmax * N2; g.sB = N2;
@@ -286,6 +324,7 @@
         if (pl.fold && !pl.sw.no_fold) {
             LegStripArgs f = a;
             f.A = reinterpret_cast<const _Float16*>(pl.pt_ffrag.p); f.tile_off = reinterpret_cast<const int*>(pl.pt_foff.p);
+            if (pl.cut && skip_dead) f.r0 = reinterpret_cast<const int*>(pl.cut_r0.p);
             if (legendre_fold_eligible(f)) {
                 if (!dry) HIP_TRY(launch_legendre_fold(f, s));
                 pl.route[1] = fold_route(f);
@@ -306,6 +345,29 @@
     }
     HIP_TRY(launch_gemm(g, s));
     return ACE_OK;
+}
+
+static const int* forward_pair_mcut(const ace_sht_plan& pl, const float* X, float* D, long N2, const unsigned* xmax, unsigned* dmax,
+                                    bool planes) {
+    if (!pl.cut) return nullptr;
+    const int before = pl.route[0];
+    const int rc = run_legendre_forward(pl, X, D, N2, nullptr, xmax, dmax, planes, true);
+    const bool folded = rc == ACE_OK && pl.route[0] >= 2;
+    pl.route[0] = before;
+    return folded ? reinterpret_cast<const int*>(pl.cut_mcut.p) : nullptr;
+}
+struct InversePair { bool skip_dead = false; const int* mcut = nullptr; };
+static InversePair inverse_pair(const ace_sht_plan& pl, const float* E, float* X, long N2, const unsigned* emax, float* y, int Bt, int C) {
+    InversePair pr;
+    if (!pl.cut) return pr;
+    const int before = pl.route[1];
+    const int rc = run_legendre_inverse(pl, E, X, N2, nullptr, emax, true);
+    const bool folded = rc == ACE_OK && pl.route[1] >= 2;
+    pl.route[1] = before;
+    if (!folded) return pr;
+    pr.mcut = reinterpret_cast<const int*>(pl.cut_mcut.p);
+    pr.skip_dead = dft_inverse_fft_takes(dft_inverse_args(pl, X, nullptr, y, Bt, C, nullptr));
+    return pr;
 }
 
 extern "C" int ace_sht_plan_create_ex(int nlat, int nlon, int lmax, int mmax, const char* grid, int precision,
@@ -345,15 +407,17 @@
     if (!p || !x || !coeffs || n <= 0) return fail(ACE_ERR_INVALID, "ace_sht_forward: bad argument");
     hipStream_t s = static_cast<hipStream_t>(stream);
     const long N2 = 2L * n;
-    HIP_TRY(p->X.ensure(((size_t)p->mmax * p->nlat + LEG_STRIP_SLACK_ROWS) * N2));
+    HIP_TRY(p->X.ensure_x(((size_t)p->mmax * p->nlat + LEG_STRIP_SLACK_ROWS) * N2, p->sw.polar_poison));
     HIP_TRY(p->D.ensure(((size_t)p->lmax + LEG_STRIP_SLACK_ROWS) * p->mmax * N2));
     unsigned* xmax = nullptr;
     if (p->f16 && p->slots.p) {
         xmax = reinterpret_cast<unsigned*>(p->slots.p);
         HIP_TRY(launch_zero_u32(xmax, 2 * AMAX_SHARDS, s));
     }
-    ACE_TRY(run_dft_forward(*p, x, nullptr, nullptr, p->X.p, 1, n, s, xmax));
-    ACE_TRY(run_legendre_forward(*p, p->X.p, p->D.p, N2, s, xmax, xmax ? xmax + AMAX_SHARDS : nullptr));
+    unsigned* dmax = xmax ? xmax + AMAX_SHARDS : nullptr;
+    const int* mcut = forward_pair_mcut(*p, p->X.p, p->D.p, N2, xmax, dmax, false);
+    ACE_TRY(run_dft_forward(*p, x, nullptr, nullptr, p->X.p, 1, n, s, xmax, nullptr, nullptr, 0, nullptr, nullptr, nullptr, mcut));
+    ACE_TRY(run_legendre_forward(*p, p->X.p, p->D.p, N2, s, xmax, dmax));
     HIP_TRY(launch_spec_to_ref(p->D.p, coeffs, 1, n, p->lmax, p->mmax, s));
     return ACE_OK;
 }
@@ -361,7 +425,7 @@
     if (!p || !x || !coeffs || n <= 0) return fail(ACE_ERR_INVALID, "ace_sht_inverse: bad argument");
     hipStream_t s = static_cast<hipStream_t>(stream);
     const long N2 = 2L * n;
-    HIP_TRY(p->X.ensure(((size_t)p->mmax * p->nlat + LEG_STRIP_SLACK_ROWS) * N2));
+    HIP_TRY(p->X.ensure_x(((size_t)p->mmax * p->nlat + LEG_STRIP_SLACK_ROWS) * N2, p->sw.polar_poison));
     HIP_TRY(p->D.ensure(((size_t)p->lmax + LEG_STRIP_SLACK_ROWS) * p->mmax * N2));
     unsigned* emax = nullptr;
     if (p->f16 && p->slots.p) {
@@ -370,8 +434,9 @@
     }
     ACE_TRY(run_legendre_inverse(*p, p->D.p, p->X.p, N2, s, emax, true));
     HIP_TRY(launch_ref_to_spec(coeffs, p->D.p, 1, n, p->lmax, p->mmax, s, emax, p->route[1] != 0));
-    ACE_TRY(run_legendre_inverse(*p, p->D.p, p->X.p, N2, s, emax));
-    ACE_TRY(run_dft_inverse(*p, p->X.p, nullptr, x, 1, n, s));
+    const InversePair pr = inverse_pair(*p, p->D.p, p->X.p, N2, emax, x, 1, n);
+    ACE_TRY(run_legendre_inverse(*p, p->D.p, p->X.p, N2, s, emax, false, pr.skip_dead));
+    ACE_TRY(run_dft_inverse(*p, p->X.p, nullptr, x, 1, n, s, nullptr, pr.mcut));
     return ACE_OK;
 }
 
@@ -814,7 +879,7 @@
         if (rl < 1 || rm < 1) return fail(ACE_ERR_INVALID, "residual_filter_factor leaves no modes");
         ACE_TRY(plan_build(c.nlat, c.nlon, rl, rm, (Grid)c.data_grid, n->plan_res, false));
         const size_t n2 = (size_t)n->Bmax * 2 * c.in_chans;
-        HIP_TRY(n->resX.alloc(((size_t)rm * c.nlat + LEG_STRIP_SLACK_ROWS) * n2));
+        HIP_TRY(n->resX.alloc_x(((size_t)rm * c.nlat + LEG_STRIP_SLACK_ROWS) * n2, n->sw.polar_poison));
         HIP_TRY(n->resD.alloc(((size_t)rl + LEG_STRIP_SLACK_ROWS) * rm * n2));
         HIP_TRY(n->inF.alloc((size_t)n->Bmax * c.in_chans * n->HW));
     }
@@ -919,7 +984,7 @@
             HIP_TRY(n->Wp1.alloc((size_t)n->Bmax * ((n->hid + 15) / 16 * 16) * cp, true));
         }
     }
-    HIP_TRY(n->X.alloc(spec_x));
+    HIP_TRY(n->X.alloc_x(spec_x, n->sw.polar_poison));
     HIP_TRY(n->D.alloc(spec_d));
     HIP_TRY(n->E.alloc(spec_d));
     HIP_TRY(n->stats.alloc((size_t)4 * n->Bmax * C));
@@ -1552,10 +1617,12 @@
         HIP_TRY(launch_absmax(f.noise, (long)f.B * c.noise_embed_dim * f.HW, f.slot(16 + 12 * c.num_layers), f.s));
     if (n->plan_res) {
         const long NR = (long)f.B * 2 * Cin;
-        ACE_TRY(run_dft_forward(*n->plan_res, in, nullptr, nullptr, n->resX.p, f.B, Cin, f.s));
+        const int* mcut = forward_pair_mcut(*n->plan_res, n->resX.p, n->resD.p, NR, nullptr, nullptr, false);
+        ACE_TRY(run_dft_forward(*n->plan_res, in, nullptr, nullptr, n->resX.p, f.B, Cin, f.s, nullptr, nullptr, nullptr, 0, nullptr, nullptr, nullptr, mcut));
         ACE_TRY(run_legendre_forward(*n->plan_res, n->resX.p, n->resD.p, NR, f.s));
-        ACE_TRY(run_legendre_inverse(*n->plan_res, n->resD.p, n->resX.p, NR, f.s));
-        ACE_TRY(run_dft_inverse(*n->plan_res, n->resX.p, nullptr, n->inF.p, f.B, Cin, f.s, f.slot(7)));
+        const InversePair pr = inverse_pair(*n->plan_res, n->resD.p, n->resX.p, NR, nullptr, n->inF.p, f.B, Cin);
+        ACE_TRY(run_legendre_inverse(*n->plan_res, n->resD.p, n->resX.p, NR, f.s, nullptr, false, pr.skip_dead));
+        ACE_TRY(run_dft_inverse(*n->plan_res, n->resX.p, nullptr, n->inF.p, f.B, Cin, f.s, f.slot(7), pr.mcut));
         f.skip_in = n->inF.p;
         f.skip_in_slot = f.slot(7);
     }
@@ -1608,18 +1675,20 @@
         skip_pack.b = f.b0; skip_pack.bias = f.wt(p + "inner_skip.bias").buf.p; skip_pack.bf = n->bf0.p; skip_pack.nsamples = B;
     }
     const PackFragArgs* ride = b.ride_skip_pack ? &skip_pack : nullptr;
+    const int* mcut = forward_pair_mcut(*b.fwd, n->X.p, n->D.p, N2, xmax, dmax, b.dplanes);
     if (b.in_planes_only)
-        ACE_TRY(run_dft_forward(*b.fwd, nullptr, f.a0, f.b0, n->X.p, B, C, f.s, xmax, f.PBh, f.PBl, (long)C * f.HW, f.hslot(i), ride, &f.skip_pack_rode));
+        ACE_TRY(run_dft_forward(*b.fwd, nullptr, f.a0, f.b0, n->X.p, B, C, f.s, xmax, f.PBh, f.PBl, (long)C * f.HW, f.hslot(i), ride, &f.skip_pack_rode, mcut));
     else
-        ACE_TRY(run_dft_forward(*b.fwd, f.h, f.a0, f.b0, n->X.p, B, C, f.s, xmax, nullptr, nullptr, 0, nullptr, ride, &f.skip_pack_rode));
+        ACE_TRY(run_dft_forward(*b.fwd, f.h, f.a0, f.b0, n->X.p, B, C, f.s, xmax, nullptr, nullptr, 0, nullptr, ride, &f.skip_pack_rode, mcut));
     MARK(ST_DFT_FWD);
     ACE_TRY(run_legendre_forward(*b.fwd, n->X.p, n->D.p, N2, f.s, xmax, dmax, b.dplanes));
     MARK(ST_LEGENDRE_FWD);
     f.res = f.h; f.ra = f.a0; f.rb = f.b0;
     if (b.scale_residual) {
-        ACE_TRY(run_legendre_inverse(*b.inv, n->D.p, n->X.p, N2, f.s, dmax));
+        const InversePair pr = inverse_pair(*b.inv, n->D.p, n->X.p, N2, dmax, n->R.p, B, C);
+        ACE_TRY(run_legendre_inverse(*b.inv, n->D.p, n->X.p, N2, f.s, dmax, false, pr.skip_dead));
         MARK(ST_LEGENDRE_INV);
-        ACE_TRY(run_dft_inverse(*b.inv, n->X.p, nullptr, n->R.p, B, C, f.s));
+        ACE_TRY(run_dft_inverse(*b.inv, n->X.p, nullptr, n->R.p, B, C, f.s, nullptr, pr.mcut));
         MARK(ST_DFT_INV);
         f.res = n->R.p; f.ra = nullptr; f.rb = nullptr;
     }
@@ -1676,9 +1745,10 @@
 static int enqueue_inverse_transform(Fwd& f, int i, const BlockRoute& b) {
     const ace_sfno* n = f.n;
     const int sb = 16 + 12 * i;
-    ACE_TRY(run_legendre_inverse(*b.inv, n->E.p, n->X.p, (long)f.B * 2 * n->C, f.s, f.slot(sb + 2)));
+    const InversePair pr = inverse_pair(*b.inv, n->E.p, n->X.p, (long)f.B * 2 * n->C, f.slot(sb + 2), n->Y.p, f.B, n->C);
+    ACE_TRY(run_legendre_inverse(*b.inv, n->E.p, n->X.p, (long)f.B * 2 * n->C, f.s, f.slot(sb + 2), false, pr.skip_dead));
     MARK(ST_LEGENDRE_INV);
-    ACE_TRY(run_dft_inverse(*b.inv, n->X.p, f.W("blocks." + std::to_string(i) + ".filter.filter.bias"), n->Y.p, f.B, n->C, f.s, f.slot(sb + 7)));
+    ACE_TRY(run_dft_inverse(*b.inv, n->X.p, f.W("blocks." + std::to_string(i) + ".filter.filter.bias"), n->Y.p, f.B, n->C, f.s, f.slot(sb + 7), pr.mcut));
     MARK(ST_DFT_INV);
     f.HW = b.hw_out;
     return ACE_OK;
diff --git a/ace_amd/csrc/fft.hip b/ace_amd/csrc/fft.hip
--- a/ace_amd/csrc/fft.hip
+++ b/ace_amd/csrc/fft.hip
@@ -145,6 +145,7 @@
     const long HW = (long)p.H * W;
     constexpr int NPF = (R * (W / 4) + NT - 1) / NT;
     const int rlast = (p.C - c0 < R ? p.C - c0 : R) - 1;
+    const int Mc = p.mcut ? min(p.Mm, p.mcut[k]) : p.Mm;
 
     const int r1 = tid % R, b1 = tid / R;
     const int cr = c0 + (r1 < rlast ? r1 : rlast);
@@ -246,22 +247,25 @@
             const unsigned od = (unsigned)(k1 * ms + r) * 4u, om = (unsigned)((N1 - k1) * ms + r) * 4u;
             const int imoff = p.C * 4;
             const bool has_mirror = k1 > 0 && k1 < N1 / 2;
+            const int kc = k1 - Mc, kd = has_mirror ? k1 + Mc : 0;
             const v2f* zcol = Zs + k1 * ZP + r;
             sfft::CFft<N2, false, v2f>::run([&](int bb) { return zcol[bb * R]; }, [&](int q, v2f out) {
                 const float mag = FULLM ? 0.f : fmaxf(fabsf(out.x), fabsf(out.y));
                 if (FULLM) vmax = fmaxf(vmax, fmaxf(fabsf(out.x), fabsf(out.y)));
                 if (q < K2N) {
-                    const bool ok = k1 + N1 * q < p.Mm && (ACE_FFT_ABL != 1 || out.x == 1.2345e-30f);
+                    const bool ok = k1 + N1 * q < p.Mm;
+                    const bool st = kc + N1 * q < 0 && (ACE_FFT_ABL != 1 || out.x == 1.2345e-30f);
                     const auto rs = wide_rsrc(obase + (long)q * N1 * ms * 4);
-                    const int off = (int)(ok ? od : kDrop);
+                    const int off = (int)(st ? od : kDrop);
                     __builtin_amdgcn_raw_buffer_store_b32(__float_as_uint(out.x), rs, off, 0, 0);
                     __builtin_amdgcn_raw_buffer_store_b32(__float_as_uint(out.y), rs, off, imoff, 0);
                     if (!FULLM) vmax = fmaxf(vmax, ok ? mag : 0.f);
                 }
                 if (q >= N2 / 2) {
-                    const bool ok = has_mirror && (N1 - k1) + N1 * (N2 - 1 - q) < p.Mm && (ACE_FFT_ABL != 1 || out.x == 1.2345e-30f);
+                    const bool ok = has_mirror && (N1 - k1) + N1 * (N2 - 1 - q) < p.Mm;
+                    const bool st = N1 * (N2 - q) < kd && (ACE_FFT_ABL != 1 || out.x == 1.2345e-30f);
                     const auto rs = wide_rsrc(obase + (long)(N2 - 1 - q) * N1 * ms * 4);
-                    const int off = (int)(ok ? om : kDrop);
+                    const int off = (int)(st ? om : kDrop);
                     __builtin_amdgcn_raw_buffer_store_b32(__float_as_uint(out.x), rs, off, 0, 0);
                     __builtin_amdgcn_raw_buffer_store_b32(__float_as_uint(-out.y), rs, off, imoff, 0);
                     if (!FULLM) vmax = fmaxf(vmax, ok ? mag : 0.f);
@@ -270,8 +274,11 @@
         }
     }
     if (p.omax) {
-#pragma unroll
-        for (int off = 32; off > 0; off >>= 1) vmax = fmaxf(vmax, __shfl_xor(vmax, off, 64));
+        int ln = tid & 63;
+        asm volatile("" : "+v"(ln));
+#pragma unroll
+        for (int off = 32; off > 0; off >>= 1)
+            vmax = fmaxf(vmax, __int_as_float(__builtin_amdgcn_ds_bpermute((ln ^ off) << 2, __float_as_int(vmax))));
         __syncthreads();
         if ((tid & 63) == 0) smem[tid >> 6] = vmax;
         __syncthreads();
@@ -333,6 +340,7 @@
             constexpr unsigned kDrop = 0xF0000000u;
             const unsigned od = (unsigned)(k1 * ms + rr) * 4u, om = (unsigned)((N1 - k1) * ms + rr) * 4u;
             const int imoff = p.C * 4;
+            const int Mc = p.mcut ? min(p.Mm, p.mcut[k]) : p.Mm;
             v2f f[N2];
 #pragma unroll
             for (int k2 = 0; k2 < N2; ++k2) {
@@ -342,15 +350,15 @@
                 if (k2 == N2 / 2) {
                     const auto rs0 = wide_rsrc(sbase + (long)(N2 / 2) * N1 * ms * 4);
                     const auto rs1 = wide_rsrc(sbase + (long)(N2 / 2 - 1) * N1 * ms * 4);
-                    const int off0 = (int)((k1 == 0 && N1 * (N2 / 2) < p.Mm) ? od : kDrop);
-                    const int off1 = (int)((k1 > 0 && m < p.Mm) ? om : kDrop);
+                    const int off0 = (int)((k1 == 0 && N1 * (N2 / 2) < Mc) ? od : kDrop);
+                    const int off1 = (int)((k1 > 0 && m < Mc) ? om : kDrop);
                     const float re0 = __uint_as_float(__builtin_amdgcn_raw_buffer_load_b32(rs0, off0, 0, 0));
                     const float re1 = __uint_as_float(__builtin_amdgcn_raw_buffer_load_b32(rs1, off1, 0, 0));
                     const float im1 = __uint_as_float(__builtin_amdgcn_raw_buffer_load_b32(rs1, off1, imoff, 0));
                     f[k2] = v2f{re0 + re1, -im1};
                 } else {
                     const auto rs = wide_rsrc(sbase + (long)blk * N1 * ms * 4);
-                    const int off = (int)(m < p.Mm ? (mir ? om : od) : kDrop);
+                    const int off = (int)(m < Mc ? (mir ? om : od) : kDrop);
                     const float re = __uint_as_float(__builtin_amdgcn_raw_buffer_load_b32(rs, off, 0, 0));
                     const float im = __uint_as_float(__builtin_amdgcn_raw_buffer_load_b32(rs, off, imoff, 0));
                     f[k2] = v2f{re, mir ? -im : ((k2 == 0 && k1 == 0) ? 0.f : im)};
@@ -453,9 +461,13 @@
 
 bool dft_fft_has_width(int W) { return W == 360 || W == 1440 || W == 720 || W == 48 || W == 24 || W == 16; }
 
+bool dft_inverse_fft_takes(const DftArgs& a) {
+    return !(a.no_fft || (reinterpret_cast<uintptr_t>(a.y) & 15) != 0 || a.Mm > a.W / 2 + 1 || a.H > 65535 || a.Bt > 65535 || !lane_offsets_fit(a)) &&
+           dft_fft_has_width(a.W);
+}
+
 bool launch_dft_inverse_fft(const DftArgs& a, hipStream_t s, hipError_t* err) {
-    if (a.no_fft || (reinterpret_cast<uintptr_t>(a.y) & 15) != 0 || a.Mm > a.W / 2 + 1 || a.H > 65535 || a.Bt > 65535 || !lane_offsets_fit(a))
-        return false;
+    if (!dft_inverse_fft_takes(a)) return false;
     switch (a.W) {
         case 360: *err = launch_inv<20, 18, ACE_FFT_INV_ROWS>(a, s); return true;
         case 1440: *err = launch_inv<40, 36, ACE_FFT_QROWS>(a, s); return true;
diff --git a/ace_amd/csrc/kernels.h b/ace_amd/csrc/kernels.h
--- a/ace_amd/csrc/kernels.h
+++ b/ace_amd/csrc/kernels.h
@@ -22,6 +22,8 @@
     bool conv_wl = true;
     bool fused_pack = true;
     bool planes_stream = true;
+    bool no_polar_cut = false;
+    bool polar_poison = false;
     bool dense_grouped_filter = false;
 };
 Switches read_switches();
@@ -123,6 +125,8 @@
     int R = 0;
     int nbatch = 0;
     int mode = 0;
+    const int* r0 = nullptr;
+    bool kdrop = false;
 };
 constexpr int LEG_STRIP_SLACK_ROWS = 16;
 bool legendre_strip_eligible(const LegStripArgs& a);
@@ -200,6 +204,7 @@
     int Bt = 1, C = 0, H = 0, W = 0, Mm = 0;
     unsigned* omax = nullptr;
     bool no_fft = false;
+    const int* mcut = nullptr;
     PackFragArgs ride; int nride = 0; bool* rode = nullptr;
 };
 hipError_t launch_dft_forward(const DftArgs& a, hipStream_t s);
@@ -207,6 +212,7 @@
 bool launch_dft_forward_fft(const DftArgs& a, hipStream_t s, hipError_t* err);
 bool launch_dft_inverse_fft(const DftArgs& a, hipStream_t s, hipError_t* err);
 bool dft_fft_has_width(int W);
+bool dft_inverse_fft_takes(const DftArgs& a);
 
 struct ClnMfmaArgs {
     const float* x = nullptr; float* y = nullptr; long sx = 0;
diff --git a/ace_amd/csrc/strip_fold.hip b/ace_amd/csrc/strip_fold.hip
--- a/ace_amd/csrc/strip_fold.hip
+++ b/ace_amd/csrc/strip_fold.hip
@@ -50,7 +50,7 @@
 struct RowMap { int rbase, rstep, vlo, vhi; };
 
 template <int NH, int OUT, bool FULLN, int MODE>
-FDEV void fold_body(const LegStripArgs& p, char* smem, const int m, const int grp, const FoldGeom gm) {
+FDEV void fold_body(const LegStripArgs& p, char* smem, const int m, const int grp, const FoldGeom gm, const int r0, const int j0) {
     constexpr int NKP = 2 * NH;
     constexpr int FSLOT_BYTES = NKP * 2048;
     constexpr bool BIG = NH > NH_MAX;
@@ -65,11 +65,13 @@
     const int nc = n < N ? n : N - 1;
     char* ring = smem;
     char* Ts = smem + FNSLOT * FSLOT_BYTES + wave * FTS_BYTES;
-    const int nunits = 2 * gm.npairs;
+    const int tp0 = MODE == 1 ? r0 >> 5 : 0;
+    const int npairs = gm.npairs > tp0 ? gm.npairs - tp0 : 0;
+    const int nunits = 2 * npairs;
 
     const unsigned raw_b = slot_load(p.bmax + lane);
 
-    const _Float16* Am = p.A + (long)p.tile_off[m] * 1024;
+    const _Float16* Am = p.A + ((long)p.tile_off[m] + (long)tp0 * 2 * NKP) * 1024;
     auto issue_unit = [&](int u) {
         const int uu = u < nunits ? u : nunits - 1;
         const _Float16* src = Am + (long)uu * NKP * 1024 + lane * 8;
@@ -92,13 +94,14 @@
     if constexpr (MODE == 0) {
         const float* Xm = p.B + (long)m * p.b_moff;
         const long rowb = ks * 4;
-        const auto rsD = __builtin_amdgcn_make_buffer_rsrc(const_cast<float*>(Xm), 0, (unsigned)((long)gm.Hh * rowb), 0x00020000);
-        const auto rsM = __builtin_amdgcn_make_buffer_rsrc(const_cast<float*>(Xm + (long)gm.Hh * ks), 0, (unsigned)((long)(H - gm.Hh) * rowb), 0x00020000);
+        const int nD = gm.Hh - r0, nM = H - gm.Hh - r0;
+        const auto rsD = __builtin_amdgcn_make_buffer_rsrc(const_cast<float*>(Xm + (long)r0 * ks), 0, (unsigned)((long)(nD > 0 ? nD : 0) * rowb), 0x00020000);
+        const auto rsM = __builtin_amdgcn_make_buffer_rsrc(const_cast<float*>(Xm + (long)gm.Hh * ks), 0, (unsigned)((long)(nM > 0 ? nM : 0) * rowb), 0x00020000);
         unsigned vd[8], vm[8];
 #pragma unroll
         for (int e = 0; e < 8; ++e) {
-            vd[e] = (unsigned)(((long)(8 * g + e) * ks + nc) * 4);
-            vm[e] = (unsigned)(((long)(H - 1 - gm.Hh - (8 * g + e)) * ks + nc) * 4);
+            vd[e] = (unsigned)(((long)(16 * j0 + 8 * g + e - r0) * ks + nc) * 4);
+            vm[e] = (unsigned)(((long)(H - 1 - gm.Hh - (16 * j0 + 8 * g + e)) * ks + nc) * 4);
         }
         constexpr int CHK = BIG ? 4 : NKP;
 #pragma unroll
@@ -175,7 +178,8 @@
         }
     };
     auto store_tile = [&](const RowMap rm, const f32x16& acc, auto inner_tag) {
-        constexpr bool NOMASK = decltype(inner_tag)::value && FULLN;
+        constexpr bool NOMASK = decltype(inner_tag)::value && FULLN && MODE == 0;
+        constexpr bool NOCOL = decltype(inner_tag)::value && FULLN;
         if (OUT == 2) {
 #pragma unroll
             for (int r = 0; r < 16; ++r) {
@@ -209,7 +213,7 @@
                 const int rl = ps * 8 + (lane >> 3);
                 const int row = rm.rbase + rm.rstep * (16 * hf + rl);
                 const u32x4 d = *reinterpret_cast<const u32x4*>(T32 + rl * 32 + c4);
-                const bool ok = NOMASK || (row >= rm.vlo && row < rm.vhi && ncol < N);
+                const bool ok = NOMASK || (row >= rm.vlo && row < rm.vhi && (NOCOL || ncol < N));
                 if (OUT == 1) {
                     u32x2 hi2, lo2;
                     hi2[0] = (d[0] & 0xffffu) | (d[1] << 16);
@@ -233,8 +237,8 @@
         }
     };
     auto fwd_map = [&](int tp, int par) { return RowMap{m + par + 64 * tp, 2, 0, R}; };
-    auto north_map = [&](int tp) { return RowMap{32 * tp, 1, 0, gm.Hh}; };
-    auto south_map = [&](int tp) { return RowMap{H - 1 - 32 * tp, -1, gm.Hh, H}; };
+    auto north_map = [&](int tp) { return RowMap{32 * (tp0 + tp), 1, r0, gm.Hh}; };
+    auto south_map = [&](int tp) { return RowMap{H - 1 - 32 * (tp0 + tp), -1, gm.Hh, H - r0}; };
 
     auto unit = [&](int u, auto par_tag, auto&& under) -> f32x16 {
         constexpr int PAR = decltype(par_tag)::value;
@@ -289,14 +293,14 @@
 #pragma unroll
     for (int r = 0; r < 16; ++r) { pa[r] = 0.f; pb[r] = 0.f; }
     if constexpr (MODE == 0) {
-        for (int tp = 0; tp < gm.npairs; ++tp) {
+        for (int tp = 0; tp < npairs; ++tp) {
             const f32x16 ev = unit(2 * tp, T0{}, [&] {
                 if (tp > 0) {
                     if (OUT != 1) tile_max(fwd_map(tp - 1, 1), pb, std::true_type{});
                     store_tile(fwd_map(tp - 1, 1), pb, std::true_type{});
                 }
             });
-            const bool last = tp + 1 == gm.npairs;
+            const bool last = tp + 1 == npairs;
             pb = unit(2 * tp + 1, T1{}, [&] {
                 if (!last) {
                     if (OUT != 1) tile_max(fwd_map(tp, 0), ev, std::true_type{});
@@ -306,11 +310,11 @@
             if (last) pa = ev;
         }
     } else if constexpr (BIG) {
-        for (int tp = 0; tp < gm.npairs; ++tp) {
+        for (int tp = 0; tp < npairs; ++tp) {
             const f32x16 ev = unit(2 * tp, T0{}, [] {});
             const f32x16 od = unit(2 * tp + 1, T1{}, [] {});
             f32x16 t = ev + od;
-            const bool inner = tp + 1 < gm.npairs;
+            const bool inner = tp + 1 < npairs;
             if (inner) { tile_max(north_map(tp), t, std::true_type{}); store_tile(north_map(tp), t, std::true_type{}); }
             else { tile_max(north_map(tp), t, std::false_type{}); store_tile(north_map(tp), t, std::false_type{}); }
             __builtin_amdgcn_sched_barrier(0);
@@ -320,7 +324,7 @@
             __builtin_amdgcn_sched_barrier(0);
         }
     } else {
-        for (int tp = 0; tp < gm.npairs; ++tp) {
+        for (int tp = 0; tp < npairs; ++tp) {
             const f32x16 ev = unit(2 * tp, T0{}, [&] {
                 if (tp > 0) {
                     tile_max(north_map(tp - 1), pa, std::true_type{});
@@ -339,9 +343,9 @@
     }
     asm volatile("s_waitcnt vmcnt(0)" ::: "memory");
     constexpr bool STORED_IN_LOOP = BIG && MODE == 1;
-    const int tl = gm.npairs - 1;
+    const int tl = npairs - 1;
     const RowMap ma = MODE == 0 ? fwd_map(tl, 0) : north_map(tl), mb = MODE == 0 ? fwd_map(tl, 1) : south_map(tl);
-    if (OUT != 1 && gm.npairs > 0 && !STORED_IN_LOOP) {
+    if (OUT != 1 && npairs > 0 && !STORED_IN_LOOP) {
         tile_max(ma, pa, std::false_type{});
         tile_max(mb, pb, std::false_type{});
     }
@@ -355,7 +359,7 @@
         if (tid == 0) atomicMax(p.omax + (blockIdx.x & 63), __float_as_uint(fmaxf(fmaxf(red[0], red[1]), fmaxf(red[2], red[3]))));
         __syncthreads();
     }
-    if (gm.npairs > 0 && !STORED_IN_LOOP) {
+    if (npairs > 0 && !STORED_IN_LOOP) {
         store_tile(ma, pa, std::false_type{});
         store_tile(mb, pb, std::false_type{});
     }
@@ -375,11 +379,13 @@
     const int m = (idx / G) * 8 + xcd;
     const int grp = idx % G;
     if (m >= p.nbatch) return;
-    const FoldGeom gm = fold_geom(MODE, m, p.R, p.K);
+    const int r0 = p.r0 ? p.r0[m] : 0;
+    const int j0 = MODE == 0 && p.kdrop ? r0 >> 4 : 0;
+    const FoldGeom gm = fold_geom_cut(MODE, m, p.R, p.K, j0);
     switch (gm.nkp2) {
-        case 2: fold_body<1, OUT, FULLN, MODE>(p, smem, m, grp, gm); break;
-        case 4: fold_body<2, OUT, FULLN, MODE>(p, smem, m, grp, gm); break;
-        case 6: fold_body<3, OUT, FULLN, MODE>(p, smem, m, grp, gm); break;
+        case 2: fold_body<1, OUT, FULLN, MODE>(p, smem, m, grp, gm, r0, j0); break;
+        case 4: fold_body<2, OUT, FULLN, MODE>(p, smem, m, grp, gm, r0, j0); break;
+        case 6: fold_body<3, OUT, FULLN, MODE>(p, smem, m, grp, gm, r0, j0); break;
         default: break;
     }
 #ifdef ACE_LF_TRACE
@@ -401,16 +407,18 @@
     const int grp = idx % G;
     if (m >= p.nbatch) return;
     const FoldGeom gm = fold_geom(MODE, m, p.R, p.K);
+    const int r0 = p.r0 ? p.r0[m] : 0;
+    constexpr int j0 = 0;
     switch (gm.nkp2) {
-        case 12: fold_body<6, OUT, true, MODE>(p, smem_big, m, grp, gm); break;
-        case 18: fold_body<9, OUT, true, MODE>(p, smem_big, m, grp, gm); break;
-        case 24: fold_body<12, OUT, true, MODE>(p, smem_big, m, grp, gm); break;
+        case 12: fold_body<6, OUT, true, MODE>(p, smem_big, m, grp, gm, r0, j0); break;
+        case 18: fold_body<9, OUT, true, MODE>(p, smem_big, m, grp, gm, r0, j0); break;
+        case 24: fold_body<12, OUT, true, MODE>(p, smem_big, m, grp, gm, r0, j0); break;
         default:
             if constexpr (MODE == 1) {
                 switch (gm.nkp2) {
-                    case 2: fold_body<1, OUT, true, MODE>(p, smem_big, m, grp, gm); break;
-                    case 4: fold_body<2, OUT, true, MODE>(p, smem_big, m, grp, gm); break;
-                    case 6: fold_body<3, OUT, true, MODE>(p, smem_big, m, grp, gm); break;
+                    case 2: fold_body<1, OUT, true, MODE>(p, smem_big, m, grp, gm, r0, j0); break;
+                    case 4: fold_body<2, OUT, true, MODE>(p, smem_big, m, grp, gm, r0, j0); break;
+                    case 6: fold_body<3, OUT, true, MODE>(p, smem_big, m, grp, gm, r0, j0); break;
                     default: break;
                 }
             }
diff --git a/ace_amd/csrc/strip_pack.h b/ace_amd/csrc/strip_pack.h
--- a/ace_amd/csrc/strip_pack.h
+++ b/ace_amd/csrc/strip_pack.h
@@ -164,19 +164,33 @@
     return mx > 0.0 ? worst / mx : 0.0;
 }
 
-inline void pack_legendre_fold(const float* tab, int mmax, int nlat, int lmax, int pitch, int mode, float scale, StripPack& out) {
+#if defined(__HIPCC__)
+__host__ __device__
+#endif
+inline FoldGeom fold_geom_cut(int mode, int m, int R, int K, int j0) {
+    FoldGeom g = fold_geom(mode, m, R, K);
+    if (mode == 0 && j0 > 0) {
+        g.nkp = g.nkp > j0 ? g.nkp - j0 : 0;
+        g.nkp2 = fold_round_nkp(g.nkp);
+    }
+    return g;
+}
+
+inline void pack_legendre_fold(const float* tab, int mmax, int nlat, int lmax, int pitch, int mode, float scale, StripPack& out,
+                               const int* kskip = nullptr) {
     const int R = mode == 0 ? lmax : nlat, K = mode == 0 ? nlat : lmax;
     out.tile_off.assign((size_t)mmax, 0);
     long blocks = 0;
     for (int m = 0; m < mmax; ++m) {
-        const FoldGeom g = fold_geom(mode, m, R, K);
+        const FoldGeom g = fold_geom_cut(mode, m, R, K, kskip ? kskip[m] : 0);
         out.tile_off[m] = (int)blocks;
         blocks += (long)g.npairs * 2 * g.nkp2;
     }
     out.blocks = blocks;
     out.frags.assign((size_t)blocks * 1024, 0);
     for (int m = 0; m < mmax; ++m) {
-        const FoldGeom g = fold_geom(mode, m, R, K);
+        const int j0 = mode == 0 && kskip ? kskip[m] : 0;
+        const FoldGeom g = fold_geom_cut(mode, m, R, K, j0);
         for (int u = 0; u < 2 * g.npairs; ++u) {
             const int tp = u >> 1, p = u & 1;
             for (int jj = 0; jj < g.nkp; ++jj) {
@@ -184,7 +198,7 @@
                 for (int lane = 0; lane < 64; ++lane) {
                     const int i = lane & 31, gg = lane >> 5;
                     for (int e = 0; e < 8; ++e) {
-                        const int c = 16 * jj + 8 * gg + e;
+                        const int c = 16 * (j0 + jj) + 8 * gg + e;
                         const int kf = mode == 0 ? c : 32 * tp + i;
                         const int l = m + p + 2 * (mode == 0 ? 32 * tp + i : c);
                         float v = 0.f;
@@ -206,6 +220,68 @@
     }
 }
 
+struct PolarCut {
+    std::vector<int> r0;
+    std::vector<int> mcut;
+    bool ok = false;
+    double dead_share = 0.0;
+};
+inline bool fold_pack_row_live(const StripPack& sp, int mode, int m, int kf, int nlat, int lmax) {
+    const int R = mode == 0 ? lmax : nlat, K = mode == 0 ? nlat : lmax;
+    const FoldGeom g = fold_geom(mode, m, R, K);
+    const uint16_t* base = sp.frags.data() + (size_t)sp.tile_off[m] * 1024;
+    auto nz = [](const uint16_t* blk, int at) { return ((blk[at] | blk[512 + at]) & 0x7fffu) != 0; };
+    for (int u = 0; u < 2 * g.npairs; ++u) {
+        if (mode == 0) {
+            const int jj = kf / 16, gg = (kf % 16) / 8, e = kf % 8;
+            if (jj >= g.nkp) continue;
+            const uint16_t* blk = base + ((size_t)u * g.nkp2 + jj) * 1024;
+            for (int i = 0; i < 32; ++i)
+                if (nz(blk, (i + 32 * gg) * 8 + e)) return true;
+        } else {
+            if ((u >> 1) != kf / 32) continue;
+            for (int jj = 0; jj < g.nkp; ++jj) {
+                const uint16_t* blk = base + ((size_t)u * g.nkp2 + jj) * 1024;
+                for (int gg = 0; gg < 2; ++gg)
+                    for (int e = 0; e < 8; ++e)
+                        if (nz(blk, (kf % 32 + 32 * gg) * 8 + e)) return true;
+            }
+        }
+    }
+    return false;
+}
+inline PolarCut derive_polar_cut(const StripPack& fwd, const StripPack& inv, int mmax, int nlat, int lmax) {
+    PolarCut c;
+    const int Hh = (nlat + 1) / 2;
+    c.r0.assign((size_t)mmax, 0);
+    c.mcut.assign((size_t)nlat, mmax);
+    c.ok = true;
+    long dead = 0;
+    for (int m = 0; m < mmax; ++m) {
+        int r = Hh;
+        for (int kf = 0; kf < Hh; ++kf) {
+            const bool live = fold_pack_row_live(fwd, 0, m, kf, nlat, lmax) || fold_pack_row_live(inv, 1, m, kf, nlat, lmax);
+            if (live) r = r < kf ? r : kf;
+            else if (r < Hh) c.ok = false;
+        }
+        c.r0[m] = r;
+        if (m > 0 && r < c.r0[m - 1]) c.ok = false;
+    }
+    if (!c.ok) {
+        c.r0.assign((size_t)mmax, 0);
+        return c;
+    }
+    for (int lat = 0; lat < nlat; ++lat) {
+        const int kf = lat < nlat - 1 - lat ? lat : nlat - 1 - lat;
+        int mc = mmax;
+        for (int m = mmax - 1; m >= 0 && c.r0[m] > kf; --m) mc = m;
+        c.mcut[lat] = mc;
+        dead += mmax - mc;
+    }
+    c.dead_share = mmax > 0 && nlat > 0 ? (double)dead / ((double)mmax * nlat) : 0.0;
+    return c;
+}
+
 inline float cln_frag_scale(float wabs) {
     int e = 0;
     if (wabs > 0.f && std::isfinite(wabs)) { (void)std::frexp(wabs, &e); e = 10 - e; }
```

Measured after the change: 190.9 steps/s, median of 6. 1.02x the previous value.
